# haowenz/FEM

Hardware: AMD Instinct MI355X
Metric: mapped Mreads/s (100 bp, e=3) at 1/2/4/8 MI355X + achieved HBM GB/s vs roofline (higher is better)
Workload: dtype u32/u64 integer + 32-bit Myers bit-vectors

## Files before the change

### fem_amd/csrc/fem_hip.hip

```cpp
#include "../../include/fem_hip.h"

#include <hip/hip_runtime.h>
#include <rccl/rccl.h>
#include <sched.h>
#if defined(__x86_64__)
#include <immintrin.h>
#endif

#include <algorithm>
#include <cctype>
#include <cstdio>
#include <cstdlib>
#include <cstring>
#include <condition_variable>
#include <functional>
#include <atomic>
#include <chrono>
#include <mutex>
#include <string>
#include <thread>
#include <vector>

#include "fem_index_build.hip.h"
#include "fem_pack.h"
#include "fem_kernels.hip.h"
#include "fem_seed_fast.hip.h"
#include "fem_seed_join.hip.h"
#include "fem_tail.hip.h"
#include "fem_bgzf.hip.h"

namespace {

#ifndef FEM_SLOTS
#define FEM_SLOTS 4
#endif
constexpr int kSlots = FEM_SLOTS;
constexpr uint32_t kMaxReadLen = 1024;
constexpr size_t kFrontPad = 16;
constexpr uint32_t kXcapSmall = 512, kFcap = 128, kCcap = 128;

constexpr int kTimedKernels = 15;
struct TimedLaunch {
  int kernel;
  hipEvent_t start, stop;
  bool counts = true;
};
constexpr int kMaxParts = 4;

struct Slot {
  hipStream_t stream = nullptr;
  uint8_t *d_bases_alloc = nullptr;
  uint8_t *bases() const { return d_bases_alloc + 16; }
  size_t bases_cap = 0;
  uint64_t *d_off = nullptr;
  size_t off_cap = 0;
  uint64_t n_reads = 0;
  uint64_t n_bases = 0;
  uint32_t max_len = 0;
  bool staged = false;
  char *h_bases = nullptr;
  size_t h_bases_cap = 0;
  uint64_t *h_off = nullptr;
  size_t h_off_cap = 0;
  uint64_t acq_reads = 0, acq_bases = 0;
  char *h_quals = nullptr, *h_names = nullptr;
  uint64_t *h_name_off = nullptr;
  size_t h_quals_cap = 0, h_names_cap = 0, h_name_off_cap = 0;
  uint8_t *d_quals = nullptr, *d_names = nullptr;
  uint64_t *d_name_off = nullptr;
  size_t d_quals_cap = 0, d_names_cap = 0, d_name_off_cap = 0;
  bool text_staged = false;
  bool host_quals = false;
  const uint64_t *qual_at = nullptr;
  hipStream_t text_stream = nullptr;
  hipStream_t out_stream = nullptr;
  hipEvent_t ev_text_staged = nullptr;
  hipEvent_t ev_text_order = nullptr;
  bool have_text_order = false;
  uint8_t *d_packed = nullptr;
  size_t packed_cap = 0;
  uint32_t *d_exc_bits = nullptr;
  size_t exc_bits_cap = 0;
  uint32_t packed_bpr = 0;
  bool prefetch_results = false, staged_by_copy = false;
  uint64_t prefetched_reads2 = 0, prefetched_cand = 0, last_n_cand = 0;
  uint64_t h2d_bytes = 0;
  bool sent_packed = false;
  int parts = 1;
  uint32_t part_begin[kMaxParts + 1] = {0, 0, 0, 0, 0};
  hipEvent_t ev_part[kMaxParts] = {nullptr, nullptr, nullptr, nullptr}, ev_sel[kMaxParts] = {nullptr, nullptr, nullptr, nullptr};
  hipEvent_t ev_zeroed = nullptr;
  hipEvent_t ev_results = nullptr, ev_home = nullptr;
  uint64_t *d_cand = nullptr;
  uint32_t *d_meta = nullptr;
  uint8_t *d_ed = nullptr;
  int16_t *d_end = nullptr;
  uint32_t cand_cap = 0;
  uint32_t *d_begin = nullptr, *d_count = nullptr, *d_nmap = nullptr;
  size_t per_read_cap = 0;
  uint8_t *d_ctl = nullptr;
  uint8_t *h_ctl = nullptr;
  uint64_t *d_arena = nullptr;
  uint64_t arena_cap = 0;
  uint32_t *d_slow = nullptr;
  uint32_t slow_cap = 0;
  uint2 *d_sel = nullptr, *d_sel_hdr = nullptr;
  size_t sel_cap = 0, sel_hdr_cap = 0;
  uint32_t *h_begin = nullptr, *h_count = nullptr;
  size_t h_per_read_cap = 0;
  uint64_t *h_cand = nullptr;
  uint8_t *h_ed = nullptr;
  int16_t *h_end = nullptr;
  size_t h_cand_cap = 0;
  uint8_t *d_count8 = nullptr, *d_ped = nullptr;
  uint32_t *d_seg = nullptr;
  uint64_t *d_pcand = nullptr;
  int16_t *d_pend = nullptr;
  uint2 *d_big = nullptr;
  size_t count8_cap = 0, seg_cap = 0, pcand_cap = 0;
  uint8_t *h_count8 = nullptr, *h_ped = nullptr;
  uint32_t *h_seg = nullptr;
  uint64_t *h_pcand = nullptr;
  int16_t *h_pend = nullptr;
  uint2 *h_big = nullptr;
  size_t h_count8_cap = 0, h_seg_cap = 0, h_pcand_cap = 0;
  bool want_packed = false;
  bool packed_enqueued = false;
  uint64_t packed_home = 0, last_n_packed = 0;
  bool packed_per_read_home = false;
  uint32_t n_packed = 0, n_big = 0;
  fem_params params{};
  bool mapped = false, synced = false;
  uint64_t stats[5] = {0, 0, 0, 0, 0};
  uint32_t n_cand = 0;
  std::vector<TimedLaunch> pending;
  femt::Tail *tail = nullptr;
  bool paired = false;
  int32_t min_insert = 0, max_insert = 0;
  uint64_t n_proper = 0;
  bool rescue = false;
  int32_t rescue_edits = 0;
  uint64_t n_rescued = 0;
  bool mapq = false;
  bool unmapped = false;
  uint64_t n_unmapped = 0;
  std::vector<uint16_t> pr_flag;
  std::vector<uint32_t> pr_tid, pr_pos0, pr_cigar_off, pr_cigar, pr_md_off;
  std::vector<uint8_t> pr_nm;
  std::vector<char> pr_md;
};

constexpr size_t kCtlPackCursor = 4 * sizeof(uint32_t) + 2 * sizeof(uint64_t) + 4 * sizeof(uint64_t);
constexpr size_t kCtlBytes = kCtlPackCursor + 2 * sizeof(uint32_t);
constexpr uint32_t kBigCap = 4096;
constexpr size_t kCtlWorkCursor = 128, kCtlWorkCursor2 = 192, kCtlPartStride = 128, kCtlAlloc = 1024;
static_assert(kCtlWorkCursor2 + (kMaxParts - 1) * kCtlPartStride + 64 <= kCtlAlloc, "control block layout");
static_assert(kCtlBytes <= kCtlWorkCursor, "control block layout");

}

namespace {
class StagePool {
 public:
  ~StagePool() {
    {
      std::lock_guard<std::mutex> l(m_);
      stop_ = true;
    }
    cv_.notify_all();
    for (auto &t : threads_) t.join();
  }
  void run(unsigned n, const std::function<void(unsigned)> &work) {
    if (n <= 1) return work(0u);
    {
      std::lock_guard<std::mutex> l(m_);
      while (threads_.size() + 1 < n) {
        const unsigned id = (unsigned)threads_.size() + 1;
        threads_.emplace_back([this, id] { loop(id); });
      }
      work_ = &work, n_ = n, pending_ = n - 1, ++epoch_;
    }
    cv_.notify_all();
    work(0u);
    std::unique_lock<std::mutex> l(m_);
    done_.wait(l, [&] { return pending_ == 0; });
    work_ = nullptr;
  }

 private:
  void loop(unsigned id) {
    uint64_t seen = 0;
    for (;;) {
      const std::function<void(unsigned)> *w = nullptr;
      {
        std::unique_lock<std::mutex> l(m_);
        cv_.wait(l, [&] { return stop_ || (epoch_ != seen && id < n_); });
        if (stop_) return;
        seen = epoch_, w = work_;
      }
      (*w)(id);
      std::lock_guard<std::mutex> l(m_);
      if (--pending_ == 0) done_.notify_one();
    }
  }
  std::mutex m_;
  std::condition_variable cv_, done_;
  std::vector<std::thread> threads_;
  const std::function<void(unsigned)> *work_ = nullptr;
  unsigned n_ = 0, pending_ = 0;
  uint64_t epoch_ = 0;
  bool stop_ = false;
};
}

struct fem_dev {
  femt::TextGate text_gate;
  femz::Bgzf *bgzf = nullptr;
  uint8_t *d_zin = nullptr;
  size_t d_zin_cap = 0;
  hipStream_t z_stream = nullptr;
  std::recursive_mutex mu;
  int device = 0;
  StagePool *stage_pool = nullptr;
  uint8_t *d_ref_names = nullptr;
  uint32_t *d_ref_name_off = nullptr;
  int n_cu = 256;
  std::string err;
  uint32_t *d_lookup = nullptr;
  uint64_t n_lookup = 0;
  uint64_t *d_occ = nullptr;
  uint64_t n_occ = 0;
  int32_t k = 0, step = 0;
  uint64_t fast_occ_key = ~0ull;
  int fast_occ_blocks = 0;
  uint32_t *d_summary = nullptr;
  uint32_t *d_occ32 = nullptr, *d_goff = nullptr, *d_blkseq = nullptr;
  uint32_t list_shift = 0;
  bool no_strided = false;
  uint32_t *d_freq11 = nullptr;
  uint32_t n_banks = 1, bank_first[5] = {0, 0, 0, 0, 0};
  uint32_t *d_bank_lo = nullptr;
  uint64_t bank_limit = 0;
  uint32_t bank_seqs = 0;
  int select_occ_blocks = 0, join_occ_blocks = 0;
  uint64_t select_occ_key = ~0ull, join_occ_key = ~0ull;
  uint8_t *d_planes = nullptr;
  uint8_t *d_ref_raw = nullptr;
  uint64_t ref_bytes = 0;
  uint64_t *d_seq_off = nullptr;
  uint32_t *d_seq_len = nullptr;
  uint32_t n_seq = 0;
  std::vector<uint64_t> seq_off;
  std::vector<uint32_t> seq_len;
  Slot slot[kSlots];
  bool timing = false;
  int verify_blocks_per_cu = 0;
  double t_ms[kTimedKernels] = {};
  uint64_t t_n[kTimedKernels] = {};
  bool force_generic = false;
  bool force_hash = false;
  bool force_dense = false;
  bool no_dense = false;
  bool tiny_buffers = false;
  std::vector<hipEvent_t> event_pool;
  hipEvent_t ev_kernels_done = nullptr;
  bool have_kernels_done = false;
  hipEvent_t ev_select_done = nullptr;
  bool have_select_done = false;
  bool no_overlap = false;
  hipEvent_t ev_h2d_done = nullptr;
  bool have_h2d_done = false;
  hipStream_t side_stream = nullptr;
  bool no_parts = false;
  int max_parts = 2;
  bool timeline = false, have_epoch = false;
  hipEvent_t ev_epoch = nullptr;
};

namespace {

bool testing_switch(const char *name) {
  const char *t = getenv("FEM_TESTING");
  if (!(t && t[0] == '1')) return false;
  const char *v = getenv(name);
  return v && v[0] == '1';
}

int fail(fem_dev *h, int rc, const std::string &msg) {
  if (h) {
    std::lock_guard<std::recursive_mutex> lock(h->mu);
    h->err = msg;
  }
  return rc;
}
#define FEM_LOCK(h) std::lock_guard<std::recursive_mutex> fem_lock_(h->mu)

#define HIP_TRY(h, expr)                                                                          \
  do {                                                                                            \
    hipError_t e_ = (expr);                                                                       \
    if (e_ != hipSuccess)                                                                         \
      return fail(h, e_ == hipErrorOutOfMemory ? FEM_ERR_NOMEM : FEM_ERR_HIP,                     \
                  std::string(#expr) + ": " + hipGetErrorString(e_));                             \
  } while (0)

template <typename T>
int dev_realloc(fem_dev *h, T **p, size_t *cap, size_t want, bool keep = false) {
  if (want <= *cap && *p) return FEM_OK;
  size_t n = std::max(want, *cap + *cap / 2);
  T *q = nullptr;
  HIP_TRY(h, hipMalloc((void **)&q, std::max<size_t>(n, 1) * sizeof(T)));
  if (keep && *p && *cap) HIP_TRY(h, hipMemcpy(q, *p, *cap * sizeof(T), hipMemcpyDeviceToDevice));
  if (*p) (void)hipFree(*p);
  *p = q;
  *cap = n;
  return FEM_OK;
}

template <typename T>
int pinned_realloc(fem_dev *h, T **p, size_t *cap, size_t want) {
  if (want <= *cap && *p) return FEM_OK;
  size_t n = std::max(want, *cap + *cap / 2);
  if (*p) (void)hipHostFree(*p);
  *p = nullptr;
  HIP_TRY(h, hipHostMalloc((void **)p, std::max<size_t>(n, 1) * sizeof(T), hipHostMallocDefault));
  *cap = n;
  return FEM_OK;
}

bool params_ok(const fem_params *p) {
  return p && p->k >= 1 && p->k <= 16 && p->step >= 1 && p->step <= 16 && p->e >= 0 && p->e <= 7 && p->a >= 0 &&
         p->a <= 2;
}

femk::SeedLayout make_layout(const fem_params &p, uint32_t max_len) {
  femk::SeedLayout l{};
  const uint32_t R = (uint32_t)(p.e + 1 + p.a);
  const uint32_t lg = (uint32_t)(p.k / p.step + (p.k % p.step ? 1 : 0));
  const uint32_t n_groups = 2u * (uint32_t)p.step;
  uint32_t smax = max_len >= (uint32_t)p.k ? max_len - (uint32_t)p.k + 1u : 1u;
  int c = (int)(smax / (uint32_t)p.step) - (int)(R * lg) + 2;
  uint32_t cmax = (uint32_t)std::max(c, 2);
  l.smax = smax;
  l.cmax = cmax;
  l.cw = (cmax + 31u) / 32u;
  l.n_words = (max_len + 15u) / 16u + 2u;
  l.xcap = kXcapSmall, l.fcap = kFcap, l.ccap = kCcap;
  uint32_t o = 0;
  auto take = [&](uint32_t bytes) {
    uint32_t at = o;
    o += (bytes + 15u) & ~15u;
    return at;
  };
  l.pkw = take(l.n_words * 4u);
  l.nkw = take(l.n_words * 4u);
  l.sf = take(2u * smax * 8u);
  l.dp_rows = take(n_groups * 2u * cmax * 4u);
  l.dp_bits = take(std::max(n_groups * R * l.cw * 4u, n_groups * R * 8u));
  l.picked = take(n_groups * R * 16u);
  l.rb = take(2u * (R + 1u) * 4u);
  l.X = take(l.xcap * 8u);
  l.F = take(l.fcap * 8u);
  l.A = take(l.ccap * 8u);
  l.B = take(l.ccap * 8u);
  l.wave_bytes = o;
  return l;
}

femk::SeedLayout make_layout_fast(const fem_params &p, uint32_t max_len, bool hash) {
  femk::SeedLayout l{};
  const uint32_t R = (uint32_t)(p.e + 1 + p.a);
  const uint32_t n_groups = 2u * (uint32_t)p.step;
  l.smax = max_len >= (uint32_t)p.k ? max_len - (uint32_t)p.k + 1u : 1u;
  l.n_words = (max_len + 15u) / 16u + 2u;
  l.xcap = 64;
  uint32_t o = 0;
  auto take = [&](uint32_t bytes) {
    uint32_t at = o;
    o += (bytes + 15u) & ~15u;
    return at;
  };
  if (hash) {
    l.pkw = take(l.n_words * 4u);
    l.nkw = take(l.n_words * 4u);
  }
  if (hash) l.sf = take(std::max(2u * l.smax * 8u, 2u * 64u * 8u));
  l.dp_bits = take(std::max(n_groups, femk::kGroupQueue) * R * 8u);
  if (hash) {
    l.X = take(64u * 8u);
    l.A = take(femk::kListScratchBytes);
  }
  l.B = take(2u * femk::kReadBlock * 8u);
  if (!hash) {
    const uint32_t blk_chars = femk::kReadBlock * std::min(max_len, 256u);
    l.strm_words = blk_chars / 16u + 3u;
    l.strm = take(3u * l.strm_words * 4u);
    const uint32_t q_at = o;
    l.F = take(femk::kQueueBytes);
    const uint32_t g0 = l.smax / (uint32_t)femk::kStep;
    const uint32_t n_used = g0 > (uint32_t)femk::kLg ? g0 - (uint32_t)femk::kLg + 1u : 1u;
    l.gq_cap = std::max(384u, n_groups * n_used);
    l.gq = take(std::max(l.gq_cap * 4u + femk::kGroupQueue * 16u + 2u * 32u * 4u, femk::kFlushScratchBytes));
    l.blk_bytes = blk_chars + 32u;
    l.blk = q_at;
    if (o < q_at + l.blk_bytes) take(q_at + l.blk_bytes - o);
  }
  if (hash) {
    l.xcap = (uint32_t)femk::bloom_chunks((int)R) * 64u;
    l.F = take(femk::bloom_slots((int)R) / 16u * 4u);
  }
  l.wave_bytes = o;
  return l;
}

femk::SeedLayout make_layout_select(const fem_params &p, uint32_t max_len) {
  femk::SeedLayout l{};
  const uint32_t R = (uint32_t)(p.e + 1 + p.a);
  l.smax = max_len >= (uint32_t)p.k ? max_len - (uint32_t)p.k + 1u : 1u;
  const uint32_t g_max = std::min<uint32_t>((l.smax + 2u) / 3u, femk::kSelMaxCols - 1u + 4u * R);
  l.gstride = 3u * g_max + 2u;
  l.gstride += l.gstride & 1u;
  if (!((l.gstride >> 1) & 1u)) l.gstride += 2u;
  l.nb = std::max<uint32_t>(1u, std::min<uint32_t>(femk::kReadBlock, 3100u / (2u * 2u * l.gstride)));
  l.strm_words = (l.nb * max_len + 15u) / 16u + 2u;
  uint32_t o = 0;
  auto take = [&](uint32_t bytes) {
    uint32_t at = o;
    o += (bytes + 15u) & ~15u;
    return at;
  };
  l.rb = take((femk::kReadBlock + 2u) * 8u);
  l.rinfo = take(4u * femk::kReadBlock * 4u);
  l.strm = take(2u * l.strm_words * 4u);
  l.fq = take(l.nb * 2u * l.gstride * 2u + 256u);
  l.wave_bytes = o;
  return l;
}

femk::SeedLayout make_layout_join(const fem_params &p, bool banked, bool padded = false) {
  femk::SeedLayout l{};
  const uint32_t R = (uint32_t)(p.e + 1 + p.a);
  uint32_t o = 0;
  auto take = [&](uint32_t bytes) {
    uint32_t at = o;
    o += (bytes + 15u) & ~15u;
    return at;
  };
  l.sf = take(2u * 64u * 4u);
  l.X = take(64u * 4u);
  l.A = take(3u * (femk::dense_flag_cap((int)R) + 1u) * 4u);
  l.B = take(2u * femk::kReadBlock * 8u);
  l.F = take(femk::join_bitmap_words((int)R, padded) * 4u);
  if (banked) l.gq = take(2u * 64u * 8u);
  l.wave_bytes = o;
  l.picked = 0;
  return l;
}

template <int R>
void launch_select_r(bool banked, dim3 grid, dim3 block, uint32_t lds, hipStream_t st, const femk::SeedParams &sp) {
  if (banked)
    hipLaunchKernelGGL((femk::seed_select_kernel<R, true>), grid, block, lds, st, sp);
  else
    hipLaunchKernelGGL((femk::seed_select_kernel<R>), grid, block, lds, st, sp);
}
template <int R>
int select_blocks_per_cu_r(bool banked, int block, uint32_t lds) {
  int nb = 0;
  const hipError_t e = banked ? hipOccupancyMaxActiveBlocksPerMultiprocessor(&nb, femk::seed_select_kernel<R, true>, block, lds)
                              : hipOccupancyMaxActiveBlocksPerMultiprocessor(&nb, femk::seed_select_kernel<R>, block, lds);
  return e == hipSuccess ? nb : 0;
}
typedef void (*JoinKernel)(femk::SeedParams);
JoinKernel join_kernel(int R, int which) {
  static const JoinKernel k[3][femk::kMaxR] = {
      {femk::seed_join_kernel_r1, femk::seed_join_kernel_r2, femk::seed_join_kernel_r3, femk::seed_join_kernel_r4, femk::seed_join_kernel_r5,
       femk::seed_join_kernel_r6, femk::seed_join_kernel_r7, femk::seed_join_kernel_r8, femk::seed_join_kernel_r9, femk::seed_join_kernel_r10},
      {femk::seed_join_banked_kernel_r1, femk::seed_join_banked_kernel_r2, femk::seed_join_banked_kernel_r3, femk::seed_join_banked_kernel_r4,
       femk::seed_join_banked_kernel_r5, femk::seed_join_banked_kernel_r6, femk::seed_join_banked_kernel_r7, femk::seed_join_banked_kernel_r8,
       femk::seed_join_banked_kernel_r9, femk::seed_join_banked_kernel_r10},
      {femk::seed_join_kernel_padded_r1, femk::seed_join_kernel_padded_r2, femk::seed_join_kernel_padded_r3, femk::seed_join_kernel_padded_r4,
       femk::seed_join_kernel_padded_r5, femk::seed_join_kernel_padded_r6, femk::seed_join_kernel_padded_r7, femk::seed_join_kernel_padded_r8,
       femk::seed_join_kernel_padded_r9, femk::seed_join_kernel_padded_r10}};
  return k[which][std::min(std::max(R, 1), femk::kMaxR) - 1];
}

#define FEM_DENSE_SWITCH(R, CALL)      \
  switch (R) {                         \
    case 1: CALL(1); break;            \
    case 2: CALL(2); break;            \
    case 3: CALL(3); break;            \
    case 4: CALL(4); break;            \
    case 5: CALL(5); break;            \
    case 6: CALL(6); break;            \
    case 7: CALL(7); break;            \
    case 8: CALL(8); break;            \
    case 9: CALL(9); break;            \
    default: CALL(10); break;          \
  }
template <int R>
uint32_t kernel_regs_r(bool join, int which) {
  hipFuncAttributes a{};
  const bool banked = which == 1;
  const void *f = join ? (const void *)join_kernel(R, which)
                       : banked ? (const void *)femk::seed_select_kernel<R, true> : (const void *)femk::seed_select_kernel<R>;
  return hipFuncGetAttributes(&a, f) == hipSuccess && a.numRegs > 0 ? (uint32_t)a.numRegs : 128u;
}
uint32_t kernel_regs(int R, bool join, int which = 0) {
  static std::atomic<uint32_t> cache[3][2][femk::kMaxR + 1] = {};
  std::atomic<uint32_t> &slot = cache[which][join ? 1 : 0][std::min(std::max(R, 1), femk::kMaxR)];
  uint32_t c = slot.load(std::memory_order_relaxed);
  if (c) return c;
#define FEM_CALL(r) c = kernel_regs_r<r>(join, which)
  FEM_DENSE_SWITCH(R, FEM_CALL)
#undef FEM_CALL
  slot.store(c, std::memory_order_relaxed);
  return c;
}
int select_blocks_per_cu(int R, bool banked, int block, uint32_t lds) {
  int nb = 0;
#define FEM_CALL(r) nb = select_blocks_per_cu_r<r>(banked, block, lds)
  FEM_DENSE_SWITCH(R, FEM_CALL)
#undef FEM_CALL
  return nb;
}
void launch_select(int R, bool banked, dim3 grid, dim3 block, uint32_t lds, hipStream_t st, const femk::SeedParams &sp) {
#define FEM_CALL(r) launch_select_r<r>(banked, grid, block, lds, st, sp)
  FEM_DENSE_SWITCH(R, FEM_CALL)
#undef FEM_CALL
}
int join_blocks_per_cu(int R, int which, int block, uint32_t lds) {
  int nb = 0;
  return hipOccupancyMaxActiveBlocksPerMultiprocessor(&nb, join_kernel(R, which), block, lds) == hipSuccess ? nb : 0;
}
void launch_join(int R, int which, dim3 grid, dim3 block, uint32_t lds, hipStream_t st, const femk::SeedParams &sp) {
  hipLaunchKernelGGL(join_kernel(R, which), grid, block, lds, st, sp);
}

template <int R>
void launch_fast(bool hash, dim3 grid, dim3 block, uint32_t lds, hipStream_t st, const femk::SeedParams &sp) {
  if (hash)
    hipLaunchKernelGGL((femk::seed_fast_kernel<R, true>), grid, block, lds, st, sp);
  else
    hipLaunchKernelGGL((femk::seed_fast_kernel<R, false>), grid, block, lds, st, sp);
}

template <int R>
int fast_blocks_per_cu_r(bool hash, int block, uint32_t lds) {
  int nb = 0;
  hipError_t err = hash ? hipOccupancyMaxActiveBlocksPerMultiprocessor(&nb, femk::seed_fast_kernel<R, true>, block, lds)
                        : hipOccupancyMaxActiveBlocksPerMultiprocessor(&nb, femk::seed_fast_kernel<R, false>, block, lds);
  return err == hipSuccess ? nb : 0;
}
int fast_blocks_per_cu(int R, bool hash, int block, uint32_t lds) {
  switch (R) {
    case 1: return fast_blocks_per_cu_r<1>(hash, block, lds);
    case 2: return fast_blocks_per_cu_r<2>(hash, block, lds);
    case 3: return fast_blocks_per_cu_r<3>(hash, block, lds);
    case 4: return fast_blocks_per_cu_r<4>(hash, block, lds);
    case 5: return fast_blocks_per_cu_r<5>(hash, block, lds);
    case 6: return fast_blocks_per_cu_r<6>(hash, block, lds);
    case 7: return fast_blocks_per_cu_r<7>(hash, block, lds);
    case 8: return fast_blocks_per_cu_r<8>(hash, block, lds);
    case 9: return fast_blocks_per_cu_r<9>(hash, block, lds);
    default: return fast_blocks_per_cu_r<10>(hash, block, lds);
  }
}

hipEvent_t get_event(fem_dev *h) {
  if (!h->event_pool.empty()) {
    hipEvent_t e = h->event_pool.back();
    h->event_pool.pop_back();
    return e;
  }
  hipEvent_t e = nullptr;
  (void)hipEventCreate(&e);
  return e;
}

struct Span {
  fem_dev *h;
  Slot &s;
  hipStream_t st;
  TimedLaunch t;
  bool on;
  Span(fem_dev *h_, Slot &s_, int id, hipStream_t st_) : h(h_), s(s_), st(st_), t{id, nullptr, nullptr, false}, on(h_->timing && h_->timeline) {
    if (on) {
      t.start = get_event(h), t.stop = get_event(h);
      (void)hipEventRecord(t.start, st);
    }
  }
  ~Span() {
    if (on) {
      (void)hipEventRecord(t.stop, st);
      s.pending.push_back(t);
    }
  }
};

void drain_timing(fem_dev *h, Slot &s) {
  for (auto &t : s.pending) {
    float ms = 0.f;
    if (hipEventElapsedTime(&ms, t.start, t.stop) == hipSuccess && t.kernel < kTimedKernels) {
      h->t_ms[t.kernel] += ms;
      h->t_n[t.kernel] += t.counts ? 1 : 0;
    }
    if (h->timeline && h->have_epoch) {
      float a = 0.f, b = 0.f;
      if (hipEventElapsedTime(&a, h->ev_epoch, t.start) == hipSuccess && hipEventElapsedTime(&b, h->ev_epoch, t.stop) == hipSuccess)
        fprintf(stderr, "TL slot %d id %2d  %9.3f %9.3f  (%.3f)\n", (int)(&s - h->slot), t.kernel, a, b, b - a);
    }
    h->event_pool.push_back(t.start);
    h->event_pool.push_back(t.stop);
  }
  s.pending.clear();
}

int ensure_outputs(fem_dev *h, Slot &s) {
  size_t want_reads = (size_t)s.n_reads;
  if (want_reads > s.per_read_cap || !s.d_begin) {
    size_t cap = std::max<size_t>(want_reads, 1);
    if (s.d_begin) (void)hipFree(s.d_begin);
    if (s.d_count) (void)hipFree(s.d_count);
    if (s.d_nmap) (void)hipFree(s.d_nmap);
    s.d_begin = s.d_count = s.d_nmap = nullptr;
    HIP_TRY(h, hipMalloc((void **)&s.d_begin, cap * 2 * sizeof(uint32_t)));
    HIP_TRY(h, hipMalloc((void **)&s.d_count, cap * 2 * sizeof(uint32_t)));
    HIP_TRY(h, hipMalloc((void **)&s.d_nmap, cap * sizeof(uint32_t)));
    s.per_read_cap = cap;
  }
  if (!s.d_cand || !s.d_meta || !s.d_ed || !s.d_end || s.cand_cap == 0) {
    for (void *p : {(void *)s.d_cand, (void *)s.d_meta, (void *)s.d_ed, (void *)s.d_end})
      if (p) (void)hipFree(p);
    s.d_cand = nullptr, s.d_meta = nullptr, s.d_ed = nullptr, s.d_end = nullptr;
    uint64_t want = 2 * s.n_reads + (5u << 20);
    if (h->tiny_buffers) want = 512;
    want = std::min<uint64_t>(want, 0xFFFFFFF0ull);
    s.cand_cap = 0;
    size_t c0 = 0, c1 = 0, c2 = 0, c3 = 0;
    int rc;
    if ((rc = dev_realloc(h, &s.d_cand, &c0, want))) return rc;
    if ((rc = dev_realloc(h, &s.d_meta, &c1, want))) return rc;
    if ((rc = dev_realloc(h, &s.d_ed, &c2, want))) return rc;
    if ((rc = dev_realloc(h, &s.d_end, &c3, want))) return rc;
    s.cand_cap = (uint32_t)want;
  }
  if (!s.d_ctl) {
    HIP_TRY(h, hipMalloc((void **)&s.d_ctl, kCtlAlloc));
    HIP_TRY(h, hipHostMalloc((void **)&s.h_ctl, kCtlBytes, hipHostMallocDefault));
  }
  if (!s.d_arena) {
    s.arena_cap = h->tiny_buffers ? 256u : (4u << 20);
    HIP_TRY(h, hipMalloc((void **)&s.d_arena, s.arena_cap * sizeof(uint64_t)));
  }
  {
    const double avg_bucket = (double)h->n_occ / (double)(h->n_lookup ? h->n_lookup : 1);
    uint64_t want = avg_bucket > 1.0 ? s.n_reads + (1u << 20) : (1u << 18);
    if (h->tiny_buffers) want = s.d_slow ? s.slow_cap : 32;
    if (want > s.slow_cap || !s.d_slow) {
      if (s.d_slow) (void)hipFree(s.d_slow);
      s.d_slow = nullptr;
      HIP_TRY(h, hipMalloc((void **)&s.d_slow, want * sizeof(uint32_t)));
      s.slow_cap = (uint32_t)want;
    }
  }
  return FEM_OK;
}

int grow_candidates(fem_dev *h, Slot &s, uint64_t want) {
  if (want > 0xFFFFFFF0ull) return fail(h, FEM_ERR_UNSUPPORTED, "more than 2^32 candidates in one batch; split the batch");
  s.cand_cap = 0;
  for (void *p : {(void *)s.d_cand, (void *)s.d_meta, (void *)s.d_ed, (void *)s.d_end})
    if (p) (void)hipFree(p);
  s.d_cand = nullptr, s.d_meta = nullptr, s.d_ed = nullptr, s.d_end = nullptr;
  HIP_TRY(h, hipMalloc((void **)&s.d_cand, want * sizeof(uint64_t)));
  HIP_TRY(h, hipMalloc((void **)&s.d_meta, want * sizeof(uint32_t)));
  HIP_TRY(h, hipMalloc((void **)&s.d_ed, want * sizeof(uint8_t)));
  HIP_TRY(h, hipMalloc((void **)&s.d_end, want * sizeof(int16_t)));
  s.cand_cap = (uint32_t)want;
  return FEM_OK;
}

int h2d_begin(fem_dev *h, Slot &s) {
  if (h->have_h2d_done) HIP_TRY(h, hipStreamWaitEvent(s.stream, h->ev_h2d_done, 0));
  return FEM_OK;
}
int h2d_end(fem_dev *h, Slot &s) {
  HIP_TRY(h, hipEventRecord(h->ev_h2d_done, s.stream));
  h->have_h2d_done = true;
  return FEM_OK;
}
bool device_idle(fem_dev *h) {
  return (!h->have_kernels_done || hipEventQuery(h->ev_kernels_done) == hipSuccess) &&
         (!h->have_select_done || hipEventQuery(h->ev_select_done) == hipSuccess);
}
constexpr uint64_t kPartMinReads = 1u << 16;

hipStream_t d2h_begin(fem_dev *h, Slot &s) {
  (void)h;
  return s.stream;
}
int d2h_end(fem_dev *h, Slot &s, hipStream_t st) {
  if (st == s.stream) return FEM_OK;
  HIP_TRY(h, hipEventRecord(s.ev_home, st));
  HIP_TRY(h, hipStreamWaitEvent(s.stream, s.ev_home, 0));
  return FEM_OK;
}

int enqueue_pack(fem_dev *h, Slot &s, bool kernel, bool send_home) {
  const size_t n2 = (size_t)s.n_reads * 2, n_seg = (n2 + 255) / 256;
  int rc;
  if ((rc = dev_realloc(h, &s.d_count8, &s.count8_cap, n2 + 16))) return rc;
  if ((rc = dev_realloc(h, &s.d_seg, &s.seg_cap, n_seg + 4))) return rc;
  if (s.pcand_cap < s.cand_cap || !s.d_pcand) {
    for (void *q : {(void *)s.d_pcand, (void *)s.d_ped, (void *)s.d_pend})
      if (q) (void)hipFree(q);
    s.d_pcand = nullptr, s.d_ped = nullptr, s.d_pend = nullptr, s.pcand_cap = 0;
    HIP_TRY(h, hipMalloc((void **)&s.d_pcand, (size_t)s.cand_cap * sizeof(uint64_t)));
    HIP_TRY(h, hipMalloc((void **)&s.d_ped, (size_t)s.cand_cap * sizeof(uint8_t)));
    HIP_TRY(h, hipMalloc((void **)&s.d_pend, (size_t)s.cand_cap * sizeof(int16_t)));
    s.pcand_cap = s.cand_cap;
  }
  if (!s.d_big) HIP_TRY(h, hipMalloc((void **)&s.d_big, kBigCap * sizeof(uint2)));
  if (n2 + 16 > s.h_count8_cap || !s.h_count8) {
    if (s.h_count8) (void)hipHostFree(s.h_count8);
    s.h_count8 = nullptr, s.h_count8_cap = 0;
    if ((rc = pinned_realloc(h, &s.h_count8, &s.h_count8_cap, n2 + 16))) return rc;
  }
  if (n_seg + 4 > s.h_seg_cap || !s.h_seg) {
    if (s.h_seg) (void)hipHostFree(s.h_seg);
    s.h_seg = nullptr, s.h_seg_cap = 0;
    if ((rc = pinned_realloc(h, &s.h_seg, &s.h_seg_cap, n_seg + 4))) return rc;
  }
  if (!s.h_big) {
    size_t c = 0;
    if ((rc = pinned_realloc(h, &s.h_big, &c, (size_t)kBigCap))) return rc;
  }
  if (kernel) {
  femk::PackParams pp{};
  pp.cand_begin = s.d_begin, pp.cand_count = s.d_count, pp.cand = s.d_cand, pp.ed = s.d_ed, pp.end = s.d_end;
  pp.ctr = (const uint32_t *)s.d_ctl, pp.n_strands = (uint32_t)n2;
  pp.count8 = s.d_count8, pp.seg_begin = s.d_seg, pp.pcand = s.d_pcand, pp.ped = s.d_ped, pp.pend = s.d_pend, pp.pcap = (uint32_t)s.pcand_cap;
  pp.cursor = (uint32_t *)(s.d_ctl + kCtlPackCursor), pp.big = s.d_big, pp.big_cap = kBigCap;
  const uint32_t grid = (uint32_t)std::max<size_t>(1, (n_seg + femk::kPackSegs - 1) / femk::kPackSegs);
  {
    TimedLaunch t{6, nullptr, nullptr, true};
    if (h->timing) {
      t.start = get_event(h), t.stop = get_event(h);
      HIP_TRY(h, hipEventRecord(t.start, s.stream));
    }
    hipLaunchKernelGGL(femk::pack_results_kernel, dim3(grid), dim3(256), 0, s.stream, pp);
    HIP_TRY(h, hipGetLastError());
    if (h->timing) {
      HIP_TRY(h, hipEventRecord(t.stop, s.stream));
      s.pending.push_back(t);
    }
  }
  s.packed_enqueued = true;
  }
  if (send_home) {
    hipStream_t st = d2h_begin(h, s);
    {
      Span span(h, s, 21, st);
      HIP_TRY(h, hipMemcpyAsync(s.h_count8, s.d_count8, n2, hipMemcpyDeviceToHost, st));
      HIP_TRY(h, hipMemcpyAsync(s.h_seg, s.d_seg, n_seg * sizeof(uint32_t), hipMemcpyDeviceToHost, st));
      s.packed_per_read_home = true;
      const size_t guess = std::min<size_t>({(size_t)(s.last_n_packed + s.last_n_packed / 32 + 1024), s.h_pcand_cap, s.pcand_cap});
      if (s.last_n_packed && s.h_pcand && guess) {
        HIP_TRY(h, hipMemcpyAsync(s.h_pcand, s.d_pcand, guess * sizeof(uint64_t), hipMemcpyDeviceToHost, st));
        HIP_TRY(h, hipMemcpyAsync(s.h_ped, s.d_ped, guess * sizeof(uint8_t), hipMemcpyDeviceToHost, st));
        HIP_TRY(h, hipMemcpyAsync(s.h_pend, s.d_pend, guess * sizeof(int16_t), hipMemcpyDeviceToHost, st));
        s.packed_home = guess;
      }
    }
    if ((rc = d2h_end(h, s, st))) return rc;
  }
  return FEM_OK;
}

int launch_batch(fem_dev *h, Slot &s) {
  const fem_params &p = s.params;
  uint32_t *d_ctr = (uint32_t *)s.d_ctl;
  unsigned long long *d_arena_ctr = (unsigned long long *)(s.d_ctl + 4 * sizeof(uint32_t));
  unsigned long long *d_stats = (unsigned long long *)(s.d_ctl + 4 * sizeof(uint32_t) + 2 * sizeof(uint64_t));
  int parts = 1;
  uint32_t part_begin[kMaxParts + 1] = {0, 0, 0, 0, 0};
  const bool copied_in_parts = s.parts > 1;
  {
    const int R_ = p.e + 1 + p.a;
    const bool dense_overlap = !h->force_generic && p.k == femk::kK && p.step == femk::kStep && R_ >= 1 && R_ <= femk::kMaxR && h->d_occ32 &&
                               h->d_freq11 && !h->no_overlap;
    if (dense_overlap && !h->no_parts && s.n_reads >= 2 * kPartMinReads && (copied_in_parts || device_idle(h))) {
      parts = copied_in_parts ? s.parts : (int)std::min<uint64_t>((uint64_t)h->max_parts, s.n_reads / kPartMinReads);
      for (int q = 0; q <= parts; ++q)
        part_begin[q] = copied_in_parts ? s.part_begin[q] : q == parts ? (uint32_t)s.n_reads : (uint32_t)((s.n_reads * q / parts) & ~63ull);
    }
    s.parts = 1;
  }
  if (parts > 1) {
    if (h->have_select_done) HIP_TRY(h, hipStreamWaitEvent(h->side_stream, h->ev_select_done, 0));
    HIP_TRY(h, hipMemsetAsync(s.d_ctl, 0, kCtlAlloc, h->side_stream));
  } else {
    HIP_TRY(h, hipMemsetAsync(s.d_ctl, 0, kCtlAlloc, s.stream));
  }

  femk::SeedParams sp{};
  sp.bases = s.bases();
  sp.read_off = s.d_off;
  sp.n_reads = (uint32_t)s.n_reads;
  sp.read_begin = 0;
  sp.lookup = h->d_lookup;
  sp.occ = h->d_occ;
  sp.inf32 = (uint32_t)h->n_occ;
  sp.seq_len = h->d_seq_len;
  sp.e = p.e, sp.a = p.a, sp.R = p.e + 1 + p.a, sp.k = p.k, sp.step = p.step;
  sp.lg = p.k / p.step + (p.k % p.step ? 1 : 0);
  sp.cand = s.d_cand, sp.cand_meta = s.d_meta, sp.cand_cap = s.cand_cap;
  sp.cand_begin = s.d_begin, sp.cand_count = s.d_count;
  sp.ctr = d_ctr;
  sp.work_cursor = (uint32_t *)(s.d_ctl + kCtlWorkCursor);
  sp.stats = d_stats;
  sp.arena = s.d_arena, sp.arena_cap = s.arena_cap, sp.arena_ctr = d_arena_ctr;
  sp.lay = make_layout(p, std::max<uint32_t>(s.max_len, (uint32_t)p.k));

  sp.n_seq = h->n_seq;
  sp.summary = h->d_summary;
  sp.slow_queue = s.d_slow, sp.slow_cap = s.slow_cap;
  sp.work_queue = nullptr;
  const int R = p.e + 1 + p.a;
  const bool use_fast = !h->force_generic && p.k == femk::kK && p.step == femk::kStep && R >= 1 && R <= femk::kMaxR;

  auto shape = [&](const femk::SeedLayout &lay, uint32_t *wpb_out, uint32_t *lds_out, uint32_t *grid_out) {
    uint32_t wpb = std::min<uint32_t>(4u, std::max<uint32_t>(1u, (64u * 1024u) / lay.wave_bytes));
    uint32_t lds_bytes = wpb * lay.wave_bytes;
    uint32_t waves_per_cu = std::min<uint32_t>(32u, (160u * 1024u / lds_bytes) * wpb);
    uint64_t blocks_wanted = (s.n_reads + wpb - 1) / wpb;
    uint64_t blocks_resident = (uint64_t)h->n_cu * std::max<uint32_t>(1u, waves_per_cu / wpb);
    *wpb_out = wpb, *lds_out = lds_bytes;
    *grid_out = (uint32_t)std::max<uint64_t>(1, std::min<uint64_t>(blocks_wanted, blocks_resident * 4));
  };
  if (sp.lay.wave_bytes > 64u * 1024u) return fail(h, FEM_ERR_UNSUPPORTED, "read too long for the device path");

  auto timed = [&](int id, hipStream_t st, auto &&launch, bool counts = true) -> int {
    TimedLaunch t{id, nullptr, nullptr, counts};
    if (h->timing) {
      t.start = get_event(h), t.stop = get_event(h);
      HIP_TRY(h, hipEventRecord(t.start, st));
    }
    launch();
    HIP_TRY(h, hipGetLastError());
    if (h->timing) {
      HIP_TRY(h, hipEventRecord(t.stop, st));
      s.pending.push_back(t);
    }
    return FEM_OK;
  };

  if (s.n_reads) {
    int rc;
    const bool split_dense = use_fast && h->d_occ32 && h->d_freq11;
    const bool overlap = split_dense && !h->no_overlap;
    if (!overlap && h->have_kernels_done) HIP_TRY(h, hipStreamWaitEvent(s.stream, h->ev_kernels_done, 0));
    femk::VerifyParams vp{};
    vp.bases = s.bases(), vp.read_off = s.d_off;
    vp.planes = h->d_planes, vp.seq_off = h->d_seq_off;
    vp.cand = s.d_cand, vp.cand_meta = s.d_meta;
    vp.ctr = d_ctr, vp.cand_cap = s.cand_cap, vp.e = p.e;
    vp.ed = s.d_ed, vp.end = s.d_end;
    vp.n_map = s.d_nmap, vp.stats = d_stats;
    HIP_TRY(h, hipMemsetAsync(s.d_nmap, 0, (size_t)s.n_reads * sizeof(uint32_t), s.stream));
    if (h->verify_blocks_per_cu == 0) {
      int nb = 0;
      if (hipOccupancyMaxActiveBlocksPerMultiprocessor(&nb, femk::verify_kernel, 256, 0) != hipSuccess || nb <= 0) nb = 4;
      h->verify_blocks_per_cu = nb;
    }
    const uint32_t vgrid = (uint32_t)h->n_cu * (uint32_t)h->verify_blocks_per_cu;
    if (split_dense) {
      const uint32_t max_len = std::max<uint32_t>(s.max_len, (uint32_t)p.k);
      const bool banked = h->n_banks > 1;
      const size_t want_sel = (size_t)s.n_reads * 6u * (size_t)R * h->n_banks;
      if ((rc = dev_realloc(h, &s.d_sel, &s.sel_cap, want_sel))) return rc;
      if ((rc = dev_realloc(h, &s.d_sel_hdr, &s.sel_hdr_cap, (size_t)s.n_reads))) return rc;
      femk::SeedParams fp = sp;
      fp.occ32 = h->d_occ32, fp.list_shift = h->list_shift, fp.goff = h->d_goff, fp.blkseq = h->d_blkseq;
      fp.freq11 = h->d_freq11, fp.sel = s.d_sel, fp.sel_hdr = s.d_sel_hdr;
      fp.n_banks = h->n_banks, fp.bank_lo = h->d_bank_lo, fp.n_buckets = (uint32_t)(h->n_lookup - 1);
      fp.blk_stride = (femk::kDenseRemap >> femk::kDenseBlkShift) + 1u;
      for (uint32_t b = 0; b <= femk::kDenseMaxBanks; ++b) fp.bank_first[b] = h->bank_first[b];
      uint32_t select_lds = 0, select_threads = 256;
      fp.lay = make_layout_select(p, max_len);
      if (fp.lay.wave_bytes > 64u * 1024u) return fail(h, FEM_ERR_UNSUPPORTED, "read too long for the device path");
      const femk::SeedLayout lay_select = fp.lay;
      femk::SeedLayout lay_join = make_layout_join(p, banked, !banked && h->list_shift != 0);
      const uint32_t wpb_s = std::min<uint32_t>(4u, std::max<uint32_t>(1u, (64u * 1024u) / lay_select.wave_bytes));
      const uint32_t wpb_j = std::min<uint32_t>(4u, std::max<uint32_t>(1u, (60u * 1024u) / lay_join.wave_bytes));
      lay_join.picked = wpb_j * lay_join.wave_bytes;
      const uint32_t lds_j = wpb_j * lay_join.wave_bytes + 64u * 8u;
      const int which = banked ? 1 : h->list_shift ? 2 : 0;
      uint64_t per_cu_s, per_cu_j;
      {
        const uint32_t lds_bytes = wpb_s * lay_select.wave_bytes;
        const uint64_t key = ((uint64_t)banked << 48) | ((uint64_t)R << 40) | lds_bytes;
        if (h->select_occ_key != key) h->select_occ_key = key, h->select_occ_blocks = select_blocks_per_cu(R, banked, (int)(64u * wpb_s), lds_bytes);
        per_cu_s = h->select_occ_blocks > 0 ? (uint64_t)h->select_occ_blocks : std::max<uint64_t>(1, 160u * 1024u / lds_bytes);
        if (overlap) per_cu_s = 1;
        select_lds = lds_bytes, select_threads = 64u * wpb_s;
      }
      {
        const uint64_t key = ((uint64_t)which << 48) | ((uint64_t)R << 40) | lds_j;
        if (h->join_occ_key != key) h->join_occ_key = key, h->join_occ_blocks = join_blocks_per_cu(R, which, (int)(64u * wpb_j), lds_j);
        per_cu_j = h->join_occ_blocks > 0 ? (uint64_t)h->join_occ_blocks : std::max<uint64_t>(1, 160u * 1024u / lds_j);
        if (overlap) {
          const uint32_t vj = (kernel_regs(R, true, which) + 7u) & ~7u, vs = (kernel_regs(R, false, banked ? 1 : 0) + 7u) & ~7u;
          const uint32_t wj = 64u * wpb_j / 256u ? 64u * wpb_j / 256u : 1u, ws = select_threads / 256u ? select_threads / 256u : 1u;
          const uint32_t lj = (lds_j + 511u) & ~511u, ls = (select_lds + 511u) & ~511u;
          while (per_cu_j > 1 && (per_cu_j * wj * vj + ws * vs > 512u || per_cu_j * lj + ls > 160u * 1024u || per_cu_j * wj + ws > 8u)) --per_cu_j;
        }
      }
      if (parts > 1 && !copied_in_parts) {
        HIP_TRY(h, hipEventRecord(s.ev_zeroed, s.stream));
        HIP_TRY(h, hipStreamWaitEvent(h->side_stream, s.ev_zeroed, 0));
      }
      for (int q = 0; q < parts; ++q) {
        const uint32_t r_lo = parts > 1 ? part_begin[q] : 0u, r_hi = parts > 1 ? part_begin[q + 1] : (uint32_t)s.n_reads;
        const uint64_t blocks_of_reads = ((uint64_t)(r_hi - r_lo) + femk::kReadBlock - 1) / femk::kReadBlock;
        fp.read_begin = r_lo, fp.n_reads = r_hi;
        hipStream_t st_sel = parts > 1 ? h->side_stream : s.stream;
        {
          fp.lay = lay_select;
          if (parts > 1) {
            if (copied_in_parts) HIP_TRY(h, hipStreamWaitEvent(st_sel, s.ev_part[q], 0));
          } else if (overlap && h->have_select_done) {
            HIP_TRY(h, hipStreamWaitEvent(s.stream, h->ev_select_done, 0));
          }
          const uint32_t grid = (uint32_t)std::max<uint64_t>(1, std::min<uint64_t>((blocks_of_reads + wpb_s - 1) / wpb_s, (uint64_t)h->n_cu * per_cu_s));
          fp.work_cursor = (uint32_t *)(s.d_ctl + kCtlWorkCursor + (size_t)q * kCtlPartStride);
          rc = timed(8, st_sel, [&] { launch_select(R, banked, dim3(grid), dim3(64u * wpb_s), select_lds, st_sel, fp); }, q == 0);
          if (rc) return rc;
          if (parts > 1) {
            HIP_TRY(h, hipEventRecord(s.ev_sel[q], st_sel));
            HIP_TRY(h, hipStreamWaitEvent(s.stream, s.ev_sel[q], 0));
          }
          if (overlap && q + 1 == parts) {
            HIP_TRY(h, hipEventRecord(h->ev_select_done, st_sel));
            h->have_select_done = true;
          }
          if (overlap && q == 0 && h->have_kernels_done) HIP_TRY(h, hipStreamWaitEvent(s.stream, h->ev_kernels_done, 0));
        }
        {
          fp.lay = lay_join;
          const uint32_t grid = (uint32_t)std::max<uint64_t>(1, std::min<uint64_t>((blocks_of_reads + wpb_j - 1) / wpb_j, (uint64_t)h->n_cu * per_cu_j));
          fp.work_cursor = (uint32_t *)(s.d_ctl + kCtlWorkCursor2 + (size_t)q * kCtlPartStride);
          rc = timed(0, s.stream, [&] { launch_join(R, which, dim3(grid), dim3(64u * wpb_j), lds_j, s.stream, fp); }, q == 0);
          if (rc) return rc;
        }
      }
      sp.work_queue = s.d_slow;
    } else if (use_fast) {
      femk::SeedParams fp = sp;
      const bool hash = h->force_hash || (double)h->n_occ > (double)h->n_lookup;
      fp.lay = make_layout_fast(p, std::max<uint32_t>(s.max_len, (uint32_t)p.k), hash);
      uint32_t wpb, lds_bytes, grid;
      shape(fp.lay, &wpb, &lds_bytes, &grid);
      {
        const uint64_t key = ((uint64_t)R << 40) | ((uint64_t)hash << 32) | lds_bytes;
        if (h->fast_occ_key != key) h->fast_occ_key = key, h->fast_occ_blocks = fast_blocks_per_cu((int)R, hash, (int)(64u * wpb), lds_bytes);
        static const uint64_t mult = testing_switch("FEM_TESTING") && getenv("FEM_GRID_MULT") ? (uint64_t)std::max(1, atoi(getenv("FEM_GRID_MULT"))) : 1;
        const uint64_t per_cu = h->fast_occ_blocks > 0 ? (uint64_t)h->fast_occ_blocks : std::max<uint64_t>(1, 160u * 1024u / lds_bytes);
        const uint64_t wanted = (s.n_reads + (uint64_t)femk::kReadBlock * wpb - 1) / ((uint64_t)femk::kReadBlock * wpb);
        grid = (uint32_t)std::max<uint64_t>(1, std::min<uint64_t>(wanted, (uint64_t)h->n_cu * per_cu * mult));
      }
      auto launch_range = [&](uint32_t lo, uint32_t hi) {
        femk::SeedParams q = fp;
        q.read_begin = lo, q.n_reads = hi;
        dim3 g(grid), b(64u * wpb);
        switch (R) {
          case 1: launch_fast<1>(hash, g, b, lds_bytes, s.stream, q); break;
          case 2: launch_fast<2>(hash, g, b, lds_bytes, s.stream, q); break;
          case 3: launch_fast<3>(hash, g, b, lds_bytes, s.stream, q); break;
          case 4: launch_fast<4>(hash, g, b, lds_bytes, s.stream, q); break;
          case 5: launch_fast<5>(hash, g, b, lds_bytes, s.stream, q); break;
          case 6: launch_fast<6>(hash, g, b, lds_bytes, s.stream, q); break;
          case 7: launch_fast<7>(hash, g, b, lds_bytes, s.stream, q); break;
          case 8: launch_fast<8>(hash, g, b, lds_bytes, s.stream, q); break;
          case 9: launch_fast<9>(hash, g, b, lds_bytes, s.stream, q); break;
          default: launch_fast<10>(hash, g, b, lds_bytes, s.stream, q); break;
        }
      };
      rc = timed(0, s.stream, [&] { launch_range(0, (uint32_t)s.n_reads); });
      if (rc) return rc;
      sp.work_queue = s.d_slow;
    }
    {
      uint32_t wpb, lds_bytes, grid;
      shape(sp.lay, &wpb, &lds_bytes, &grid);
      rc = timed(2, s.stream, [&] { hipLaunchKernelGGL(femk::seed_filter_kernel, dim3(grid), dim3(64u * wpb), lds_bytes, s.stream, sp); });
      if (rc) return rc;
    }
    rc = timed(1, s.stream, [&] { hipLaunchKernelGGL(femk::verify_kernel, dim3(vgrid), dim3(256), 0, s.stream, vp); });
    if (rc) return rc;
    s.packed_enqueued = false, s.packed_home = 0, s.packed_per_read_home = false;
    if (s.want_packed && split_dense && (rc = enqueue_pack(h, s, true, false))) return rc;
    HIP_TRY(h, hipEventRecord(h->ev_kernels_done, s.stream));
    h->have_kernels_done = true;
    if (s.want_packed && (rc = enqueue_pack(h, s, !split_dense, true))) return rc;
  } else {
    s.packed_enqueued = false, s.packed_home = 0, s.packed_per_read_home = false;
  }
  HIP_TRY(h, hipMemcpyAsync(s.h_ctl, s.d_ctl, kCtlBytes, hipMemcpyDeviceToHost, s.stream));
  s.prefetched_reads2 = 0, s.prefetched_cand = 0;
  static const bool no_prefetch = testing_switch("FEM_NO_PREFETCH");
  if (s.prefetch_results && !s.want_packed && s.staged_by_copy && !no_prefetch) {
    hipStream_t st = d2h_begin(h, s);
    {
      Span span(h, s, 21, st);
      const size_t n2 = (size_t)s.n_reads * 2;
      if (n2 && s.h_begin && n2 <= s.h_per_read_cap) {
        HIP_TRY(h, hipMemcpyAsync(s.h_begin, s.d_begin, n2 * sizeof(uint32_t), hipMemcpyDeviceToHost, st));
        HIP_TRY(h, hipMemcpyAsync(s.h_count, s.d_count, n2 * sizeof(uint32_t), hipMemcpyDeviceToHost, st));
        s.prefetched_reads2 = n2;
      }
      const size_t guess = std::min<size_t>({(size_t)(s.last_n_cand + s.last_n_cand / 32 + 1024), s.h_cand_cap, (size_t)s.cand_cap});
      if (s.last_n_cand && s.h_cand && guess) {
        HIP_TRY(h, hipMemcpyAsync(s.h_cand, s.d_cand, guess * sizeof(uint64_t), hipMemcpyDeviceToHost, st));
        HIP_TRY(h, hipMemcpyAsync(s.h_ed, s.d_ed, guess * sizeof(uint8_t), hipMemcpyDeviceToHost, st));
        HIP_TRY(h, hipMemcpyAsync(s.h_end, s.d_end, guess * sizeof(int16_t), hipMemcpyDeviceToHost, st));
        s.prefetched_cand = guess;
      }
    }
    int rc2 = d2h_end(h, s, st);
    if (rc2) return rc2;
  }
  s.mapped = true;
  s.synced = false;
  return FEM_OK;
}

int refresh_summary(fem_dev *h) {
  if (h->d_summary) (void)hipFree(h->d_summary);
  h->d_summary = nullptr;
  const uint64_t n_buckets = h->n_lookup - 1;
  if (h->n_occ >= n_buckets || h->n_occ >= 0x80000000ull || (n_buckets >> 3) >= (1ull << 22)) return FEM_OK;
  const uint64_t words = n_buckets / femk::kSummaryBuckets + 2;
  HIP_TRY(h, hipMalloc((void **)&h->d_summary, words * sizeof(uint32_t)));
  HIP_TRY(h, hipMemset(h->d_summary, 0, words * sizeof(uint32_t)));
  hipLaunchKernelGGL(femk::bucket_summary_kernel, dim3((uint32_t)h->n_cu * 8u), dim3(256), 0, 0, h->d_lookup, n_buckets, h->d_summary);
  HIP_TRY(h, hipGetLastError());
  HIP_TRY(h, hipDeviceSynchronize());
  return FEM_OK;
}

constexpr double kDenseMinAvgBucket = 4.0;
int refresh_dense(fem_dev *h) {
  for (void *p : {(void *)h->d_occ32, (void *)h->d_goff, (void *)h->d_blkseq, (void *)h->d_freq11, (void *)h->d_bank_lo})
    if (p) (void)hipFree(p);
  h->d_occ32 = nullptr, h->d_goff = nullptr, h->d_blkseq = nullptr, h->d_freq11 = nullptr, h->d_bank_lo = nullptr;
  h->n_banks = 1, h->list_shift = 0;
  if (!h->d_occ || !h->d_ref_raw || h->no_dense || h->k != femk::kK || h->step != femk::kStep || h->n_occ == 0) return FEM_OK;
  const uint64_t n_buckets = h->n_lookup - 1;
  if (!h->force_dense && (double)h->n_occ < kDenseMinAvgBucket * (double)n_buckets) return FEM_OK;
  const uint64_t limit = h->bank_limit ? std::min<uint64_t>(h->bank_limit, femk::kDenseLimit) : femk::kDenseLimit;
  const uint32_t seq_limit = h->bank_seqs ? std::min<uint32_t>(h->bank_seqs, femk::kDenseMaxSeq) : femk::kDenseMaxSeq;
  std::vector<uint32_t> goff(h->n_seq + 1);
  uint32_t n_banks = 1, bank_first[5] = {0, 0, 0, 0, 0};
  uint64_t cap = limit;
  {
    uint64_t total_c = femk::kDenseGap, longest = 0;
    for (uint32_t i = 0; i < h->n_seq; ++i) total_c += (uint64_t)h->seq_len[i] + femk::kDenseGap, longest = std::max<uint64_t>(longest, h->seq_len[i]);
    const uint64_t want = (total_c + limit - 1) / limit;
    if (want > 1) cap = std::min<uint64_t>(limit, (total_c + want - 1) / want + longest + femk::kDenseGap);
  }
  uint64_t at = femk::kDenseGap;
  for (uint32_t i = 0; i < h->n_seq; ++i) {
    if ((at + (uint64_t)h->seq_len[i] + femk::kDenseGap > cap && at != femk::kDenseGap) || i - bank_first[n_banks - 1] >= seq_limit) {
      if (n_banks == femk::kDenseMaxBanks) return FEM_OK;
      bank_first[n_banks++] = i;
      at = femk::kDenseGap;
    }
    goff[i] = (uint32_t)at;
    at += (uint64_t)h->seq_len[i] + femk::kDenseGap;
    if (at > femk::kDenseLimit) return FEM_OK;
  }
  goff[h->n_seq] = (uint32_t)at;
  for (uint32_t b = n_banks; b <= femk::kDenseMaxBanks; ++b) bank_first[b] = h->n_seq;
  const uint32_t n_blk = (femk::kDenseRemap >> femk::kDenseBlkShift) + 1u;
  std::vector<uint32_t> blkseq((size_t)n_blk * n_banks, 0);
  for (uint32_t bank = 0; bank < n_banks; ++bank)
    for (uint32_t b = 0, sq = bank_first[bank]; b < n_blk; ++b) {
      const uint64_t first = (uint64_t)b << femk::kDenseBlkShift;
      while (sq + 1u < bank_first[bank + 1] && goff[sq + 1u] <= first) ++sq;
      blkseq[(size_t)bank * n_blk + b] = sq;
    }
  uint32_t *d_bad = nullptr;
  auto decline = [&]() {
    for (void *q : {(void *)h->d_occ32, (void *)h->d_goff, (void *)h->d_blkseq, (void *)h->d_freq11, (void *)h->d_bank_lo, (void *)d_bad})
      if (q) (void)hipFree(q);
    h->d_occ32 = nullptr, h->d_goff = nullptr, h->d_blkseq = nullptr, h->d_freq11 = nullptr, h->d_bank_lo = nullptr;
    h->n_banks = 1, h->list_shift = 0;
    (void)hipGetLastError();
    return FEM_OK;
  };
  uint32_t list_shift = 0;
  const bool strided_pays = h->force_dense || h->n_occ >= (n_buckets << 4);
  if (n_banks == 1 && !h->no_strided && strided_pays) {
    const size_t words = ((size_t)n_buckets + femk::kDensePadBuckets) << femk::kDenseListShift;
    bool ok = hipMalloc((void **)&h->d_occ32, words * sizeof(uint32_t)) == hipSuccess;
    if (ok) {
      hipLaunchKernelGGL(femk::dense_pad_kernel, dim3((uint32_t)h->n_cu * 16u), dim3(256), 0, 0, (uint4 *)h->d_occ32, (uint64_t)(words / 4));
      ok = hipGetLastError() == hipSuccess;
    }
    if (ok) {
      list_shift = femk::kDenseListShift;
    } else {
      if (h->d_occ32) (void)hipFree(h->d_occ32);
      h->d_occ32 = nullptr;
      (void)hipGetLastError();
    }
  }
  if (hipMalloc((void **)&h->d_goff, goff.size() * sizeof(uint32_t)) != hipSuccess ||
      hipMalloc((void **)&h->d_blkseq, blkseq.size() * sizeof(uint32_t)) != hipSuccess ||
      (!list_shift && hipMalloc((void **)&h->d_occ32, (h->n_occ + 256) * sizeof(uint32_t)) != hipSuccess) ||
      hipMalloc((void **)&h->d_freq11, (size_t)femk::kX11 * 4u * sizeof(uint32_t)) != hipSuccess ||
      (n_banks > 1 && hipMalloc((void **)&h->d_bank_lo, (size_t)(n_banks - 1) * n_buckets * sizeof(uint32_t)) != hipSuccess) ||
      hipMalloc((void **)&d_bad, sizeof(uint32_t)) != hipSuccess)
    return decline();
  if (hipMemset(d_bad, 0, sizeof(uint32_t)) != hipSuccess ||
      hipMemcpy(h->d_goff, goff.data(), goff.size() * sizeof(uint32_t), hipMemcpyHostToDevice) != hipSuccess ||
      hipMemcpy(h->d_blkseq, blkseq.data(), blkseq.size() * sizeof(uint32_t), hipMemcpyHostToDevice) != hipSuccess) {
    (void)decline();
    return fail(h, FEM_ERR_HIP, "dense tables: copy to the device failed");
  }
  femk::BankFirst bf{};
  bf.n = n_banks;
  for (uint32_t b = 0; b <= femk::kDenseMaxBanks; ++b) bf.first[b] = bank_first[b];
  if (list_shift)
    hipLaunchKernelGGL(femk::dense_occ32_strided_kernel, dim3((uint32_t)h->n_cu * 8u), dim3(256), 0, 0, h->d_occ, h->d_lookup, (uint32_t)n_buckets, h->d_goff,
                       h->n_seq, h->d_occ32, d_bad);
  else
    hipLaunchKernelGGL(femk::dense_occ32_kernel, dim3((uint32_t)h->n_cu * 8u), dim3(256), 0, 0, h->d_occ, h->n_occ, h->d_goff, h->n_seq, bf,
                       h->d_occ32, d_bad);
  uint32_t bad = 0;
  if (hipGetLastError() != hipSuccess || hipMemcpy(&bad, d_bad, sizeof bad, hipMemcpyDeviceToHost) != hipSuccess) {
    (void)decline();
    return fail(h, FEM_ERR_HIP, "dense tables: building the 32-bit occurrence table failed");
  }
  if (bad) return decline();
  (void)hipFree(d_bad);
  d_bad = nullptr;
  for (uint32_t b = 1; b < n_banks; ++b)
    hipLaunchKernelGGL(femk::bank_split_kernel, dim3((uint32_t)h->n_cu * 8u), dim3(256), 0, 0, h->d_occ, h->d_lookup, (uint32_t)n_buckets, bank_first[b],
                       h->d_bank_lo + (size_t)(b - 1) * n_buckets);
  h->n_banks = n_banks, h->list_shift = list_shift;
  for (uint32_t b = 0; b <= femk::kDenseMaxBanks; ++b) h->bank_first[b] = bank_first[b];
  hipLaunchKernelGGL(femk::freq11_kernel, dim3((uint32_t)h->n_cu * 8u), dim3(256), 0, 0, h->d_lookup, h->d_freq11);
  HIP_TRY(h, hipGetLastError());
  HIP_TRY(h, hipDeviceSynchronize());
  return FEM_OK;
}

struct CommSet {
  std::vector<int> devs;
  std::vector<ncclComm_t> comms;
  std::vector<uint64_t *> bufs;
};
std::mutex g_comm_mu;
CommSet *g_comm = nullptr;
void destroy_comm_set() {
  if (!g_comm) return;
  for (size_t i = 0; i < g_comm->devs.size(); ++i) {
    (void)hipSetDevice(g_comm->devs[i]);
    if (g_comm->bufs[i]) (void)hipFree(g_comm->bufs[i]);
    if (g_comm->comms[i]) ncclCommDestroy(g_comm->comms[i]);
  }
  delete g_comm;
  g_comm = nullptr;
}

int check_slot(fem_dev *h, int slot) {
  if (!h) return FEM_ERR_INVALID;
  if (slot < 0 || slot >= kSlots) return fail(h, FEM_ERR_INVALID, "slot out of range");
  return FEM_OK;
}


using fempack::pack_bases;

int enqueue_packed(fem_dev *h, Slot &s, uint64_t n, uint32_t len, uint64_t n_exc) {
  const uint32_t bpr = fempack::bytes_per_read(len);
  const uint64_t code_bytes = fempack::code_bytes(n, len), n_bases = n * (uint64_t)len;
  const uint64_t total = code_bytes + n_exc * 5u;
  int rc;
  if ((rc = dev_realloc(h, &s.d_packed, &s.packed_cap, (size_t)total + 64))) return rc;
  if ((rc = dev_realloc(h, &s.d_bases_alloc, &s.bases_cap, kFrontPad + (size_t)n_bases + 64))) return rc;
  if ((rc = dev_realloc(h, &s.d_off, &s.off_cap, (size_t)n + 1))) return rc;
  if ((rc = dev_realloc(h, &s.d_exc_bits, &s.exc_bits_cap, (size_t)n / 32 + 2))) return rc;
  s.parts = 1;
  if (!h->no_parts && !h->no_overlap && n_exc == 0 && n >= 2 * kPartMinReads && device_idle(h))
    s.parts = (int)std::min<uint64_t>((uint64_t)h->max_parts, n / kPartMinReads);
  for (int q = 0; q <= s.parts; ++q) s.part_begin[q] = q == s.parts ? (uint32_t)n : (uint32_t)((n * q / s.parts) & ~63ull);
  HIP_TRY(h, hipMemsetAsync(s.d_exc_bits, 0, ((size_t)n / 32 + 1) * sizeof(uint32_t), s.stream));
  hipLaunchKernelGGL(femk::uniform_offsets_kernel, dim3((uint32_t)std::min<uint64_t>((n + 256) / 256, (uint64_t)h->n_cu * 8u)), dim3(256), 0,
                     s.stream, s.d_off, n, len);
  if ((rc = h2d_begin(h, s))) return rc;
  for (int q = 0; q < s.parts; ++q) {
    const uint64_t r0 = s.part_begin[q], r1 = s.part_begin[q + 1];
    const uint64_t b0 = r0 * bpr, b1 = q + 1 == s.parts ? total : r1 * bpr;
    Span span(h, s, 20, s.stream);
    if (b1 > b0) HIP_TRY(h, hipMemcpyAsync(s.d_packed + b0, s.h_bases + b0, b1 - b0, hipMemcpyHostToDevice, s.stream));
    if (q + 1 == s.parts && (rc = h2d_end(h, s))) return rc;
    if (r1 > r0) {
      const uint32_t grid = (uint32_t)std::min<uint64_t>(((r1 - r0) * bpr + 255) / 256, (uint64_t)h->n_cu * 16u);
      hipLaunchKernelGGL(femk::unpack_reads_kernel, dim3(grid), dim3(256), 0, s.stream, (const uint8_t *)s.d_packed + b0, r1 - r0, len, bpr,
                         s.bases() + r0 * len);
    }
    if (s.parts > 1) HIP_TRY(h, hipEventRecord(s.ev_part[q], s.stream));
  }
  if (n_exc) {
    const dim3 g((uint32_t)std::min<uint64_t>((n_exc + 255) / 256, (uint64_t)h->n_cu * 4u));
    hipLaunchKernelGGL(femk::scatter_chars_kernel, g, dim3(256), 0, s.stream, (const uint32_t *)(s.d_packed + code_bytes),
                       (const uint8_t *)(s.d_packed + code_bytes + 4u * n_exc), n_exc, s.bases());
    hipLaunchKernelGGL(femk::mark_exception_reads_kernel, g, dim3(256), 0, s.stream, (const uint32_t *)(s.d_packed + code_bytes), n_exc, len,
                       s.d_exc_bits);
  }
  s.packed_bpr = bpr;
  HIP_TRY(h, hipGetLastError());
  s.n_reads = n, s.n_bases = n_bases, s.max_len = len;
  s.staged = true, s.mapped = false, s.synced = false;
  s.h2d_bytes = total, s.sent_packed = true;
  return FEM_OK;
}

unsigned stage_threads(uint64_t n_reads) {
  unsigned want = 12;
  if (const char *e = getenv("FEM_STAGE_THREADS")) want = (unsigned)std::max(1, atoi(e));
  const unsigned hw = std::thread::hardware_concurrency();
  return (unsigned)std::max<uint64_t>(1, std::min<uint64_t>({(uint64_t)(hw ? hw : 1), (uint64_t)want, n_reads / 65536 + 1}));
}

}

extern "C" {

const char *fem_strerror(int rc) {
  switch (rc) {
    case FEM_OK: return "ok";
    case FEM_ERR_INVALID: return "invalid argument";
    case FEM_ERR_HIP: return "HIP runtime error";
    case FEM_ERR_NOMEM: return "out of memory";
    case FEM_ERR_STATE: return "call order violated";
    case FEM_ERR_UNSUPPORTED: return "input not supported by the device path";
    case FEM_ERR_RCCL: return "RCCL error";
    default: return "unknown error";
  }
}

const char *fem_dev_last_error(const fem_dev *h) { return h ? h->err.c_str() : "null handle"; }

static std::atomic<int> g_blocking_waits{0};
int fem_set_blocking_waits(int on) {
  g_blocking_waits.store(on ? 1 : 0);
  return FEM_OK;
}

int fem_dev_open(int device, fem_dev **out) {
  if (!out) return FEM_ERR_INVALID;
  *out = nullptr;
  int n = 0;
  if (hipGetDeviceCount(&n) != hipSuccess || n <= 0) return FEM_ERR_HIP;
  if (device < 0 || device >= n) return FEM_ERR_INVALID;
  fem_dev *h = new (std::nothrow) fem_dev();
  if (!h) return FEM_ERR_NOMEM;
  h->device = device;
  if (hipSetDevice(device) != hipSuccess) {
    delete h;
    return FEM_ERR_HIP;
  }
  if (g_blocking_waits.load() || testing_switch("FEM_BLOCKING_SYNC")) (void)hipSetDeviceFlags(hipDeviceScheduleBlockingSync);
  hipDeviceProp_t prop;
  if (hipGetDeviceProperties(&prop, device) == hipSuccess) h->n_cu = prop.multiProcessorCount;
  for (int i = 0; i < kSlots; ++i) {
    if (hipStreamCreateWithFlags(&h->slot[i].stream, hipStreamNonBlocking) != hipSuccess) {
      delete h;
      return FEM_ERR_HIP;
    }
  }
  bool ok_ev = hipEventCreateWithFlags(&h->ev_kernels_done, hipEventDisableTiming) == hipSuccess &&
               hipEventCreateWithFlags(&h->ev_select_done, hipEventDisableTiming) == hipSuccess &&
               hipEventCreateWithFlags(&h->ev_h2d_done, hipEventDisableTiming) == hipSuccess &&
               hipStreamCreateWithFlags(&h->side_stream, hipStreamNonBlocking) == hipSuccess;
  for (int i = 0; ok_ev && i < kSlots; ++i) {
    Slot &sl = h->slot[i];
    ok_ev = hipEventCreateWithFlags(&sl.ev_zeroed, hipEventDisableTiming) == hipSuccess &&
            hipEventCreateWithFlags(&sl.ev_results, hipEventDisableTiming) == hipSuccess &&
            hipEventCreateWithFlags(&sl.ev_home, hipEventDisableTiming) == hipSuccess;
    for (int q = 0; ok_ev && q < kMaxParts; ++q)
      ok_ev = hipEventCreateWithFlags(&sl.ev_part[q], hipEventDisableTiming) == hipSuccess &&
              hipEventCreateWithFlags(&sl.ev_sel[q], hipEventDisableTiming) == hipSuccess;
  }
  if (!ok_ev) {
    (void)fem_dev_close(h);
    return FEM_ERR_HIP;
  }
  if (testing_switch("FEM_TESTING")) {
    h->no_overlap = testing_switch("FEM_NO_OVERLAP");
    h->no_parts = testing_switch("FEM_NO_PARTS");
    if (const char *mp = getenv("FEM_PARTS")) h->max_parts = std::min(kMaxParts, std::max(1, atoi(mp)));
    h->timeline = testing_switch("FEM_TIMELINE");
    if (h->timeline && hipEventCreate(&h->ev_epoch) == hipSuccess && hipEventRecord(h->ev_epoch, h->side_stream) == hipSuccess)
      h->timing = true, h->have_epoch = true;
    h->force_generic = testing_switch("FEM_FORCE_GENERIC");
    h->force_hash = testing_switch("FEM_FORCE_HASH");
    h->force_dense = testing_switch("FEM_FORCE_DENSE");
    h->no_dense = testing_switch("FEM_NO_DENSE");
    h->no_strided = testing_switch("FEM_NO_STRIDED");
    h->tiny_buffers = testing_switch("FEM_TEST_TINY_BUFFERS");
    if (const char *bl = getenv("FEM_TEST_BANK_BASES")) h->bank_limit = strtoull(bl, nullptr, 10);
    if (const char *bs = getenv("FEM_TEST_BANK_SEQS")) h->bank_seqs = (uint32_t)strtoul(bs, nullptr, 10);
  }
  *out = h;
  return FEM_OK;
}

int fem_dev_close(fem_dev *h) {
  if (!h) return FEM_ERR_INVALID;
  {
    std::lock_guard<std::mutex> lock(g_comm_mu);
    if (g_comm && std::find(g_comm->devs.begin(), g_comm->devs.end(), h->device) != g_comm->devs.end()) destroy_comm_set();
  }
  (void)hipSetDevice(h->device);
  (void)hipDeviceSynchronize();
  delete h->stage_pool;
  h->stage_pool = nullptr;
  for (auto &s : h->slot) {
    drain_timing(h, s);
    for (void *p : {(void *)s.d_bases_alloc, (void *)s.d_off, (void *)s.d_cand, (void *)s.d_meta, (void *)s.d_ed,
                    (void *)s.d_end, (void *)s.d_begin, (void *)s.d_count, (void *)s.d_nmap, (void *)s.d_ctl,
                    (void *)s.d_arena, (void *)s.d_slow, (void *)s.d_sel, (void *)s.d_sel_hdr, (void *)s.d_packed, (void *)s.d_exc_bits, (void *)s.d_quals, (void *)s.d_names,
                    (void *)s.d_name_off, (void *)s.d_count8, (void *)s.d_seg, (void *)s.d_pcand, (void *)s.d_ped, (void *)s.d_pend, (void *)s.d_big})
      if (p) (void)hipFree(p);
    for (void *p : {(void *)s.h_ctl, (void *)s.h_begin, (void *)s.h_count, (void *)s.h_cand, (void *)s.h_ed,
                    (void *)s.h_end, (void *)s.h_bases, (void *)s.h_off, (void *)s.h_quals, (void *)s.h_names, (void *)s.h_name_off,
                    (void *)s.h_count8, (void *)s.h_seg, (void *)s.h_pcand, (void *)s.h_ped, (void *)s.h_pend, (void *)s.h_big})
      if (p) (void)hipHostFree(p);
    if (s.stream) (void)hipStreamDestroy(s.stream);
    if (s.text_stream) (void)hipStreamDestroy(s.text_stream);
    if (s.out_stream) (void)hipStreamDestroy(s.out_stream);
    if (s.ev_text_staged) (void)hipEventDestroy(s.ev_text_staged);
    if (s.ev_text_order) (void)hipEventDestroy(s.ev_text_order);
    delete s.tail;
    s.tail = nullptr;
  }
  delete h->bgzf;
  h->bgzf = nullptr;
  if (h->d_zin) (void)hipFree(h->d_zin);
  if (h->z_stream) (void)hipStreamDestroy(h->z_stream);
  if (h->d_ref_names) (void)hipFree(h->d_ref_names);
  if (h->d_ref_name_off) (void)hipFree(h->d_ref_name_off);
  for (hipEvent_t e : h->event_pool) (void)hipEventDestroy(e);
  if (h->ev_kernels_done) (void)hipEventDestroy(h->ev_kernels_done);
  if (h->ev_select_done) (void)hipEventDestroy(h->ev_select_done);
  if (h->ev_h2d_done) (void)hipEventDestroy(h->ev_h2d_done);
  if (h->ev_epoch) (void)hipEventDestroy(h->ev_epoch);
  if (h->side_stream) (void)hipStreamDestroy(h->side_stream);
  for (int i = 0; i < kSlots; ++i) {
    Slot &sl = h->slot[i];
    if (sl.ev_zeroed) (void)hipEventDestroy(sl.ev_zeroed);
    if (sl.ev_results) (void)hipEventDestroy(sl.ev_results);
    if (sl.ev_home) (void)hipEventDestroy(sl.ev_home);
    for (int q = 0; q < kMaxParts; ++q) {
      if (sl.ev_part[q]) (void)hipEventDestroy(sl.ev_part[q]);
      if (sl.ev_sel[q]) (void)hipEventDestroy(sl.ev_sel[q]);
    }
  }
  for (void *p : {(void *)h->d_lookup, (void *)h->d_occ, (void *)h->d_ref_raw, (void *)h->d_seq_off,
                  (void *)h->d_seq_len, (void *)h->d_summary, (void *)h->d_planes, (void *)h->d_occ32, (void *)h->d_goff, (void *)h->d_blkseq,
                  (void *)h->d_freq11, (void *)h->d_bank_lo})
    if (p) (void)hipFree(p);
  delete h;
  return FEM_OK;
}

int fem_dev_limits(const fem_dev *h, uint32_t *max_read_len, int32_t *n_slots) {
  if (!h) return FEM_ERR_INVALID;
  if (max_read_len) *max_read_len = kMaxReadLen;
  if (n_slots) *n_slots = kSlots;
  return FEM_OK;
}

int fem_dev_upload_index(fem_dev *h, int32_t k, int32_t step, const uint32_t *lookup, uint64_t n_lookup,
                         const uint64_t *occ, uint64_t n_occ) {
  if (!h || !lookup || (!occ && n_occ)) return FEM_ERR_INVALID;
  if (k < 1 || k > 16 || step < 1) return fail(h, FEM_ERR_INVALID, "k must be 1..16 and step >= 1");
  if (n_lookup != (1ull << (2 * k)) + 1) return fail(h, FEM_ERR_INVALID, "lookup table must have 4^k + 1 entries");
  if (n_occ > 0xFFFFFFFFull) return fail(h, FEM_ERR_INVALID, "occurrence table larger than its uint32 prefix sums");
  HIP_TRY(h, hipSetDevice(h->device));
  if (h->d_lookup) (void)hipFree(h->d_lookup);
  if (h->d_occ) (void)hipFree(h->d_occ);
  h->d_lookup = nullptr, h->d_occ = nullptr;
  HIP_TRY(h, hipMalloc((void **)&h->d_lookup, n_lookup * sizeof(uint32_t)));
  HIP_TRY(h, hipMalloc((void **)&h->d_occ, std::max<uint64_t>(n_occ, 1) * sizeof(uint64_t)));
  HIP_TRY(h, hipMemcpy(h->d_lookup, lookup, n_lookup * sizeof(uint32_t), hipMemcpyHostToDevice));
  if (n_occ) HIP_TRY(h, hipMemcpy(h->d_occ, occ, n_occ * sizeof(uint64_t), hipMemcpyHostToDevice));
  h->n_lookup = n_lookup, h->n_occ = n_occ, h->k = k, h->step = step;
  int rc = refresh_summary(h);
  return rc ? rc : refresh_dense(h);
}

namespace {
int make_codes(fem_dev *h, uint8_t **out) {
  *out = nullptr;
  uint8_t *codes = nullptr;
  const uint64_t total = h->ref_bytes;
  HIP_TRY(h, hipMalloc((void **)&codes, total + 128));
  hipError_t e = hipMemcpy(codes, h->d_ref_raw, total, hipMemcpyDeviceToDevice);
  if (e == hipSuccess) e = hipMemset(codes + total, 4, 128);
  if (e == hipSuccess && total) {
    hipLaunchKernelGGL(femk::ref_encode_kernel, dim3((uint32_t)h->n_cu * 8u), dim3(256), 0, 0, codes, total);
    e = hipGetLastError();
    if (e == hipSuccess) e = hipDeviceSynchronize();
  }
  if (e != hipSuccess) {
    (void)hipFree(codes);
    HIP_TRY(h, e);
  }
  *out = codes;
  return FEM_OK;
}
}

int fem_dev_upload_reference(fem_dev *h, uint32_t n_seq, const char *const *seq, const uint32_t *seq_len) {
  if (!h || !seq || !seq_len || n_seq == 0) return FEM_ERR_INVALID;
  HIP_TRY(h, hipSetDevice(h->device));
  h->seq_off.assign(n_seq, 0);
  h->seq_len.assign(seq_len, seq_len + n_seq);
  uint64_t total = 0;
  for (uint32_t i = 0; i < n_seq; ++i) {
    h->seq_off[i] = total;
    total += seq_len[i];
  }
  for (void *p : {(void *)h->d_ref_raw, (void *)h->d_seq_off, (void *)h->d_seq_len, (void *)h->d_planes})
    if (p) (void)hipFree(p);
  h->d_ref_raw = nullptr, h->d_seq_off = nullptr, h->d_seq_len = nullptr;
  h->d_planes = nullptr;
  h->ref_bytes = 0, h->n_seq = 0;
  HIP_TRY(h, hipMalloc((void **)&h->d_ref_raw, total + 128));
  HIP_TRY(h, hipMalloc((void **)&h->d_seq_off, n_seq * sizeof(uint64_t)));
  HIP_TRY(h, hipMalloc((void **)&h->d_seq_len, n_seq * sizeof(uint32_t)));
  for (uint32_t i = 0; i < n_seq; ++i)
    if (seq_len[i]) HIP_TRY(h, hipMemcpy(h->d_ref_raw + h->seq_off[i], seq[i], seq_len[i], hipMemcpyHostToDevice));
  HIP_TRY(h, hipMemset(h->d_ref_raw + total, 0, 128));
  HIP_TRY(h, hipMemcpy(h->d_seq_off, h->seq_off.data(), n_seq * sizeof(uint64_t), hipMemcpyHostToDevice));
  HIP_TRY(h, hipMemcpy(h->d_seq_len, h->seq_len.data(), n_seq * sizeof(uint32_t), hipMemcpyHostToDevice));
  HIP_TRY(h, hipMemset(h->d_ref_raw + total, 'N', 128));
  h->ref_bytes = total, h->n_seq = n_seq;
  {
    auto drop_reference = [&]() {
      for (void *q : {(void *)h->d_ref_raw, (void *)h->d_seq_off, (void *)h->d_seq_len, (void *)h->d_planes})
        if (q) (void)hipFree(q);
      h->d_ref_raw = nullptr, h->d_seq_off = nullptr, h->d_seq_len = nullptr, h->d_planes = nullptr;
      h->ref_bytes = 0, h->n_seq = 0;
    };
    uint8_t *codes = nullptr;
    int rc = make_codes(h, &codes);
    if (rc) {
      drop_reference();
      return rc;
    }
    const uint64_t n_pb = (total + 64 + 7) / 8;
    hipError_t e = hipMalloc((void **)&h->d_planes, femk::plane_bytes(n_pb));
    if (e == hipSuccess) e = hipMemset(h->d_planes, 0, femk::plane_bytes(n_pb));
    if (e == hipSuccess) {
      hipLaunchKernelGGL(femk::ref_planes_kernel, dim3((uint32_t)h->n_cu * 8u), dim3(256), 0, 0, codes, h->d_ref_raw, n_pb, h->d_planes);
      e = hipGetLastError();
      if (e == hipSuccess) e = hipDeviceSynchronize();
    }
    (void)hipFree(codes);
    if (e != hipSuccess) drop_reference();
    HIP_TRY(h, e);
  }
  return refresh_dense(h);
}

int fem_dev_build_index(fem_dev *h, int32_t k, int32_t step, uint32_t *lookup_out, uint64_t *occ_out, uint64_t occ_cap,
                        uint64_t *n_occ_out) {
  if (!h) return FEM_ERR_INVALID;
  if (!h->d_ref_raw) return fail(h, FEM_ERR_STATE, "upload the reference before building the index");
  if (k < 1 || k > 16 || step < 1) return fail(h, FEM_ERR_INVALID, "k must be 1..16 and step >= 1");
  HIP_TRY(h, hipSetDevice(h->device));
  if (h->d_lookup) (void)hipFree(h->d_lookup);
  if (h->d_occ) (void)hipFree(h->d_occ);
  h->d_lookup = nullptr, h->d_occ = nullptr;
  uint64_t n_occ = 0;
  std::string err;
  uint8_t *codes = nullptr;
  int rc = make_codes(h, &codes);
  if (rc) return rc;
  rc = femix::build_index(codes, h->seq_off, h->seq_len, k, step, h->n_cu, &h->d_lookup, &h->d_occ, &n_occ, &err);
  (void)hipFree(codes);
  if (rc != FEM_OK) return fail(h, rc, err);
  h->n_lookup = (1ull << (2 * k)) + 1, h->n_occ = n_occ, h->k = k, h->step = step;
  if ((rc = refresh_summary(h))) return rc;
  if ((rc = refresh_dense(h))) return rc;
  if (n_occ_out) *n_occ_out = n_occ;
  if (lookup_out)
    HIP_TRY(h, hipMemcpy(lookup_out, h->d_lookup, h->n_lookup * sizeof(uint32_t), hipMemcpyDeviceToHost));
  if (occ_out) {
    if (occ_cap < n_occ) return fail(h, FEM_ERR_INVALID, "occ_out too small");
    if (n_occ) HIP_TRY(h, hipMemcpy(occ_out, h->d_occ, n_occ * sizeof(uint64_t), hipMemcpyDeviceToHost));
  }
  return FEM_OK;
}

int fem_dev_fetch_index(fem_dev *h, uint32_t *lookup_out, uint64_t *occ_out, uint64_t occ_cap) {
  if (!h) return FEM_ERR_INVALID;
  if (!h->d_lookup) return fail(h, FEM_ERR_STATE, "no index is resident");
  HIP_TRY(h, hipSetDevice(h->device));
  if (lookup_out) HIP_TRY(h, hipMemcpy(lookup_out, h->d_lookup, h->n_lookup * sizeof(uint32_t), hipMemcpyDeviceToHost));
  if (occ_out) {
    if (occ_cap < h->n_occ) return fail(h, FEM_ERR_INVALID, "occ_out too small");
    if (h->n_occ) HIP_TRY(h, hipMemcpy(occ_out, h->d_occ, h->n_occ * sizeof(uint64_t), hipMemcpyDeviceToHost));
  }
  return FEM_OK;
}

int fem_dev_acquire_stage(fem_dev *h, int slot, uint64_t n_reads_cap, uint64_t n_bases_cap, char **bases, uint64_t **offsets) {
  int rc = check_slot(h, slot);
  if (rc) return rc;
  FEM_LOCK(h);
  if (!bases || !offsets) return fail(h, FEM_ERR_INVALID, "null output pointer");
  if (n_reads_cap > 0x3FFFFFF0ull) return fail(h, FEM_ERR_UNSUPPORTED, "more than 2^30 reads in one batch");
  Slot &s = h->slot[slot];
  HIP_TRY(h, hipSetDevice(h->device));
  HIP_TRY(h, hipStreamSynchronize(s.stream));
  if (s.out_stream) HIP_TRY(h, hipStreamSynchronize(s.out_stream));
  drain_timing(h, s);
  if ((rc = pinned_realloc(h, &s.h_bases, &s.h_bases_cap, (size_t)n_bases_cap + 64))) return rc;
  if ((rc = pinned_realloc(h, &s.h_off, &s.h_off_cap, (size_t)n_reads_cap + 1))) return rc;
  s.staged = false, s.mapped = false, s.synced = false, s.text_staged = false;
  s.acq_reads = n_reads_cap, s.acq_bases = n_bases_cap;
  *bases = s.h_bases, *offsets = s.h_off;
  return FEM_OK;
}

int fem_dev_commit_stage(fem_dev *h, int slot, uint64_t n_reads, uint32_t max_len) {
  int rc = check_slot(h, slot);
  if (rc) return rc;
  FEM_LOCK(h);
  Slot &s = h->slot[slot];
  if (!s.h_bases || !s.h_off) return fail(h, FEM_ERR_STATE, "acquire the slot's staging buffers first");
  if (n_reads > s.acq_reads) return fail(h, FEM_ERR_INVALID, "more reads than the staging buffers were acquired for");
  if (max_len > kMaxReadLen)
    return fail(h, FEM_ERR_UNSUPPORTED, "read longer than the device path supports (" + std::to_string(kMaxReadLen) + ")");
  const uint64_t n_bases = n_reads ? s.h_off[n_reads] : 0;
  if (n_reads && (s.h_off[0] != 0 || n_bases > s.acq_bases)) return fail(h, FEM_ERR_INVALID, "staged offsets must start at 0 and end inside the buffer");
  HIP_TRY(h, hipSetDevice(h->device));
  if ((rc = dev_realloc(h, &s.d_bases_alloc, &s.bases_cap, kFrontPad + (size_t)n_bases + 64))) return rc;
  if ((rc = dev_realloc(h, &s.d_off, &s.off_cap, (size_t)n_reads + 1))) return rc;
  if ((rc = h2d_begin(h, s))) return rc;
  if (n_bases) HIP_TRY(h, hipMemcpyAsync(s.bases(), s.h_bases, n_bases, hipMemcpyHostToDevice, s.stream));
  if (n_reads) HIP_TRY(h, hipMemcpyAsync(s.d_off, s.h_off, (n_reads + 1) * sizeof(uint64_t), hipMemcpyHostToDevice, s.stream));
  if ((rc = h2d_end(h, s))) return rc;
  s.parts = 1;
  s.n_reads = n_reads, s.n_bases = n_bases, s.max_len = max_len;
  s.staged = true, s.mapped = false, s.synced = false;
  s.h2d_bytes = n_bases + (n_reads ? (n_reads + 1) * sizeof(uint64_t) : 0), s.sent_packed = false, s.staged_by_copy = false;
  return FEM_OK;
}

int fem_dev_commit_stage_uniform(fem_dev *h, int slot, uint64_t n_reads, uint32_t read_len) {
  int rc = check_slot(h, slot);
  if (rc) return rc;
  FEM_LOCK(h);
  Slot &s = h->slot[slot];
  if (!s.h_bases) return fail(h, FEM_ERR_STATE, "acquire the slot's staging buffers first");
  if (read_len > kMaxReadLen)
    return fail(h, FEM_ERR_UNSUPPORTED, "read longer than the device path supports (" + std::to_string(kMaxReadLen) + ")");
  const uint64_t n_bases = n_reads * (uint64_t)read_len;
  if (n_reads > s.acq_reads || n_bases > s.acq_bases) return fail(h, FEM_ERR_INVALID, "more reads than the staging buffers were acquired for");
  HIP_TRY(h, hipSetDevice(h->device));
  if ((rc = dev_realloc(h, &s.d_bases_alloc, &s.bases_cap, kFrontPad + (size_t)n_bases + 64))) return rc;
  if ((rc = dev_realloc(h, &s.d_off, &s.off_cap, (size_t)n_reads + 1))) return rc;
  if ((rc = h2d_begin(h, s))) return rc;
  if (n_bases) HIP_TRY(h, hipMemcpyAsync(s.bases(), s.h_bases, n_bases, hipMemcpyHostToDevice, s.stream));
  if ((rc = h2d_end(h, s))) return rc;
  s.parts = 1;
  hipLaunchKernelGGL(femk::uniform_offsets_kernel, dim3((uint32_t)std::min<uint64_t>((n_reads + 256) / 256, (uint64_t)h->n_cu * 8u)), dim3(256), 0,
                     s.stream, s.d_off, n_reads, read_len);
  HIP_TRY(h, hipGetLastError());
  s.n_reads = n_reads, s.n_bases = n_bases, s.max_len = read_len;
  s.staged = true, s.mapped = false, s.synced = false;
  s.h2d_bytes = n_bases, s.sent_packed = false, s.staged_by_copy = false;
  return FEM_OK;
}

int fem_dev_packed_layout(uint64_t n_reads, uint32_t read_len, uint32_t *bytes_per_read, uint64_t *exc_offset, uint64_t *exc_cap) {
  if (read_len == 0 || read_len > kMaxReadLen) return FEM_ERR_INVALID;
  const uint64_t n_bases = n_reads * (uint64_t)read_len, cb = fempack::code_bytes(n_reads, read_len);
  if (bytes_per_read) *bytes_per_read = fempack::bytes_per_read(read_len);
  if (exc_offset) *exc_offset = cb;
  if (exc_cap) *exc_cap = std::min<uint64_t>((n_bases + 64 - std::min<uint64_t>(cb, n_bases + 64)) / 5u, n_bases / 16u);
  return FEM_OK;
}

int fem_dev_commit_stage_packed(fem_dev *h, int slot, uint64_t n_reads, uint32_t read_len, uint64_t n_exceptions) {
  int rc = check_slot(h, slot);
  if (rc) return rc;
  FEM_LOCK(h);
  Slot &s = h->slot[slot];
  if (!s.h_bases) return fail(h, FEM_ERR_STATE, "acquire the slot's staging buffers first");
  if (read_len == 0 && n_reads) return fail(h, FEM_ERR_INVALID, "packed batches hold reads of one non-zero length");
  if (read_len > kMaxReadLen)
    return fail(h, FEM_ERR_UNSUPPORTED, "read longer than the device path supports (" + std::to_string(kMaxReadLen) + ")");
  const uint64_t n_bases = n_reads * (uint64_t)read_len;
  if (n_reads > s.acq_reads || n_bases > s.acq_bases) return fail(h, FEM_ERR_INVALID, "more reads than the staging buffers were acquired for");
  if (n_bases >= 0xFFFFFFF0ull) return fail(h, FEM_ERR_UNSUPPORTED, "a packed batch holds fewer than 2^32 bases; split the batch");
  const uint64_t code_bytes = fempack::code_bytes(n_reads, read_len);
  if (code_bytes + n_exceptions * 5u > s.acq_bases + 64 || n_exceptions > n_bases / 16u)
    return fail(h, FEM_ERR_INVALID, "more exceptions than a packed batch may carry (fem_dev_packed_layout): commit the characters instead");
  const uint32_t *pos = (const uint32_t *)(s.h_bases + code_bytes);
  for (uint64_t i = 0; i < n_exceptions; ++i)
    if (pos[i] >= n_bases) return fail(h, FEM_ERR_INVALID, "exception position outside the batch");
  HIP_TRY(h, hipSetDevice(h->device));
  if ((rc = enqueue_packed(h, s, n_reads, read_len, n_exceptions))) return rc;
  s.staged_by_copy = true;
  return FEM_OK;
}

int fem_dev_stage_reads(fem_dev *h, int slot, const fem_read_batch *reads) {
  int rc = check_slot(h, slot);
  if (rc) return rc;
  if (!reads || (reads->n_reads && (!reads->bases || !reads->offsets))) return fail(h, FEM_ERR_INVALID, "null read batch");
  if (reads->n_reads > 0x3FFFFFF0ull) return fail(h, FEM_ERR_UNSUPPORTED, "more than 2^30 reads in one batch");
  const uint64_t n = reads->n_reads;
  const uint64_t base0 = n ? reads->offsets[0] : 0;
  if (n && reads->offsets[n] < base0) return fail(h, FEM_ERR_INVALID, "read offsets must be ascending");
  const uint64_t n_bases = n ? reads->offsets[n] - base0 : 0;
  char *hb = nullptr;
  uint64_t *ho = nullptr;
  if ((rc = fem_dev_acquire_stage(h, slot, n, n_bases, &hb, &ho))) return rc;
  Slot &s = h->slot[slot];
  const unsigned n_thr = stage_threads(n);
  if (!h->stage_pool) h->stage_pool = new (std::nothrow) StagePool();
  if (!h->stage_pool) return fail(h, FEM_ERR_NOMEM, "out of host memory");
  auto run_threads = [&](unsigned nt, const std::function<void(unsigned)> &work) { h->stage_pool->run(nt, work); };
  std::vector<uint32_t> t_max(n_thr, 0), t_min(n_thr, 0xFFFFFFFFu);
  std::atomic<int> bad{0};
  run_threads(n_thr, [&](unsigned t) {
    const uint64_t r_lo = n * t / n_thr, r_hi = n * (t + 1) / n_thr;
    uint32_t mx = 0, mn = 0xFFFFFFFFu;
    for (uint64_t i = r_lo; i < r_hi; ++i) {
      const uint64_t o0 = reads->offsets[i], o1 = reads->offsets[i + 1];
      if (o1 < o0) {
        bad.store(1);
        return;
      }
      const uint64_t len = o1 - o0;
      if (len > kMaxReadLen) {
        bad.store(2);
        return;
      }
      mx = std::max<uint32_t>(mx, (uint32_t)len), mn = std::min<uint32_t>(mn, (uint32_t)len);
    }
    t_max[t] = mx, t_min[t] = mn;
  });
  if (bad.load() == 1) return fail(h, FEM_ERR_INVALID, "read offsets must be ascending");
  if (bad.load() == 2)
    return fail(h, FEM_ERR_UNSUPPORTED, "read longer than the device path supports (" + std::to_string(kMaxReadLen) + ")");
  uint32_t max_len = 0, min_len = 0xFFFFFFFFu;
  for (unsigned t = 0; t < n_thr; ++t) max_len = std::max(max_len, t_max[t]), min_len = std::min(min_len, t_min[t]);
  const bool no_pack = testing_switch("FEM_NO_PACK");
  if (n && min_len == max_len && max_len > 0 && n_bases < 0xFFFFFFF0ull && !no_pack) {
    const uint32_t len = max_len, bpr = (len + 3u) / 4u;
    const uint64_t code_bytes = (n * bpr + 7u) & ~7ull;
    const uint64_t exc_cap = (n_bases + 64 - std::min<uint64_t>(code_bytes, n_bases + 64)) / 5u;
    std::vector<std::vector<uint64_t>> exc(n_thr);
    const uint8_t *src = (const uint8_t *)reads->bases + base0;
    constexpr uint64_t kPiece = 32768;
    std::atomic<uint64_t> next_piece{0};
    run_threads(n_thr, [&](unsigned t) {
      for (;;) {
        const uint64_t r_lo = next_piece.fetch_add(1, std::memory_order_relaxed) * kPiece;
        if (r_lo >= n) break;
        const uint64_t r_hi = std::min(n, r_lo + kPiece);
        if ((len & 3u) == 0u) {
          pack_bases(src + r_lo * len, (r_hi - r_lo) * len, (uint8_t *)hb + r_lo * bpr, r_lo * len, exc[t]);
        } else {
          for (uint64_t i = r_lo; i < r_hi; ++i) pack_bases(src + i * len, len, (uint8_t *)hb + i * bpr, i * len, exc[t]);
        }
      }
    });
    uint64_t n_exc = 0;
    for (const auto &v : exc) n_exc += v.size();
    if (n_exc <= exc_cap && n_exc <= n_bases / 16u) {
      uint32_t *he = (uint32_t *)(hb + code_bytes);
      uint8_t *hc = (uint8_t *)(he + n_exc);
      for (const auto &v : exc)
        for (uint64_t x : v) *he++ = (uint32_t)(x >> 8), *hc++ = (uint8_t)x;
      {
        FEM_LOCK(h);
        if ((rc = enqueue_packed(h, s, n, len, n_exc))) return rc;
      }
      s.staged_by_copy = true;
      return FEM_OK;
    }
  }
  run_threads(n_thr, [&](unsigned t) {
    const uint64_t r_lo = n * t / n_thr, r_hi = n * (t + 1) / n_thr;
    for (uint64_t i = r_lo; i < r_hi; ++i) ho[i] = reads->offsets[i] - base0;
    if (r_hi == n) ho[n] = reads->offsets[n] - base0;
    if (r_hi > r_lo) memcpy(hb + (reads->offsets[r_lo] - base0), reads->bases + reads->offsets[r_lo], reads->offsets[r_hi] - reads->offsets[r_lo]);
  });
  if (n == 0) ho[0] = 0;
  rc = fem_dev_commit_stage(h, slot, n, max_len);
  s.staged_by_copy = true;
  return rc;
}

int fem_dev_stage_info(fem_dev *h, int slot, uint64_t *h2d_bytes, int32_t *packed) {
  int rc = check_slot(h, slot);
  if (rc) return rc;
  if (h2d_bytes) *h2d_bytes = h->slot[slot].h2d_bytes;
  if (packed) *packed = h->slot[slot].sent_packed ? 1 : 0;
  return FEM_OK;
}

int fem_dev_map_staged(fem_dev *h, int slot, const fem_params *p) {
  int rc = check_slot(h, slot);
  if (rc) return rc;
  FEM_LOCK(h);
  if (!params_ok(p)) return fail(h, FEM_ERR_INVALID, "parameters out of range (k 1..16, step 1..16, e 0..7, a 0..2)");
  if (!h->d_lookup || !h->d_ref_raw || !h->d_planes) return fail(h, FEM_ERR_STATE, "index and reference must be uploaded first");
  if (p->k != h->k) return fail(h, FEM_ERR_INVALID, "k differs from the uploaded index");
  Slot &s = h->slot[slot];
  if (!s.staged) return fail(h, FEM_ERR_STATE, "no reads staged in this slot");
  HIP_TRY(h, hipSetDevice(h->device));
  s.params = *p;
  if ((rc = ensure_outputs(h, s))) return rc;
  return launch_batch(h, s);
}

int fem_dev_sync(fem_dev *h, int slot) {
  int rc = check_slot(h, slot);
  if (rc) return rc;
  Slot &s = h->slot[slot];
  if (!s.mapped) return fail(h, FEM_ERR_STATE, "nothing was mapped in this slot");
  HIP_TRY(h, hipSetDevice(h->device));
  if (s.synced) return FEM_OK;
  for (int attempt = 0; attempt < 8; ++attempt) {
    HIP_TRY(h, hipStreamSynchronize(s.stream));
    FEM_LOCK(h);
    drain_timing(h, s);
    const uint32_t *ctr = (const uint32_t *)s.h_ctl;
    const uint64_t *arena_ctr = (const uint64_t *)(s.h_ctl + 4 * sizeof(uint32_t));
    const uint64_t *st = (const uint64_t *)(s.h_ctl + 4 * sizeof(uint32_t) + 2 * sizeof(uint64_t));
    uint32_t flags = ctr[1];
    if (flags & femk::kFlagTooLarge)
      return fail(h, FEM_ERR_UNSUPPORTED, "a read selects more than 2^31 occurrence entries in one seed group");
    if (flags == 0) {
      s.n_cand = ctr[0];
      s.n_packed = ((const uint32_t *)(s.h_ctl + kCtlPackCursor))[0], s.n_big = ((const uint32_t *)(s.h_ctl + kCtlPackCursor))[1];
      s.stats[0] = s.n_reads;
      s.stats[1] = st[3];
      s.stats[2] = st[0];
      s.stats[3] = st[1];
      s.stats[4] = st[2];
      s.synced = true;
      return FEM_OK;
    }
    if (flags & femk::kFlagCandOverflow) {
      uint64_t want = (uint64_t)ctr[0] + ctr[0] / 8 + 1024;
      if ((rc = grow_candidates(h, s, std::min<uint64_t>(want, 0xFFFFFFF0ull)))) return rc;
    }
    if (flags & femk::kFlagQueueOverflow) {
      uint64_t want = (uint64_t)ctr[2] + ctr[2] / 8 + 4096;
      (void)hipFree(s.d_slow);
      s.d_slow = nullptr;
      s.slow_cap = 0;
      hipError_t e = hipMalloc((void **)&s.d_slow, want * sizeof(uint32_t));
      if (e != hipSuccess) return fail(h, FEM_ERR_NOMEM, "slow-read queue does not fit in device memory");
      s.slow_cap = (uint32_t)std::min<uint64_t>(want, 0xFFFFFFF0ull);
    }
    if (flags & femk::kFlagArenaOverflow) {
      uint64_t want = arena_ctr[1] + arena_ctr[1] / 8 + 1024;
      (void)hipFree(s.d_arena);
      s.d_arena = nullptr;
      hipError_t e = hipMalloc((void **)&s.d_arena, want * sizeof(uint64_t));
      if (e != hipSuccess) {
        s.arena_cap = 0;
        return fail(h, FEM_ERR_NOMEM, "scratch arena for oversized seed lists does not fit in device memory; use smaller batches");
      }
      s.arena_cap = want;
    }
    if ((rc = launch_batch(h, s))) return rc;
  }
  return fail(h, FEM_ERR_HIP, "batch kept overflowing its scratch buffers");
}

int fem_dev_fetch_stats(fem_dev *h, int slot, uint64_t stats[5]) {
  int rc = fem_dev_sync(h, slot);
  if (rc) return rc;
  if (stats) memcpy(stats, h->slot[slot].stats, sizeof(uint64_t) * 5);
  h->slot[slot].prefetch_results = false;
  return FEM_OK;
}

int fem_dev_fetch(fem_dev *h, int slot, fem_batch_result *out) {
  int rc = fem_dev_sync(h, slot);
  if (rc) return rc;
  if (!out) return fail(h, FEM_ERR_INVALID, "null result");
  Slot &s = h->slot[slot];
  const size_t n2 = (size_t)s.n_reads * 2, nc = s.n_cand;
  bool regrown = false;
  if (n2 > s.h_per_read_cap || !s.h_begin) {
    regrown = true;
    size_t c0 = 0, c1 = 0;
    if (s.h_begin) (void)hipHostFree(s.h_begin);
    if (s.h_count) (void)hipHostFree(s.h_count);
    s.h_begin = s.h_count = nullptr;
    if ((rc = pinned_realloc(h, &s.h_begin, &c0, std::max<size_t>(n2, 2)))) return rc;
    if ((rc = pinned_realloc(h, &s.h_count, &c1, std::max<size_t>(n2, 2)))) return rc;
    s.h_per_read_cap = c0;
  }
  if (nc > s.h_cand_cap || !s.h_cand) {
    regrown = true;
    size_t c0 = 0, c1 = 0, c2 = 0;
    for (void *p : {(void *)s.h_cand, (void *)s.h_ed, (void *)s.h_end})
      if (p) (void)hipHostFree(p);
    s.h_cand = nullptr, s.h_ed = nullptr, s.h_end = nullptr;
    size_t want = std::max<size_t>(nc + nc / 4, 1024);
    if ((rc = pinned_realloc(h, &s.h_cand, &c0, want))) return rc;
    if ((rc = pinned_realloc(h, &s.h_ed, &c1, want))) return rc;
    if ((rc = pinned_realloc(h, &s.h_end, &c2, want))) return rc;
    s.h_cand_cap = c0;
  }
  const bool per_read_home = !regrown && s.prefetched_reads2 == n2;
  const size_t c_from = regrown ? 0 : std::min<size_t>(s.prefetched_cand, nc);
  if (n2 && !per_read_home) {
    HIP_TRY(h, hipMemcpyAsync(s.h_begin, s.d_begin, n2 * sizeof(uint32_t), hipMemcpyDeviceToHost, s.stream));
    HIP_TRY(h, hipMemcpyAsync(s.h_count, s.d_count, n2 * sizeof(uint32_t), hipMemcpyDeviceToHost, s.stream));
  }
  if (nc > c_from) {
    HIP_TRY(h, hipMemcpyAsync(s.h_cand + c_from, s.d_cand + c_from, (nc - c_from) * sizeof(uint64_t), hipMemcpyDeviceToHost, s.stream));
    HIP_TRY(h, hipMemcpyAsync(s.h_ed + c_from, s.d_ed + c_from, (nc - c_from) * sizeof(uint8_t), hipMemcpyDeviceToHost, s.stream));
    HIP_TRY(h, hipMemcpyAsync(s.h_end + c_from, s.d_end + c_from, (nc - c_from) * sizeof(int16_t), hipMemcpyDeviceToHost, s.stream));
  }
  if ((n2 && !per_read_home) || nc > c_from) HIP_TRY(h, hipStreamSynchronize(s.stream));
  s.prefetch_results = true, s.last_n_cand = nc, s.want_packed = false;
  out->n_reads = s.n_reads;
  out->n_candidates = nc;
  out->cand_begin = s.h_begin, out->cand_count = s.h_count;
  out->cand = s.h_cand, out->ed = s.h_ed, out->end = s.h_end;
  memcpy(out->stats, s.stats, sizeof s.stats);
  return FEM_OK;
}

int fem_dev_fetch_packed(fem_dev *h, int slot, fem_batch_packed *out) {
  int rc = fem_dev_sync(h, slot);
  if (rc) return rc;
  if (!out) return fail(h, FEM_ERR_INVALID, "null result");
  Slot &s = h->slot[slot];
  const size_t n2 = (size_t)s.n_reads * 2, n_seg = (n2 + 255) / 256;
  if (!s.packed_enqueued && s.n_reads) {
    if ((rc = enqueue_pack(h, s, true, false))) return rc;
    HIP_TRY(h, hipMemcpyAsync(s.h_ctl, s.d_ctl, kCtlBytes, hipMemcpyDeviceToHost, s.stream));
    HIP_TRY(h, hipStreamSynchronize(s.stream));
    s.n_packed = ((const uint32_t *)(s.h_ctl + kCtlPackCursor))[0], s.n_big = ((const uint32_t *)(s.h_ctl + kCtlPackCursor))[1];
  }
  if (s.n_big > kBigCap) return fail(h, FEM_ERR_UNSUPPORTED, "more strands with 255 candidates and more than a packed result lists: use fem_dev_fetch");
  const size_t np = s.n_reads ? s.n_packed : 0;
  bool regrown = false;
  if (np > s.h_pcand_cap || !s.h_pcand) {
    regrown = true;
    for (void *q : {(void *)s.h_pcand, (void *)s.h_ped, (void *)s.h_pend})
      if (q) (void)hipHostFree(q);
    s.h_pcand = nullptr, s.h_ped = nullptr, s.h_pend = nullptr;
    size_t c0 = 0, c1 = 0, c2 = 0;
    const size_t want = std::max<size_t>(np + np / 4, 1024);
    if ((rc = pinned_realloc(h, &s.h_pcand, &c0, want))) return rc;
    if ((rc = pinned_realloc(h, &s.h_ped, &c1, want))) return rc;
    if ((rc = pinned_realloc(h, &s.h_pend, &c2, want))) return rc;
    s.h_pcand_cap = c0;
  }
  bool copied = false;
  if (n2 && !s.packed_per_read_home) {
    HIP_TRY(h, hipMemcpyAsync(s.h_count8, s.d_count8, n2, hipMemcpyDeviceToHost, s.stream));
    HIP_TRY(h, hipMemcpyAsync(s.h_seg, s.d_seg, n_seg * sizeof(uint32_t), hipMemcpyDeviceToHost, s.stream));
    s.packed_per_read_home = true, copied = true;
  }
  const size_t c_from = regrown ? 0 : std::min<size_t>(s.packed_home, np);
  if (np > c_from) {
    HIP_TRY(h, hipMemcpyAsync(s.h_pcand + c_from, s.d_pcand + c_from, (np - c_from) * sizeof(uint64_t), hipMemcpyDeviceToHost, s.stream));
    HIP_TRY(h, hipMemcpyAsync(s.h_ped + c_from, s.d_ped + c_from, (np - c_from) * sizeof(uint8_t), hipMemcpyDeviceToHost, s.stream));
    HIP_TRY(h, hipMemcpyAsync(s.h_pend + c_from, s.d_pend + c_from, (np - c_from) * sizeof(int16_t), hipMemcpyDeviceToHost, s.stream));
    s.packed_home = np, copied = true;
  }
  if (s.n_big) {
    HIP_TRY(h, hipMemcpyAsync(s.h_big, s.d_big, (size_t)s.n_big * sizeof(uint2), hipMemcpyDeviceToHost, s.stream));
    copied = true;
  }
  if (copied) HIP_TRY(h, hipStreamSynchronize(s.stream));
  s.want_packed = true, s.last_n_packed = np;
  out->n_reads = s.n_reads;
  out->n_candidates = np;
  out->count = s.h_count8, out->seg_begin = s.h_seg;
  out->cand = s.h_pcand, out->ed = s.h_ped, out->end = s.h_pend;
  out->big = (const uint32_t *)s.h_big, out->n_big = s.n_big;
  memcpy(out->stats, s.stats, sizeof s.stats);
  return FEM_OK;
}

int fem_dev_upload_reference_names(fem_dev *h, uint32_t n_seq, const char *names, const uint64_t *name_off) {
  if (!h || !names || !name_off || n_seq == 0) return FEM_ERR_INVALID;
  if (h->n_seq && n_seq != h->n_seq) return fail(h, FEM_ERR_INVALID, "as many names as reference sequences, please");
  if (name_off[n_seq] < name_off[0] || name_off[n_seq] - name_off[0] > 0xFFFFFFF0ull) return fail(h, FEM_ERR_INVALID, "name offsets out of range");
  HIP_TRY(h, hipSetDevice(h->device));
  std::vector<uint32_t> off(n_seq + 1);
  for (uint32_t i = 0; i <= n_seq; ++i) {
    if (name_off[i] < name_off[0] || (i && name_off[i] < name_off[i - 1])) return fail(h, FEM_ERR_INVALID, "name offsets must be ascending");
    off[i] = (uint32_t)(name_off[i] - name_off[0]);
  }
  if (h->d_ref_names) (void)hipFree(h->d_ref_names);
  if (h->d_ref_name_off) (void)hipFree(h->d_ref_name_off);
  h->d_ref_names = nullptr, h->d_ref_name_off = nullptr;
  HIP_TRY(h, hipMalloc((void **)&h->d_ref_names, std::max<size_t>(off[n_seq], 1)));
  HIP_TRY(h, hipMalloc((void **)&h->d_ref_name_off, (n_seq + 1) * sizeof(uint32_t)));
  if (off[n_seq]) HIP_TRY(h, hipMemcpy(h->d_ref_names, names + name_off[0], off[n_seq], hipMemcpyHostToDevice));
  HIP_TRY(h, hipMemcpy(h->d_ref_name_off, off.data(), (n_seq + 1) * sizeof(uint32_t), hipMemcpyHostToDevice));
  return FEM_OK;
}

int fem_dev_acquire_text_stage(fem_dev *h, int slot, uint64_t n_reads_cap, uint64_t n_bases_cap, uint64_t n_name_bytes_cap, char **quals,
                               char **names, uint64_t **name_off) {
  int rc = check_slot(h, slot);
  if (rc) return rc;
  FEM_LOCK(h);
  if (!quals || !names || !name_off) return fail(h, FEM_ERR_INVALID, "null output pointer");
  Slot &s = h->slot[slot];
  HIP_TRY(h, hipSetDevice(h->device));
  HIP_TRY(h, hipStreamSynchronize(s.stream));
  if (s.text_stream) HIP_TRY(h, hipStreamSynchronize(s.text_stream));
  if (s.out_stream) HIP_TRY(h, hipStreamSynchronize(s.out_stream));
  if ((rc = pinned_realloc(h, &s.h_quals, &s.h_quals_cap, (size_t)n_bases_cap + 64))) return rc;
  if ((rc = pinned_realloc(h, &s.h_names, &s.h_names_cap, (size_t)n_name_bytes_cap + 64))) return rc;
  if ((rc = pinned_realloc(h, &s.h_name_off, &s.h_name_off_cap, (size_t)n_reads_cap + 1))) return rc;
  s.text_staged = false;
  *quals = s.h_quals, *names = s.h_names, *name_off = s.h_name_off;
  return FEM_OK;
}

int fem_dev_reserve_text(fem_dev *h, int slot, uint64_t n_reads, uint64_t n_bases, uint64_t n_name_bytes, uint64_t text_bytes) {
  int rc = check_slot(h, slot);
  if (rc) return rc;
  FEM_LOCK(h);
  Slot &s = h->slot[slot];
  HIP_TRY(h, hipSetDevice(h->device));
  if ((rc = dev_realloc(h, &s.d_bases_alloc, &s.bases_cap, kFrontPad + (size_t)n_bases + 64))) return rc;
  if ((rc = dev_realloc(h, &s.d_off, &s.off_cap, (size_t)n_reads + 1))) return rc;
  if ((rc = dev_realloc(h, &s.d_quals, &s.d_quals_cap, (size_t)n_bases + 64))) return rc;
  if ((rc = dev_realloc(h, &s.d_names, &s.d_names_cap, (size_t)n_name_bytes + 64))) return rc;
  if ((rc = dev_realloc(h, &s.d_name_off, &s.d_name_off_cap, (size_t)n_reads + 1))) return rc;
  if (!s.tail) s.tail = new (std::nothrow) femt::Tail();
  if (!s.tail) return fail(h, FEM_ERR_NOMEM, "out of host memory");
  std::string err;
  if ((rc = s.tail->reserve_text(text_bytes, &err))) return fail(h, rc, err);
  return FEM_OK;
}

static hipStream_t out_stream_of(fem_dev *h, Slot &s) {
  static const bool plain = testing_switch("FEM_NO_OUT_PRIORITY");
  if (plain) return s.stream;
  if (!s.out_stream) {
    int least = 0, greatest = 0;
    if (hipDeviceGetStreamPriorityRange(&least, &greatest) != hipSuccess ||
        hipStreamCreateWithPriority(&s.out_stream, hipStreamNonBlocking, greatest) != hipSuccess)
      s.out_stream = nullptr;
  }
  (void)h;
  return s.out_stream ? s.out_stream : s.stream;
}

int fem_dev_reserve_batch(fem_dev *h, int slot, uint64_t n_reads, uint64_t n_records, uint32_t max_len, const fem_params *p) {
  int rc = check_slot(h, slot);
  if (rc) return rc;
  FEM_LOCK(h);
  if (!params_ok(p)) return fail(h, FEM_ERR_INVALID, "parameters out of range (k 1..16, step 1..16, e 0..7, a 0..2)");
  if (!h->d_lookup) return fail(h, FEM_ERR_STATE, "the index must be uploaded first (what a batch needs depends on it)");
  if (n_reads == 0 || n_reads > 0x7FFFFFF0ull || n_records > 0xFFFFFFF0ull || max_len == 0 || max_len > kMaxReadLen)
    return fail(h, FEM_ERR_INVALID, "batch shape out of range");
  Slot &s = h->slot[slot];
  if (s.mapped && !s.synced) return fail(h, FEM_ERR_STATE, "a batch is in flight in this slot");
  HIP_TRY(h, hipSetDevice(h->device));
  const uint64_t n_was = s.n_reads;
  s.n_reads = n_reads;
  rc = ensure_outputs(h, s);
  s.n_reads = n_was;
  if (rc) return rc;
  const uint64_t n_bases = n_reads * (uint64_t)max_len;
  if ((rc = dev_realloc(h, &s.d_packed, &s.packed_cap, (size_t)fempack::code_bytes(n_reads, max_len) + 64))) return rc;
  if ((rc = dev_realloc(h, &s.d_bases_alloc, &s.bases_cap, kFrontPad + (size_t)n_bases + 64))) return rc;
  if ((rc = dev_realloc(h, &s.d_off, &s.off_cap, (size_t)n_reads + 1))) return rc;
  if ((rc = dev_realloc(h, &s.d_exc_bits, &s.exc_bits_cap, (size_t)n_reads / 32 + 2))) return rc;
  if (h->d_occ32 && h->d_freq11 && p->k == 12 && p->step == 3) {
    const size_t R = (size_t)(p->e + 1 + p->a);
    if ((rc = dev_realloc(h, &s.d_sel, &s.sel_cap, (size_t)n_reads * 6u * R * h->n_banks))) return rc;
    if ((rc = dev_realloc(h, &s.d_sel_hdr, &s.sel_hdr_cap, (size_t)n_reads))) return rc;
  }
  if (!s.tail) s.tail = new (std::nothrow) femt::Tail();
  if (!s.tail) return fail(h, FEM_ERR_NOMEM, "out of host memory");
  std::string err;
  if ((rc = s.tail->reserve((uint32_t)n_reads, (uint32_t)n_records, max_len, p->e, h->tiny_buffers, &err))) return fail(h, rc, err);
  if (!s.text_stream) HIP_TRY(h, hipStreamCreateWithFlags(&s.text_stream, hipStreamNonBlocking));
  HIP_TRY(h, hipMemsetAsync(s.d_sel_hdr ? (void *)s.d_sel_hdr : (void *)s.d_off, 0, 8, s.text_stream));
  HIP_TRY(h, hipStreamSynchronize(s.text_stream));
  HIP_TRY(h, hipMemsetAsync(s.d_off, 0, 8, h->side_stream));
  HIP_TRY(h, hipStreamSynchronize(h->side_stream));
  const size_t probe = 1u << 20;
  if (s.h_bases && s.h_bases_cap >= probe && s.bases_cap >= kFrontPad + probe)
    HIP_TRY(h, hipMemcpyAsync(s.d_bases_alloc + kFrontPad, s.h_bases, probe, hipMemcpyHostToDevice, s.stream));
  if (s.h_quals && s.d_quals && s.h_quals_cap >= probe && s.d_quals_cap >= probe)
    HIP_TRY(h, hipMemcpyAsync(s.d_quals, s.h_quals, probe, hipMemcpyHostToDevice, s.text_stream));
  HIP_TRY(h, hipMemcpyAsync(s.h_ctl, s.d_ctl, kCtlBytes, hipMemcpyDeviceToHost, s.stream));
  HIP_TRY(h, hipStreamSynchronize(s.text_stream));
  HIP_TRY(h, hipStreamSynchronize(s.stream));
  if ((rc = s.tail->warm(out_stream_of(h, s), &err))) return fail(h, rc, err);
  return FEM_OK;
}

static int commit_text(fem_dev *h, int slot, uint64_t n_reads, uint64_t n_name_bytes, bool with_quals) {
  int rc = check_slot(h, slot);
  if (rc) return rc;
  FEM_LOCK(h);
  Slot &s = h->slot[slot];
  if (!s.staged) return fail(h, FEM_ERR_STATE, "commit the reads of the batch first");
  if ((with_quals && !s.h_quals) || !s.h_names || !s.h_name_off) return fail(h, FEM_ERR_STATE, "acquire the slot's text staging buffers first");
  if (n_reads != s.n_reads) return fail(h, FEM_ERR_INVALID, "as many names as reads, please");
  if ((with_quals && s.n_bases + 64 > s.h_quals_cap) || n_name_bytes + 64 > s.h_names_cap || n_reads + 1 > s.h_name_off_cap)
    return fail(h, FEM_ERR_INVALID, "more qualities or names than the text staging buffers were acquired for");
  if (n_reads && (s.h_name_off[0] != 0 || s.h_name_off[n_reads] != n_name_bytes))
    return fail(h, FEM_ERR_INVALID, "name offsets must start at 0 and end at the number of name bytes");
  HIP_TRY(h, hipSetDevice(h->device));
  if (with_quals && (rc = dev_realloc(h, &s.d_quals, &s.d_quals_cap, (size_t)s.n_bases + 64))) return rc;
  if ((rc = dev_realloc(h, &s.d_names, &s.d_names_cap, (size_t)n_name_bytes + 64))) return rc;
  if ((rc = dev_realloc(h, &s.d_name_off, &s.d_name_off_cap, (size_t)n_reads + 1))) return rc;
  if (!s.text_stream) HIP_TRY(h, hipStreamCreateWithFlags(&s.text_stream, hipStreamNonBlocking));
  if (!s.ev_text_staged) HIP_TRY(h, hipEventCreateWithFlags(&s.ev_text_staged, hipEventDisableTiming));
  if (s.have_text_order) HIP_TRY(h, hipStreamWaitEvent(s.text_stream, s.ev_text_order, 0));
  if (with_quals && s.n_bases) HIP_TRY(h, hipMemcpyAsync(s.d_quals, s.h_quals, s.n_bases, hipMemcpyHostToDevice, s.text_stream));
  if (n_name_bytes) HIP_TRY(h, hipMemcpyAsync(s.d_names, s.h_names, n_name_bytes, hipMemcpyHostToDevice, s.text_stream));
  HIP_TRY(h, hipMemcpyAsync(s.d_name_off, s.h_name_off, (n_reads + 1) * sizeof(uint64_t), hipMemcpyHostToDevice, s.text_stream));
  HIP_TRY(h, hipEventRecord(s.ev_text_staged, s.text_stream));
  s.text_staged = true, s.host_quals = !with_quals, s.qual_at = nullptr;
// ... 571 lines not shown
```

### fem_amd/csrc/fem_kernels.hip.h

```cpp
#pragma once
#include <hip/hip_runtime.h>
#include <stdint.h>
#include "fem_planes.hip.h"

namespace femk {

constexpr int kWave = 64;
constexpr uint32_t kFlagCandOverflow = 1u;
constexpr uint32_t kFlagArenaOverflow = 2u;
constexpr uint32_t kFlagTooLarge = 4u;
constexpr uint32_t kInvalidMeta = 0xFFFFFFFFu;
constexpr int kMaxR = 10;
constexpr uint32_t kMeta16 = 0x80000000u;
constexpr uint32_t kSlotChunk = 256u;
constexpr uint32_t kFlagQueueOverflow = 8u;
constexpr uint32_t kQueueChunk = 32u;
constexpr uint32_t kInvalidRead = 0xFFFFFFFFu;

struct SeedLayout {
  uint32_t pkw, nkw;
  uint32_t sf;
  uint32_t dp_rows;
  uint32_t dp_bits;
  uint32_t picked;
// ... 885 lines not shown
  lds.B = (uint64_t *)(wbase + p.lay.B);
  lds.xcap = p.lay.xcap, lds.fcap = p.lay.fcap, lds.ccap = p.lay.ccap;

  const int k = p.k, step = p.step, R = p.R, lg = p.lg;
  const uint32_t hash_mask = (k == 16) ? 0xFFFFFFFFu : ((1u << (2 * k)) - 1u);
  const uint32_t smax = p.lay.smax, cmax = p.lay.cmax, cw = p.lay.cw;
  unsigned long long pre_sum = 0, cand_sum = 0;
  SlotChunk chunk;
  Prof prof;

  const uint32_t wave_global = blockIdx.x * waves_per_block + wave_in_block;
  const uint32_t n_waves = gridDim.x * waves_per_block;

  const uint32_t n_items = p.work_queue ? min(p.ctr[2], p.slow_cap) : p.n_reads;
  for (uint32_t item = wave_global; item < n_items; item += n_waves) {
    const uint32_t read = p.work_queue ? p.work_queue[item] : item;
    if (read == kInvalidRead) continue;
    STAMP_START(prof);
    const uint64_t off = p.read_off[read];
    const uint32_t L = (uint32_t)(p.read_off[read + 1] - off);
    const uint8_t *seq = p.bases + off;
    const int S = (int)L - k + 1;

    bool shape_ok = S > 0 && R <= S / step;
    if (shape_ok) {
      int g_min = (S - (step - 1)) / step;
      shape_ok = g_min - R * lg + 2 >= 2;
    }
    if (!shape_ok || (uint32_t)S > smax) {
      if (ln < 2) {
        p.cand_begin[read * 2u + ln] = 0;
        p.cand_count[read * 2u + ln] = 0;
      }
      continue;
    }

    uint32_t n_fwd_amb = 0, n_rev_amb = 0;
    {
      const uint32_t n_words = (L + 15u) / 16u + 2u;
      for (uint32_t w = ln; w < n_words; w += kWave) {
        pkw[w] = 0;
        nkw[w] = 0;
      }
      wave_sync_lds();
      uint8_t *pkb = (uint8_t *)pkw, *nkb = (uint8_t *)nkw;
      for (uint32_t b0 = 0; b0 < L; b0 += 256u) {
        uint32_t idx = b0 + 4u * ln;
        if (idx < L) {
          uint32_t pv = 0, nv = 0;
#pragma unroll
          for (int q = 0; q < 4; ++q) {
            uint32_t c = 0, isn = 0;
            if (idx + q < L) {
              uint32_t code = base_code(seq[idx + q]);
              isn = code >> 2;
              c = code & 3u & (isn - 1u);
              n_fwd_amb += isn & (uint32_t)(idx + q >= (uint32_t)k);
              n_rev_amb += isn & (uint32_t)(L - 1u - (idx + q) >= (uint32_t)k);
            }
            pv = (pv << 2) | c;
            nv = (nv << 2) | (isn * 3u);
          }
          uint32_t byte_addr = (idx >> 4) * 4u + (3u - ((idx >> 2) & 3u));
          pkb[byte_addr] = (uint8_t)pv;
          nkb[byte_addr] = (uint8_t)nv;
        }
      }
      if (__any(n_fwd_amb | n_rev_amb)) {
        for (int d = 32; d >= 1; d >>= 1) {
          n_fwd_amb += __shfl_xor(n_fwd_amb, d);
          n_rev_amb += __shfl_xor(n_rev_amb, d);
        }
      }
      wave_sync_lds();
    }
    const bool strand_ok[2] = {n_fwd_amb <= (uint32_t)p.e, n_rev_amb <= (uint32_t)p.e};
    STAMP(prof, 0);

    for (int j0 = 0; j0 < S; j0 += kWave) {
      int j = j0 + (int)ln;
      if (j < S) {
        uint32_t w = (uint32_t)j >> 4, sh = 2u * ((uint32_t)j & 15u);
        uint64_t pw = ((uint64_t)pkw[w] << 32) | pkw[w + 1];
        uint64_t nw = ((uint64_t)nkw[w] << 32) | nkw[w + 1];
        uint32_t hf = (uint32_t)(pw >> (64 - 2 * k - sh)) & hash_mask;
        uint32_t nm = (uint32_t)(nw >> (64 - 2 * k - sh)) & hash_mask;
        uint32_t hr = reverse_pairs((~hf) & ~nm & hash_mask, k);
        if (strand_ok[0]) {
          uint32_t lo = p.lookup[hf], hi = p.lookup[hf + 1];
          sf[j] = make_uint2(lo, hi - lo);
        }
        if (strand_ok[1]) {
          uint32_t lo = p.lookup[hr], hi = p.lookup[hr + 1];
          sf[smax + (uint32_t)(S - 1 - j)] = make_uint2(lo, hi - lo);
        }
      }
    }
    wave_sync_lds();
    STAMP(prof, 1);

    uint32_t pre_g = 0;
    uint32_t dp_w = 0;
    if (2u * (uint32_t)step * (uint32_t)R <= (uint32_t)kWave && R <= kMaxR) {
      uint32_t widest = (uint32_t)(S / step - R * lg + 1);
      dp_w = widest <= 16u ? 16u : widest <= 32u ? 32u : widest <= 64u ? 64u : 0u;
    }
    if (dp_w) {
      pre_g = select_seeds_dpp<0, 0, 0>(p, S, strand_ok, sf, smax, dp_w, (unsigned long long *)dp_bits, picked);
    } else if (ln < 2u * (uint32_t)step && strand_ok[ln / (uint32_t)step]) {
      const uint32_t strand = ln / (uint32_t)step, si = ln % (uint32_t)step;
      const int G = (S - (int)si) / step;
      const int C = G - R * lg + 2;
      uint32_t *rows = dp_rows + (size_t)ln * 2u * cmax;
      uint32_t *bits = dp_bits + (size_t)ln * (uint32_t)R * cw;
      const uint2 *sfs = sf + strand * smax;
      for (int c = 1; c < C; ++c) rows[c] = 0;
      uint32_t left = p.inf32;
      for (int row = 1; row <= R; ++row) {
        const uint32_t *prev = rows + (size_t)((row - 1) & 1) * cmax;
        uint32_t *cur = rows + (size_t)(row & 1) * cmax;
        left = p.inf32;
        uint32_t acc = 0;
        for (int col = 1; col < C; ++col) {
          uint32_t pos = (uint32_t)(col + (row - 1) * lg - 1);
          uint32_t with_new = prev[col] + sfs[si + (uint32_t)step * pos].y;
          bool take = with_new < left;
          left = take ? with_new : left;
          cur[col] = left;
          acc |= (uint32_t)take << (col & 31);
          if ((col & 31) == 31 || col == C - 1) {
            bits[(uint32_t)(row - 1) * cw + ((uint32_t)col >> 5)] = acc;
            acc = 0;
          }
        }
      }
      pre_g = left;
      Picked *out = picked + (size_t)ln * (uint32_t)R;
      for (int t = 0; t < R; ++t) out[t] = Picked{0, 0, 0, 0};
      int r = R, c = C - 1, n_out = 0;
      while (r > 0 && c > 0) {
        uint32_t bit = (bits[(uint32_t)(r - 1) * cw + ((uint32_t)c >> 5)] >> (c & 31)) & 1u;
        if (bit) {
          uint32_t sidx = si + (uint32_t)step * (uint32_t)(c + (r - 1) * lg - 1);
          uint2 s = sfs[sidx];
          out[n_out++] = Picked{sidx, s.x, s.y, 0};
          --r;
        } else {
          --c;
        }
      }
      for (int i = 1; i < R; ++i) {
        Picked t = out[i];
        int j = i;
        while (j > 0 && t.freq < out[j - 1].freq) {
          out[j] = out[j - 1];
          --j;
        }
        out[j] = t;
      }
    }
    wave_sync_lds();
    STAMP(prof, 2);

    for (uint32_t strand = 0; strand < 2; ++strand) {
      if (!strand_ok[strand]) {
        if (ln == 0) {
          p.cand_begin[read * 2u + strand] = 0;
          p.cand_count[read * 2u + strand] = 0;
        }
        continue;
      }
      uint32_t pre = 0, pre_max = 0;
      unsigned long long pre_wide = 0;
      for (int si = 0; si < step; ++si) {
        uint32_t v = __shfl(pre_g, (int)(strand * (uint32_t)step) + si);
        pre += v;
        pre_wide += v;
        pre_max = v > pre_max ? v : pre_max;
      }
      pre_sum += pre;
      const Picked *pk = picked + (size_t)strand * (uint32_t)step * (uint32_t)R;
      uint64_t *list = nullptr;
      STAMP(prof, 3);
      if (strand_small(p, pk, lds.X, read, strand, L, cand_sum, chunk)) {
        STAMP(prof, 8);
        continue;
      }
      uint32_t n = strand_lists<false>(p, pk, rb, lds, &list, prof);
      if (n < 0xFFFFFFFEu) {
        clip_and_emit<false>(p, read, strand, L, list, n, list == lds.A ? lds.B : lds.A, cand_sum, chunk);
      } else if (n == 0xFFFFFFFEu) {
        if (ln == 0) atomicOr(&p.ctr[1], kFlagTooLarge);
      } else {
        unsigned long long want = 2ull * pre_max + 2ull * pre_wide + 8ull;
        unsigned long long base = 0;
        if (ln == 0) {
          base = atomicAdd(&p.arena_ctr[0], want);
          atomicAdd(&p.arena_ctr[1], want);
        }
        base = ((unsigned long long)bcast0((uint32_t)(base >> 32)) << 32) | bcast0((uint32_t)base);
        if (base + want > p.arena_cap) {
          if (ln == 0) atomicOr(&p.ctr[1], kFlagArenaOverflow);
          if (ln == 0) {
            p.cand_begin[read * 2u + strand] = 0;
            p.cand_count[read * 2u + strand] = 0;
          }
        } else {
          Bufs g;
          g.X = p.arena + base;
          g.F = g.X + pre_max + 2;
          g.A = g.F + pre_max + 2;
          g.B = g.A + pre_wide + 2;
          g.xcap = pre_max + 1u, g.fcap = pre_max + 1u;
          g.ccap = pre_wide > 0x7ffffff0ull ? 0x7ffffff0u : (uint32_t)pre_wide + 1u;
          uint32_t n2 = strand_lists_big(p, pk, rb, g, lds.X, p.lay.xcap + p.lay.fcap + 2u * p.lay.ccap, &list, prof);
          if (n2 < 0xFFFFFFFEu) {
            clip_and_emit<true>(p, read, strand, L, list, n2, list == g.A ? g.B : g.A, cand_sum, chunk);
          } else {
            if (ln == 0) atomicOr(&p.ctr[1], kFlagTooLarge);
          }
        }
      }
      wave_sync_lds();
      STAMP(prof, 7);
    }
  }
  pad_chunk(p, chunk);
#ifdef FEM_STAMPS
  prof.flush();
#endif
  if (ln == 0) {
    if (pre_sum) atomicAdd(&p.stats[0], pre_sum);
    if (cand_sum) atomicAdd(&p.stats[1], cand_sum);
  }
}

struct VerifyParams {
  const uint8_t *bases;
  const uint64_t *read_off;
  const uint8_t *planes;
  const uint64_t *seq_off;
  const uint64_t *cand;
  const uint32_t *cand_meta;
  const uint32_t *ctr;
  uint32_t cand_cap;
  int32_t e;
  uint8_t *ed;
  int16_t *end;
  uint32_t *n_map;
  unsigned long long *stats;
};

__device__ __forceinline__ uint4 load_u128_unaligned(const uint8_t *p) {
  uint4 w;
  __builtin_memcpy(&w, p, 16);
  return w;
}

__device__ __forceinline__ uint4 plane_window(const uint8_t *planes, int q, uint64_t at) {
  return load_u128_unaligned(plane_addr(planes, q, at));
}
__device__ __forceinline__ uint32_t load_u32_unaligned(const uint8_t *p) {
  uint32_t w;
  __builtin_memcpy(&w, p, 4);
  return w;
}

struct MyersState {
  uint32_t VP, VN;
  int score;
};

__device__ __forceinline__ void decode4(uint32_t chars, uint32_t complement, uint32_t &code, uint32_t &nflag) {
  const uint32_t t = (chars >> 1) & 0x03030303u;
  const uint32_t c = t ^ ((t >> 1) & 0x01010101u);
  const uint32_t upper = chars & 0xDFDFDFDFu;
  const uint32_t expect = __builtin_amdgcn_perm(0u, 0x54474341u , c);
  const uint32_t z = upper ^ expect;
  nflag = ((((z & 0x7F7F7F7Fu) + 0x7F7F7F7Fu) | z) >> 7) & 0x01010101u;
  code = (c ^ complement) & ~(nflag * 3u);
}

__device__ __forceinline__ uint32_t window_head(const uint4 &w, uint32_t off) { return __builtin_amdgcn_alignbit(w.y, w.x, off); }
__device__ __forceinline__ void window_advance16(uint4 &w) {
  w.x = __builtin_amdgcn_alignbit(w.y, w.x, 16u), w.y = __builtin_amdgcn_alignbit(w.z, w.y, 16u);
  w.z = __builtin_amdgcn_alignbit(w.w, w.z, 16u), w.w >>= 16;
}

__device__ __forceinline__ void myers_column(MyersState &m, uint32_t B0, uint32_t B1, uint32_t B2, uint32_t m0, uint32_t m1,
                                             uint32_t m2, uint32_t j, uint32_t width, uint32_t wm) {
  const uint32_t eq = __builtin_amdgcn_ubfe(~((B0 ^ m0) | (B1 ^ m1) | (B2 ^ m2)), j, width);
  uint32_t X = eq | m.VN;
  const uint32_t D0 = ((((X & m.VP) + m.VP) ^ m.VP) | X) & wm;
  const uint32_t HN = m.VP & D0;
  const uint32_t HP = (m.VN | ~(m.VP | D0)) & wm;
  X = D0 >> 1;
  m.VN = X & HP;
  m.VP = (HN | ~(X | HP)) & wm;
  m.score += 1 - (int)(D0 & 1u);
}

constexpr int kStepsPerPlaneLoad = 6;

__global__ void __launch_bounds__(256) verify_kernel(VerifyParams p) {
  if (p.ctr[1] != 0) return;
  const uint32_t total = min(p.ctr[0], p.cand_cap);
  const uint32_t stride = gridDim.x * blockDim.x;
  const int e = p.e;
  const uint32_t width = 2u * (uint32_t)e + 1u;
  constexpr int kStageChunks = 4;
  __shared__ uint4 stage[kStageChunks][256];
  uint32_t(*part)[4] = (uint32_t(*)[4]) & stage[0][0];
  uint32_t mappings = 0, mapped = 0;
  for (uint32_t i = blockIdx.x * blockDim.x + threadIdx.x; i < total; i += stride) {
    const uint32_t meta = p.cand_meta[i];
    if (meta == kInvalidMeta) {
      p.ed[i] = 0xFF, p.end[i] = 0;
      continue;
    }
    const uint32_t read = (meta & ~kMeta16) >> 1, strand = meta & 1u;
    const uint32_t wm = (meta & kMeta16) ? 0xFFFFu : 0xFFFFFFFFu;
    const uint64_t c = p.cand[i];
    const uint64_t pat = p.seq_off[(uint32_t)(c >> 32)] + (uint32_t)c;
    const uint64_t off = p.read_off[read];
    const int L = (int)(p.read_off[read + 1] - off);
    const uint8_t *rd = p.bases + off;
    const uint32_t complement = strand ? 0x03030303u : 0u;
    MyersState m{0, 0, 0};
    bool rejected = false;
    const int n_steps = (L + 15) >> 4;
    auto text_chunk = [&](int col) { return load_u128_unaligned(strand == 0 ? rd + col : rd + (L - 16 - col)); };
    auto plane_chunk = [&](int q, int col) { return plane_window(p.planes, q, (pat + (uint32_t)col) >> 3); };
    uint4 P0 = make_uint4(0, 0, 0, 0), P1 = P0, P2 = P0, P0n = P0, P1n = P0, P2n = P0;
    if (n_steps > 0) {
      P0n = plane_chunk(0, 0), P1n = plane_chunk(1, 0), P2n = plane_chunk(2, 0);
    }
    const uint32_t pat_bit = (uint32_t)pat & 7u;
    for (int step = 0; step < n_steps && !rejected; ++step) {
      const int col = step << 4, sub = step % kStepsPerPlaneLoad;
      if (step % kStageChunks == 0) {
        uint4 t4[kStageChunks];
#pragma unroll
        for (int c = 0; c < kStageChunks; ++c) t4[c] = step + c < n_steps ? text_chunk(col + 16 * c) : make_uint4(0, 0, 0, 0);
#pragma unroll
        for (int c = 0; c < kStageChunks; ++c) stage[c][threadIdx.x] = t4[c];
      }
      const uint4 r = stage[step % kStageChunks][threadIdx.x];
      if (sub == 0) {
        P0 = P0n, P1 = P1n, P2 = P2n;
        if (step + kStepsPerPlaneLoad < n_steps) {
          const int nc = col + 16 * kStepsPerPlaneLoad;
          P0n = plane_chunk(0, nc), P1n = plane_chunk(1, nc), P2n = plane_chunk(2, nc);
        }
      } else {
        window_advance16(P0), window_advance16(P1), window_advance16(P2);
      }
      const uint32_t b0 = window_head(P0, pat_bit), b1 = window_head(P1, pat_bit), b2 = window_head(P2, pat_bit);
      uint32_t cw[4], nw[4];
      {
        const uint32_t w0 = strand ? __builtin_bswap32(r.w) : r.x, w1 = strand ? __builtin_bswap32(r.z) : r.y;
        const uint32_t w2 = strand ? __builtin_bswap32(r.y) : r.z, w3 = strand ? __builtin_bswap32(r.x) : r.w;
        decode4(w0, complement, cw[0], nw[0]);
        decode4(w1, complement, cw[1], nw[1]);
        decode4(w2, complement, cw[2], nw[2]);
        decode4(w3, complement, cw[3], nw[3]);
      }
      if (col + 16 <= L) {
#pragma unroll
        for (int q = 0; q < 16; ++q) {
          const uint32_t m0 = (uint32_t)__builtin_amdgcn_sbfe((int)cw[q >> 2], 8 * (q & 3), 1);
          const uint32_t m1 = (uint32_t)__builtin_amdgcn_sbfe((int)cw[q >> 2], 8 * (q & 3) + 1, 1);
          const uint32_t m2 = (uint32_t)__builtin_amdgcn_sbfe((int)nw[q >> 2], 8 * (q & 3), 1);
          myers_column(m, b0, b1, b2, m0, m1, m2, (uint32_t)q, width, wm);
        }
      } else {
        const uint64_t clo = ((uint64_t)cw[1] << 32) | cw[0], chi = ((uint64_t)cw[3] << 32) | cw[2];
        const uint64_t nlo = ((uint64_t)nw[1] << 32) | nw[0], nhi = ((uint64_t)nw[3] << 32) | nw[2];
        for (int q = 0; q < L - col; ++q) {
          const uint32_t cb = (uint32_t)((q < 8 ? clo : chi) >> (8 * (q & 7)));
          const uint32_t nb = (uint32_t)((q < 8 ? nlo : nhi) >> (8 * (q & 7)));
          myers_column(m, b0, b1, b2, 0u - (cb & 1u), 0u - ((cb >> 1) & 1u), 0u - (nb & 1u), (uint32_t)q, width, wm);
        }
      }
      rejected = m.score > 3 * e;
    }
    int score = m.score;
    int best = score, endp = L - 1;
    if (!rejected) {
      for (int j = 0; j < 2 * e; ++j) {
        score += (int)((m.VP >> j) & 1u) - (int)((m.VN >> j) & 1u);
        if (score < best) {
          best = score;
          endp = L + j;
        }
      }
    }
    const bool accepted = !rejected && best <= e;
    p.ed[i] = accepted ? (uint8_t)best : (uint8_t)0xFF;
    p.end[i] = accepted ? (int16_t)endp : (int16_t)0;
    {
      const uint32_t ln = lane_id();
      const uint64_t acc = __ballot(accepted);
      const uint32_t prev_read = __shfl_up(read, 1);
      const bool joins_prev = accepted && ln > 0u && ((acc >> (ln - 1u)) & 1ull) && prev_read == read;
      const uint64_t heads = __ballot(accepted && !joins_prev);
      if (accepted && !joins_prev) {
        const uint64_t stop = (heads | ~acc) >> ln >> 1;
        const uint32_t run = stop ? (uint32_t)__builtin_ctzll(stop) + 1u : 64u - ln;
        mapped += (uint32_t)(atomicAdd(&p.n_map[read], run) == 0u);
      }
      if (accepted) ++mappings;
    }
  }
  for (int d = 32; d >= 1; d >>= 1) mappings += __shfl_xor(mappings, d), mapped += __shfl_xor(mapped, d);
  __syncthreads();
  if (lane_id() == 0) part[0][threadIdx.x >> 6] = mappings, part[1][threadIdx.x >> 6] = mapped;
  __syncthreads();
  if (threadIdx.x == 0) {
    const uint32_t a = part[0][0] + part[0][1] + part[0][2] + part[0][3], b = part[1][0] + part[1][1] + part[1][2] + part[1][3];
    if (a) atomicAdd(&p.stats[2], (unsigned long long)a);
    if (b) atomicAdd(&p.stats[3], (unsigned long long)b);
  }
}

struct PackParams {
  const uint32_t *cand_begin, *cand_count;
  const uint64_t *cand;
  const uint8_t *ed;
  const int16_t *end;
  const uint32_t *ctr;
  uint32_t n_strands;
  uint8_t *count8;
  uint32_t *seg_begin;
  uint64_t *pcand;
  uint8_t *ped;
  int16_t *pend;
  uint32_t pcap;
  uint32_t *cursor;
  uint2 *big;
  uint32_t big_cap;
};
constexpr uint32_t kPackSegs = 16;
__global__ void __launch_bounds__(256) pack_results_kernel(PackParams p) {
  if (p.ctr[1] != 0) return;
  __shared__ uint32_t part[kPackSegs * 4u];
  __shared__ uint32_t block_base;
  const uint32_t seg0 = blockIdx.x * kPackSegs;
  const uint32_t wave = threadIdx.x >> 6;
  uint32_t cnt[kPackSegs], beg[kPackSegs], incl[kPackSegs];
#pragma unroll
  for (uint32_t i = 0; i < kPackSegs; ++i) {
    const uint32_t s = (seg0 + i) * 256u + threadIdx.x;
    const bool in = s < p.n_strands;
    cnt[i] = in ? p.cand_count[s] : 0u;
    beg[i] = in ? p.cand_begin[s] : 0u;
  }
#pragma unroll
  for (uint32_t i = 0; i < kPackSegs; ++i) {
    uint32_t x = cnt[i];
    for (int d = 1; d < 64; d <<= 1) {
      const uint32_t o = __shfl_up(x, d);
      if ((int)lane_id() >= d) x += o;
    }
    incl[i] = x;
    if (lane_id() == 63) part[i * 4u + wave] = x;
  }
  __syncthreads();
  if (threadIdx.x < 64u) {
    const uint32_t v = part[threadIdx.x];
    uint32_t x = v;
    for (int d = 1; d < 64; d <<= 1) {
      const uint32_t o = __shfl_up(x, d);
      if ((int)threadIdx.x >= d) x += o;
    }
    part[threadIdx.x] = x - v;
    if (threadIdx.x == 63u) block_base = x ? atomicAdd(&p.cursor[0], x) : 0u;
  }
  __syncthreads();
  const uint32_t n_seg = (p.n_strands + 255u) / 256u;
#pragma unroll
  for (uint32_t i = 0; i < kPackSegs; ++i) {
    const uint32_t seg = seg0 + i, s = seg * 256u + threadIdx.x;
    if (threadIdx.x == 0 && seg < n_seg) p.seg_begin[seg] = block_base + part[i * 4u];
    if (s >= p.n_strands) continue;
    const uint32_t c = cnt[i], at = block_base + part[i * 4u + wave] + incl[i] - c;
    p.count8[s] = (uint8_t)(c < 255u ? c : 255u);
    if (c >= 255u) {
      const uint32_t j = atomicAdd(&p.cursor[1], 1u);
      if (j < p.big_cap) p.big[j] = make_uint2(s, c);
    }
    for (uint32_t k = 0; k < c; ++k) {
      if (at + k >= p.pcap) break;
      p.pcand[at + k] = p.cand[beg[i] + k];
      p.ped[at + k] = p.ed[beg[i] + k];
      p.pend[at + k] = p.end[beg[i] + k];
    }
  }
}

__global__ void ref_planes_kernel(const uint8_t *codes, const uint8_t *raw, uint64_t n_bytes, uint8_t *planes) {
  const uint64_t stride = (uint64_t)gridDim.x * blockDim.x;
  for (uint64_t b = (uint64_t)blockIdx.x * blockDim.x + threadIdx.x; b < n_bytes; b += stride) {
    uint64_t w, r;
    __builtin_memcpy(&w, codes + 8 * b, 8);
    __builtin_memcpy(&r, raw + 8 * b, 8);
    uint32_t o[4] = {0, 0, 0, 0};
    for (int k = 0; k < 8; ++k) {
      const uint32_t c = (uint32_t)(w >> (8 * k)) & 0xFFu, ch = (uint32_t)(r >> (8 * k)) & 0xFFu;
      o[0] |= (c & 1u) << k, o[1] |= ((c >> 1) & 1u) << k, o[2] |= ((c >> 2) & 1u) << k;
      o[3] |= (uint32_t)(ch != ((0x4E54474341ull >> (8u * c)) & 0xFFu)) << k;
    }
    const uint64_t g = b >> 4, r16 = b & 15u;
    for (int q = 0; q < 4; ++q) {
      planes[g * kPlaneGroup + (uint32_t)q * 32u + r16] = (uint8_t)o[q];
      if (g) planes[(g - 1) * kPlaneGroup + (uint32_t)q * 32u + 16u + r16] = (uint8_t)o[q];
    }
  }
}

constexpr uint32_t kSummaryBuckets = 24;

__device__ __forceinline__ void summary_slot(uint32_t h, uint32_t &q, uint32_t &r) {
  q = (uint32_t)((float)(h >> 3) * 0.33333334f);
  r = h - __umul24(q, kSummaryBuckets);
}
__device__ __forceinline__ bool summary_nonempty(uint32_t w, uint32_t r) { return (w >> r) & 1u; }
__device__ __forceinline__ bool summary_multi(uint32_t w, uint32_t r) { return (w >> (kSummaryBuckets + (__umul24(r, 11u) >> 5))) & 1u; }

__global__ void bucket_summary_kernel(const uint32_t *lookup, uint64_t n_buckets, uint32_t *summary) {
  const uint64_t stride = (uint64_t)gridDim.x * blockDim.x;
  for (uint64_t h = (uint64_t)blockIdx.x * blockDim.x + threadIdx.x; h < n_buckets; h += stride) {
    const uint32_t f = lookup[h + 1] - lookup[h];
    if (f == 0u) continue;
    const uint32_t q = (uint32_t)(h / kSummaryBuckets), r = (uint32_t)(h % kSummaryBuckets);
    atomicOr(&summary[q], (1u << r) | (f >= 2u ? 1u << (kSummaryBuckets + r / 3u) : 0u));
  }
}

__global__ void ref_encode_kernel(uint8_t *text, uint64_t n) {
  uint64_t stride = (uint64_t)gridDim.x * blockDim.x;
  for (uint64_t i = (uint64_t)blockIdx.x * blockDim.x + threadIdx.x; i < n; i += stride)
    text[i] = (uint8_t)base_code(text[i]);
}

}
```

### fem_amd/csrc/fem_seed_join.hip.h

```cpp
#pragma once
#include "fem_seed_dense.hip.h"

namespace femk {

#ifndef FEM_JOIN_SLOTS_HI
#define FEM_JOIN_SLOTS_HI 32768u
#endif
#ifndef FEM_JOIN_OPT
#define FEM_JOIN_OPT 15
#endif
#ifndef FEM_JOIN_OPT_HI
#define FEM_JOIN_OPT_HI 12
#endif
#ifndef FEM_JOIN_ABL
#define FEM_JOIN_ABL 0
#endif
#ifndef FEM_JOIN_SLOTS_LO
#define FEM_JOIN_SLOTS_LO 32768u
#endif
constexpr uint32_t join_slots(int R, bool padded = false) { return R >= 7 ? FEM_JOIN_SLOTS_HI : padded ? FEM_JOIN_SLOTS_LO : 32768u; }
#ifndef FEM_JOIN_BATCH_HI
#define FEM_JOIN_BATCH_HI 3
#endif

// ... 182 lines not shown
          }
        };
#pragma unroll 1
        for (int t = 0; t < R; ++t) {
          uint32_t a_ = 0, b_ = 0;
#pragma unroll
          for (int q = 0; q < R; ++q) a_ = q == t ? val[q] : a_, b_ = q == t ? hv[q] : b_;
          uint32_t f_t = 0, st_t = 0;
#pragma unroll
          for (int q = 0; q < R; ++q) f_t = q == t ? f[q] : f_t, st_t = q == t ? st[q] : st_t;
          settle(a_, ln < f_t, st_t);
          settle(b_, long_lists && ln + (uint32_t)kWave < f_t, st_t);
          if (t < R - 1) {
            if (a_ < kDenseVLimit) mx = a_ > mx ? a_ : mx, have_u = 1;
            if (b_ < kDenseVLimit) mx = b_ > mx ? b_ : mx, have_u = 1;
          }
          if (kOptSent) a_ = a_ < kDenseVLimit ? a_ : sent_b;
#pragma unroll
          for (int q = 0; q < R; ++q) val[q] = q == t ? a_ : val[q], hv[q] = q == t ? b_ : hv[q];
        }
        any_u = __builtin_amdgcn_ballot_w64(have_u != 0) != 0;
        max_u = wave_max_u32(mx);
        if (kOptSent) {
#pragma unroll
          for (int t = 0; t < R; ++t) vm[t] = __builtin_amdgcn_ballot_w64(val[t] < kDenseVLimit);
        }
      } else {
        if (kOptSent) {
#pragma unroll
          for (int t = 0; t < R; ++t) {
            if (PADDED) {
              vm[t] = __builtin_amdgcn_ballot_w64(ln < f[t]);
              val[t] -= st[t];
            } else {
              const bool in = ln < f[t];
              vm[t] = __builtin_amdgcn_ballot_w64(in);
              val[t] = (in ? val[t] : sent_a) - st[t];
            }
          }
        } else {
#pragma unroll
          for (int t = 0; t < R; ++t) val[t] = PADDED ? val[t] - st[t] : ln < f[t] ? val[t] - st[t] : kDenseSent;
        }
        if (long_lists) {
#pragma unroll
          for (int t = 0; t < R; ++t) {
            if (PADDED && (!kOptLong || f[t] > (uint32_t)kWave))
              hv[t] -= st[t];
            else
              hv[t] = ln + (uint32_t)kWave < f[t] ? hv[t] - st[t] : kDenseSent;
          }
#pragma unroll
          for (int t = 0; t < R - 1; ++t) {
            const uint32_t l_lo = (uint32_t)__builtin_amdgcn_readlane((int)val[t], (int)((f[t] - 1u) & 63u));
            const uint32_t l_hi = (uint32_t)__builtin_amdgcn_readlane((int)hv[t], (int)((f[t] - 65u) & 63u));
            const uint32_t lastv = f[t] > (uint32_t)kWave ? l_hi : l_lo;
            max_u = f[t] && lastv > max_u ? lastv : max_u;
          }
        } else {
#pragma unroll
          for (int t = 0; t < R - 1; ++t) {
            const uint32_t lastv = (uint32_t)__builtin_amdgcn_readlane((int)val[t], (int)((f[t] - 1u) & 63u));
            max_u = f[t] && lastv > max_u ? lastv : max_u;
          }
        }
      }
      if (keep_all) any_u = true, max_u = 0xFFFFFFFFu;
      if (any_u) {
        if (kOptSent) {
          const bool keep = val[R - 1] <= max_u;
          vm[R - 1] &= __builtin_amdgcn_ballot_w64(keep);
          val[R - 1] = keep ? val[R - 1] : sent_b;
        } else {
          val[R - 1] = val[R - 1] <= max_u ? val[R - 1] : kDenseSent;
        }
        if (long_lists) hv[R - 1] = hv[R - 1] <= max_u ? hv[R - 1] : kDenseSent;
        constexpr int kBatch = R <= 6 ? R : FEM_JOIN_BATCH_HI;
        auto flag_chunk = [&](uint32_t v, uint32_t xw, uint64_t valid, bool exact) {
          if (FEM_JOIN_ABL & 1) {
            asm volatile("" ::"v"(xw), "v"(v));
            return;
          }
          bool near = xw >= kNearTop;
          if (exact) near = near && v < kDenseVLimit;
          const uint64_t m = exact ? __builtin_amdgcn_ballot_w64(near) : __builtin_amdgcn_ballot_w64(near) & valid;
          if (!exact && m == 0) return;
          uint32_t pos = __builtin_amdgcn_mbcnt_hi((uint32_t)(m >> 32), __builtin_amdgcn_mbcnt_lo((uint32_t)m, n_flag));
          pos = pos < kFlagCap ? pos : kFlagCap;
          if (near) flg_g[pos] = v;
          n_flag += (uint32_t)__popcll(m);
        };
        auto insert_all = [&](uint32_t (&vals)[R], bool checked, bool second) {
#pragma unroll
          for (int t0 = 0; t0 < R; t0 += kBatch) {
            uint32_t hit[kBatch];
#pragma unroll
            for (int q = 0; q < kBatch; ++q)
              if (t0 + q < R) {
                hit[q] = 0;
                if (second && kOptLong && f[t0 + q] <= (uint32_t)kWave) continue;
                hit[q] = checked ? insert(vals[t0 + q]) : insert_plain(vals[t0 + q]);
              }
#pragma unroll
            for (int q = 0; q < kBatch; ++q)
              if (t0 + q < R) {
                if (second && kOptLong && f[t0 + q] <= (uint32_t)kWave) continue;
                if (kOptHit) {
                  mark(vals[t0 + q], hit[q]);
                } else if (__builtin_amdgcn_ballot_w64(hit[q] != 0u)) {
                  mark(vals[t0 + q], hit[q]);
                }
              }
          }
        };
        auto flag_all = [&](uint32_t (&vals)[R], bool second, bool exact) {
#pragma unroll
          for (int t0 = 0; t0 < R; t0 += kBatch) {
            uint32_t x[kBatch];
#pragma unroll
            for (int q = 0; q < kBatch; ++q)
              if (t0 + q < R) {
                if (second && kOptLong && f[t0 + q] <= (uint32_t)kWave) continue;
                x[q] = window_top(vals[t0 + q]);
              }
#pragma unroll
            for (int q = 0; q < kBatch; ++q)
              if (t0 + q < R) {
                if (second && kOptLong && f[t0 + q] <= (uint32_t)kWave) continue;
                flag_chunk(vals[t0 + q], x[q], vm[t0 + q], exact);
              }
          }
        };
        if (FEM_JOIN_ABL & 64) {
#pragma unroll
          for (int t = 0; t < R; ++t) asm volatile("" ::"v"(val[t]), "v"(hv[t]));
        } else {
        insert_all(val, !kOptSent, false);
        if (long_lists) insert_all(hv, true, true);
        wave_sync_lds();
        if (!kOptSent || __builtin_expect(remap, 0)) flag_all(val, false, true); else flag_all(val, false, false);
        if (long_lists) flag_all(hv, true, true);
        wave_sync_lds();
        }
        if (!(FEM_JOIN_ABL & 8)) {
          uint4 *b4 = (uint4 *)bitmap;
#pragma unroll
          for (uint32_t k = 0; k < kWords / 4u / (uint32_t)kWave; ++k) b4[k * (uint32_t)kWave + ln] = make_uint4(0u, 0u, 0u, 0u);
        }
        wave_sync_lds();
        if (n_flag > kFlagCap) return false;
      }
    }
    if (kSecondProbe && n_flag > kProbeMin) {
      const bool have0 = ln < n_flag, have1 = ln + (uint32_t)kWave < n_flag;
      const uint32_t v0 = have0 ? flg_g[ln] : 0u, v1 = have1 ? flg_g[ln + (uint32_t)kWave] : 0u;
      auto key2 = [&](uint32_t v) -> uint32_t {
        const uint32_t slot2 = (__builtin_amdgcn_ubfe(v, 3u, kSlotBits) + (v >> kPeriodBits) * 0x9E5u) & (kSlots - 1u);
        return (slot2 << 3) | (v & 7u);
      };
      auto edge = [&](uint32_t v) -> bool {
        const uint32_t lo = v & ((1u << kPeriodBits) - 1u);
        return lo < e || lo + e >= (1u << kPeriodBits);
      };
      auto wipe = [&](uint32_t k) {
        const uint32_t qm = (k >> 3) - 1u;
        uint32_t *w = bitmap + __builtin_amdgcn_ubfe(qm, 5u, kWordBits);
        w[0] = 0u, w[1] = 0u;
      };
      const uint32_t k0 = key2(v0), k1 = key2(v1);
      const uint32_t h0 = insert(have0 ? k0 : kDenseSent), h1 = insert(have1 ? k1 : kDenseSent);
      if (__builtin_amdgcn_ballot_w64((h0 | h1) != 0u)) mark(k0, h0), mark(k1, h1);
      wave_sync_lds();
      const bool keep0 = have0 && (edge(v0) || (window(k0) & 5u) != 0u);
      const bool keep1 = have1 && (edge(v1) || (window(k1) & 5u) != 0u);
      wave_sync_lds();
      if (have0) wipe(k0);
      if (have1) wipe(k1);
      wave_sync_lds();
      if (ln == 0) bitmap[kWords] = 0xFFFFFFFFu;
      const uint64_t m0 = __builtin_amdgcn_ballot_w64(keep0), m1 = __builtin_amdgcn_ballot_w64(keep1);
      const uint32_t c0 = (uint32_t)__popcll(m0);
      if (keep0) flg_g[__builtin_amdgcn_mbcnt_hi((uint32_t)(m0 >> 32), __builtin_amdgcn_mbcnt_lo((uint32_t)m0, 0u))] = v0;
      if (keep1) flg_g[__builtin_amdgcn_mbcnt_hi((uint32_t)(m1 >> 32), __builtin_amdgcn_mbcnt_lo((uint32_t)m1, c0))] = v1;
      n_flag = c0 + (uint32_t)__popcll(m1);
      wave_sync_lds();
      if (kOptPairs) {
        if (ln >= n_flag) flg_g[ln] = 0xFFFFFFFFu;
        if (kFlagCap > (uint32_t)kWave && ln + (uint32_t)kWave >= n_flag) flg_g[ln + (uint32_t)kWave] = 0xFFFFFFFFu;
        wave_sync_lds();
      }
    }
    if (!(FEM_JOIN_ABL & 2) && n_flag > (uint32_t)p.a) {
      const bool have = ln < n_flag;
      uint32_t fv;
      uint32_t cnt = 0;
      bool pass_hi = false;
      uint32_t fv_hi = 0;
      if (kOptPairs && n_flag <= 8u) {
        const uint32_t xj = flg_g[ln & 7u], fi = flg_g[ln >> 3];
        const uint64_t m = __builtin_amdgcn_ballot_w64(xj - fi <= e);
        cnt = (uint32_t)__popc((uint32_t)(m >> (8u * (ln & 7u))) & 0xFFu);
        fv = have ? xj : 0u;
      } else if (kOptPairs && n_flag <= 16u) {
        const uint32_t xj = flg_g[ln & 15u];
        const uint32_t *fp = flg_g + (ln >> 4);
        const uint64_t m0 = __builtin_amdgcn_ballot_w64(xj - fp[0] <= e), m1 = __builtin_amdgcn_ballot_w64(xj - fp[4] <= e);
        const uint64_t m2 = __builtin_amdgcn_ballot_w64(xj - fp[8] <= e), m3 = __builtin_amdgcn_ballot_w64(xj - fp[12] <= e);
        const uint32_t r0 = (uint32_t)(m0 >> sh16), r1 = (uint32_t)(m1 >> sh16), r2 = (uint32_t)(m2 >> sh16), r3 = (uint32_t)(m3 >> sh16);
        uint32_t row = r0;
        asm("v_cndmask_b32 %0, %0, %1, %2" : "+v"(row) : "v"(r1), "s"(q_is1));
        asm("v_cndmask_b32 %0, %0, %1, %2" : "+v"(row) : "v"(r2), "s"(q_is2));
        asm("v_cndmask_b32 %0, %0, %1, %2" : "+v"(row) : "v"(r3), "s"(q_is3));
        cnt = (uint32_t)__popc(row & 0xFFFFu);
        fv = have ? xj : 0u;
      } else {
        fv = have ? flg_g[ln] : 0u;
        const uint32_t n_lo = n_flag < (uint32_t)kWave ? n_flag : (uint32_t)kWave;
        if (kFlagCap > (uint32_t)kWave && n_flag > (uint32_t)kWave) {
          const bool have_hi = ln + (uint32_t)kWave < n_flag;
          fv_hi = have_hi ? flg_g[ln + (uint32_t)kWave] : 0u;
          uint32_t cnt_hi = 0;
          for (uint32_t j = 0; j < n_lo; ++j) {
            const uint32_t x = (uint32_t)__builtin_amdgcn_readlane((int)fv, (int)j);
            cnt += (uint32_t)(x - fv <= e), cnt_hi += (uint32_t)(x - fv_hi <= e);
          }
          for (uint32_t j = (uint32_t)kWave; j < n_flag; ++j) {
            const uint32_t x = (uint32_t)__builtin_amdgcn_readlane((int)fv_hi, (int)(j - (uint32_t)kWave));
            cnt += (uint32_t)(x - fv <= e), cnt_hi += (uint32_t)(x - fv_hi <= e);
          }
          pass_hi = have_hi && cnt_hi > (uint32_t)p.a;
        } else {
          for (uint32_t j = 0; j < n_lo; ++j) {
            const uint32_t x = (uint32_t)__builtin_amdgcn_readlane((int)fv, (int)j);
            cnt += (uint32_t)(x - fv <= e);
          }
        }
      }
      const bool pass = have && cnt > (uint32_t)p.a;
      const uint64_t pm = __builtin_amdgcn_ballot_w64(pass);
      if (__builtin_amdgcn_ballot_w64(pass_hi)) {
        any_hi = true;
        cmin = pass_hi && fv_hi < cmin ? fv_hi : cmin;
        cmax = pass_hi && fv_hi > cmax ? fv_hi : cmax;
      }
      if (pm != 0) {
        if (g == 0) pm0 = pm, nf0 = n_flag;
        else if (g == 1) pm1 = pm, nf1 = n_flag;
        else pm2 = pm, nf2 = n_flag;
        cmin = pass && fv < cmin ? fv : cmin;
        cmax = pass && fv > cmax ? fv : cmax;
      }
    }
    if (g != (uint32_t)kStep - 1u) continue;
    uint32_t kept = 0, cv = 0;
    if ((pm0 | pm1 | pm2) != 0 || any_hi) {
      const uint32_t lo_all = wave_min_u32(cmin), hi_all = wave_max_u32(cmax);
      if (hi_all - lo_all <= e) {
        cv = ln == 0 ? lo_all : 0u;
        kept = 1;
      } else if (any_hi) {
        return false;
      } else {
#pragma unroll 1
        for (uint32_t gg = 0; gg < (uint32_t)kStep; ++gg) {
          const uint64_t pm = gg == 0 ? pm0 : gg == 1 ? pm1 : pm2;
          const uint32_t nfl = gg == 0 ? nf0 : gg == 1 ? nf1 : nf2;
          if (pm == 0) continue;
          const uint32_t nF = (uint32_t)__popcll(pm);
          const bool mine = (pm >> ln) & 1ull;
          const uint32_t fv = ln < nfl ? flg[gg * kFlgStride + ln] : 0u;
          uint32_t rank = 0;
          for (uint64_t m = pm; m;) {
            const int j = __builtin_ctzll(m);
            m &= m - 1;
            const uint32_t x = (uint32_t)__builtin_amdgcn_readlane((int)fv, j);
            rank += (uint32_t)(x < fv || (x == fv && (uint32_t)j < ln));
          }
          wave_sync_lds();
          if (mine) scatter[rank] = fv;
          wave_sync_lds();
          const uint32_t fs = ln < nF ? scatter[ln] : 0u;
          kept = dense_merge_group(cv, kept, fs, nF, e);
          if (kept == 0xFFFFFFFFu) return false;
        }
      }
    }
    cand_lds[(u >= (uint32_t)kStep ? (uint32_t)kWave : 0u) + ln] = cv;
    if (u >= (uint32_t)kStep) kept1 = kept; else kept0 = kept;
    cmin = 0xFFFFFFFFu, cmax = 0u, any_hi = false;
    pm0 = pm1 = pm2 = 0, nf0 = nf1 = nf2 = 0;
  }
  return true;
}

#ifndef FEM_JOIN_WAVES_LO
#define FEM_JOIN_WAVES_LO 7
#endif
#ifndef FEM_JOIN_WAVES_HI
#define FEM_JOIN_WAVES_HI 6
#endif

constexpr int join_waves(int R) { return R <= 6 ? FEM_JOIN_WAVES_LO : FEM_JOIN_WAVES_HI; }

template <int R, bool BANKED = false, bool PADDED = false>
__device__ __forceinline__ void seed_join_body(const SeedParams &p, uint8_t *smem) {
  constexpr uint32_t kSeeds = (uint32_t)(kStep * R);
  static_assert(2 * kStep * R <= kWave, "both strands' seeds must fit the lanes of one wave");
  const uint32_t ln = lane_id();
  const uint32_t wave_in_block = (uint32_t)__builtin_amdgcn_readfirstlane((int)(threadIdx.x >> 6));
  uint8_t *wbase = smem + (size_t)wave_in_block * p.lay.wave_bytes;
  uint32_t *scatter = (uint32_t *)(wbase + p.lay.X);
  uint32_t *flg = (uint32_t *)(wbase + p.lay.A);
  uint32_t *bitmap = (uint32_t *)(wbase + p.lay.F);
  uint2 *blk_entries = (uint2 *)(wbase + p.lay.B);
  uint32_t *cand_lds = (uint32_t *)(wbase + p.lay.sf);
  uint2 *seqtab = (uint2 *)(smem + p.lay.picked);
  const bool small_ref = p.n_seq <= (uint32_t)kWave;
  if (wave_in_block == 0) seqtab[ln] = ln < p.n_seq ? make_uint2(p.goff[ln], p.seq_len[ln]) : make_uint2(0xFFFFFFFFu, 0u);
  __syncthreads();
  for (uint32_t i = ln; i < join_bitmap_words(R, PADDED); i += kWave) bitmap[i] = i < join_slots(R, PADDED) / 32u ? 0u : 0xFFFFFFFFu;
  wave_sync_lds();
  unsigned long long pre_sum = 0, cand_sum = 0;
  SlotChunk chunk, qchunk;

  auto queue_slow = [&](uint32_t read) {
    if (qchunk.left == 0) {
      uint32_t base = 0;
      if (ln == 0) base = atomicAdd(&p.ctr[2], kQueueChunk);
      qchunk.next = bcast0(base);
      qchunk.left = kQueueChunk;
    }
    if (qchunk.next < p.slow_cap) {
      if (ln == 0) p.slow_queue[qchunk.next] = read;
    } else if (ln == 0) {
      atomicOr(&p.ctr[1], kFlagQueueOverflow);
    }
    ++qchunk.next, --qchunk.left;
  };

  for (;;) {
    uint32_t pull = 0;
    if (ln == 0) pull = atomicAdd(p.work_cursor, kReadBlock);
    pull = bcast0(pull);
    if ((uint64_t)p.read_begin + pull >= p.n_reads) break;
    const uint32_t r0 = p.read_begin + pull;
    const uint32_t n_blk = p.n_reads - r0 < kReadBlock ? p.n_reads - r0 : kReadBlock;
    if (ln < 2u * kReadBlock) blk_entries[ln] = make_uint2(kBlkSkip, 0u);
    uint2 hdr = make_uint2(kSelSlow, 0u);
    if (ln < n_blk) hdr = p.sel_hdr[r0 + ln];
    uint2 sel_next = make_uint2(0u, 0u);
    if (!BANKED && ln < 2u * kSeeds) sel_next = p.sel[(size_t)r0 * (2u * kSeeds) + ln];
    for (uint32_t rb = 0; rb < n_blk; ++rb) {
      const uint32_t read = r0 + rb;
      const uint32_t h0 = (uint32_t)__builtin_amdgcn_readlane((int)hdr.x, (int)rb);
      const uint32_t status = h0 & 3u, L = h0 >> 8;
      const uint2 sel = sel_next;
      if (!BANKED && rb + 1u < n_blk && ln < 2u * kSeeds) sel_next = p.sel[(size_t)(read + 1u) * (2u * kSeeds) + ln];
      if (status == kSelSlow) continue;
      if (status == kSelNone) {
        if (ln / 2u == rb) blk_entries[ln] = make_uint2(0u, 0u);
        continue;
      }
      if constexpr (BANKED) {
        constexpr uint32_t kStash = (uint32_t)kWave;
        uint64_t *stash = (uint64_t *)(wbase + p.lay.gq);
        uint32_t acc[2] = {0u, 0u};
        bool failed = false;
        for (uint32_t b = 0; b < p.n_banks && !failed; ++b) {
          uint2 sel_b = make_uint2(0u, 0u);
          if (ln < 2u * kSeeds) sel_b = p.sel[((size_t)read * p.n_banks + b) * (2u * kSeeds) + ln];
          uint32_t kept0 = 0, kept1 = 0;
          if (!join_read<R, true>(p, sel_b.y & 0xFFFFu, sel_b.x, sel_b.y >> 16, bitmap, flg, scatter, cand_lds, kept0, kept1, p.bank_first[b])) {
            failed = true;
            break;
          }
          const uint32_t sq_lo = p.bank_first[b], sq_hi = p.bank_first[b + 1u];
#pragma unroll 1
          for (uint32_t strand = 0; strand < 2u; ++strand) {
            const uint32_t kept = strand ? kept1 : kept0;
            if (kept == 0) continue;
            const uint32_t v = cand_lds[strand * (uint32_t)kWave + ln];
            uint32_t sq = 0, pos = 0, slen = 0;
            if (small_ref) {
              const uint2 tab = seqtab[ln];
              const bool mine = ln >= sq_lo && ln < sq_hi;
              for (uint32_t i = 0; i < kept; ++i) {
                const uint32_t vi = (uint32_t)__builtin_amdgcn_readlane((int)v, (int)i);
                const uint32_t s_i = sq_lo + (uint32_t)__popcll(__builtin_amdgcn_ballot_w64(mine && tab.x <= vi)) - 1u;
                const uint32_t g_i = (uint32_t)__builtin_amdgcn_readlane((int)tab.x, (int)s_i);
                const uint32_t l_i = (uint32_t)__builtin_amdgcn_readlane((int)tab.y, (int)s_i);
                if (ln == i) sq = s_i, pos = vi - g_i, slen = l_i;
              }
            } else if (ln < kept) {
              sq = p.blkseq[(size_t)b * p.blk_stride + (v >> kDenseBlkShift)];
              while (sq + 1u < sq_hi && p.goff[sq + 1u] <= v) ++sq;
              pos = v - p.goff[sq];
              slen = p.seq_len[sq];
            }
            const bool ok = ln < kept && pos >= (uint32_t)p.e && pos + L + (uint32_t)p.e < slen;
            const uint64_t mo = __ballot(ok);
            const uint32_t n_ok = (uint32_t)__popcll(mo);
            if (acc[strand] + n_ok > kStash) {
              failed = true;
              break;
            }
            if (ok) stash[strand * kStash + acc[strand] + (uint32_t)__popcll(mo & ((1ull << ln) - 1ull))] = (((uint64_t)sq << 32) | pos) - (uint64_t)p.e;
            acc[strand] += n_ok;
          }
        }
        if (failed) {
          queue_slow(read);
          continue;
        }
        pre_sum += (uint32_t)__builtin_amdgcn_readlane((int)hdr.y, (int)rb);
        wave_sync_lds();
#pragma unroll 1
        for (uint32_t strand = 0; strand < 2u; ++strand) {
          const uint32_t n_out = acc[strand];
          uint32_t base = 0;
          if (n_out > 0) {
            if (n_out <= chunk.left) {
              base = chunk.next;
              chunk.next += n_out, chunk.left -= n_out;
            } else {
              pad_chunk(p, chunk);
              if (ln == 0) base = atomicAdd(&p.ctr[0], kSlotChunk);
              base = bcast0(base);
              chunk.next = base + n_out, chunk.left = kSlotChunk - n_out;
            }
            if ((unsigned long long)base + n_out > p.cand_cap) {
              if (ln == 0) atomicOr(&p.ctr[1], kFlagCandOverflow);
            } else {
              for (uint32_t i = ln; i < n_out; i += (uint32_t)kWave) {
                p.cand[base + i] = stash[strand * kStash + i];
                p.cand_meta[base + i] = (read * 2u + strand) | (i < (n_out & ~7u) ? kMeta16 : 0u);
              }
            }
          }
          if (ln == 0) blk_entries[2u * rb + strand] = make_uint2(base, n_out);
          cand_sum += n_out;
        }
        wave_sync_lds();
        continue;
      }
      const uint32_t s_lo = sel.x, s_start = sel.y & 0xFFFFu, s_freq = sel.y >> 16;
      uint32_t kept0 = 0, kept1 = 0;
      if (!join_read<R, false, PADDED>(p, s_start, s_lo, s_freq, bitmap, flg, scatter, cand_lds, kept0, kept1)) {
        queue_slow(read);
        continue;
      }
      if (FEM_JOIN_ABL & 16) kept0 = kept1 = 0;
      pre_sum += (uint32_t)__builtin_amdgcn_readlane((int)hdr.y, (int)rb);
#pragma unroll 1
      for (uint32_t strand = 0; strand < 2u; ++strand) {
        const uint32_t kept = strand ? kept1 : kept0;
        uint64_t out = 0;
        bool ok = false;
        if (kept == 0) {
          if (ln == 0) blk_entries[2u * rb + strand] = make_uint2(0u, 0u);
          continue;
        }
        const uint32_t v = cand_lds[strand * (uint32_t)kWave + ln];
        uint32_t sq = 0, pos = 0, slen = 0;
        if (small_ref) {
          const uint2 tab = seqtab[ln];
          for (uint32_t i = 0; i < kept; ++i) {
            const uint32_t vi = (uint32_t)__builtin_amdgcn_readlane((int)v, (int)i);
            const uint32_t s_i = (uint32_t)__popcll(__builtin_amdgcn_ballot_w64(tab.x <= vi)) - 1u;
            const uint32_t g_i = (uint32_t)__builtin_amdgcn_readlane((int)tab.x, (int)s_i);
            const uint32_t l_i = (uint32_t)__builtin_amdgcn_readlane((int)tab.y, (int)s_i);
            if (ln == i) sq = s_i, pos = vi - g_i, slen = l_i;
          }
        } else if (ln < kept) {
          sq = p.blkseq[v >> kDenseBlkShift];
          while (sq + 1u < p.n_seq && p.goff[sq + 1u] <= v) ++sq;
          pos = v - p.goff[sq];
          slen = p.seq_len[sq];
        }
        if (ln < kept) {
          ok = pos >= (uint32_t)p.e && pos + L + (uint32_t)p.e < slen;
          out = (((uint64_t)sq << 32) | pos) - (uint64_t)p.e;
        }
        const uint64_t mo = __ballot(ok);
        const uint32_t n_out = (uint32_t)__popcll(mo);
        uint32_t base = 0;
        if (n_out > 0) {
          if (n_out <= chunk.left) {
            base = chunk.next;
            chunk.next += n_out, chunk.left -= n_out;
          } else {
            pad_chunk(p, chunk);
            if (ln == 0) base = atomicAdd(&p.ctr[0], kSlotChunk);
            base = bcast0(base);
            chunk.next = base + n_out, chunk.left = kSlotChunk - n_out;
          }
          if ((unsigned long long)base + n_out > p.cand_cap) {
            if (ln == 0) atomicOr(&p.ctr[1], kFlagCandOverflow);
          } else if (ok) {
            const uint32_t rank = (uint32_t)__popcll(mo & ((1ull << ln) - 1ull)), at = base + rank;
            p.cand[at] = out;
            p.cand_meta[at] = (read * 2u + strand) | (rank < (n_out & ~7u) ? kMeta16 : 0u);
          }
        }
        if (ln == 0) blk_entries[2u * rb + strand] = make_uint2(base, n_out);
        cand_sum += n_out;
      }
    }
    wave_sync_lds();
    const uint2 entry = blk_entries[ln];
    wave_sync_lds();
    if (ln < 2u * kReadBlock && r0 + ln / 2u < p.n_reads && entry.x != kBlkSkip) {
      __builtin_nontemporal_store(entry.x, &p.cand_begin[r0 * 2u + ln]);
      __builtin_nontemporal_store(entry.y, &p.cand_count[r0 * 2u + ln]);
    }
  }
  pad_chunk(p, chunk);
  for (uint32_t i = ln; i < qchunk.left; i += kWave)
    if (qchunk.next + i < p.slow_cap) p.slow_queue[qchunk.next + i] = kInvalidRead;
  if (ln == 0) {
    if (pre_sum) atomicAdd(&p.stats[0], pre_sum);
    if (cand_sum) atomicAdd(&p.stats[1], cand_sum);
  }
}


#define FEM_JOIN_KERNEL(R, WAVES)                                                                                               \
  __global__ void __launch_bounds__(256) __attribute__((amdgpu_waves_per_eu(WAVES, 8))) seed_join_kernel_r##R(SeedParams p) {                         \
    extern __shared__ __attribute__((aligned(16))) uint8_t smem[];                                                               \
    seed_join_body<R>(p, smem);                                                                                                  \
  }                                                                                                                              \
  __global__ void __launch_bounds__(256) __attribute__((amdgpu_waves_per_eu(FEM_JOIN_WAVES_HI, 8))) seed_join_banked_kernel_r##R(SeedParams p) {  \
    extern __shared__ __attribute__((aligned(16))) uint8_t smem[];                                                               \
    seed_join_body<R, true>(p, smem);                                                                                            \
  }                                                                                                                              \
  __global__ void __launch_bounds__(256) __attribute__((amdgpu_waves_per_eu(WAVES, 8))) seed_join_kernel_padded_r##R(SeedParams p) {  \
    extern __shared__ __attribute__((aligned(16))) uint8_t smem[];                                                               \
    seed_join_body<R, false, true>(p, smem);                                                                                     \
  }
FEM_JOIN_KERNEL(1, FEM_JOIN_WAVES_LO)
FEM_JOIN_KERNEL(2, FEM_JOIN_WAVES_LO)
FEM_JOIN_KERNEL(3, FEM_JOIN_WAVES_LO)
FEM_JOIN_KERNEL(4, FEM_JOIN_WAVES_LO)
FEM_JOIN_KERNEL(5, FEM_JOIN_WAVES_LO)
FEM_JOIN_KERNEL(6, FEM_JOIN_WAVES_LO)
FEM_JOIN_KERNEL(7, FEM_JOIN_WAVES_HI)
FEM_JOIN_KERNEL(8, FEM_JOIN_WAVES_HI)
FEM_JOIN_KERNEL(9, FEM_JOIN_WAVES_HI)
FEM_JOIN_KERNEL(10, FEM_JOIN_WAVES_HI)
#undef FEM_JOIN_KERNEL

}
```

Baseline: 336.9.

## Defer verify kernel and run it as a ride-along tail of the next batch's join kernel

Instead of launching verify_kernel right after a batch's seeding, the batch's verify parameters are parked and executed by waves of the next batch's seed_join kernel once they finish their join work, pulling tickets of candidates from an atomic cursor and reusing the join's LDS bitmap as staging. This is meant to fill the idle tail of the join kernel and remove a separate kernel launch and its serialization. Pending verifies are settled explicitly whenever a slot is reused, synced, destroyed or takes a non-overlap path. It adds cross-batch coupling, extra register/code pressure in join kernels (mitigated with noinline cold tails), and delays result delivery for the previous batch.

```diff
diff --git a/fem_amd/csrc/fem_hip.hip b/fem_amd/csrc/fem_hip.hip
--- a/fem_amd/csrc/fem_hip.hip
+++ b/fem_amd/csrc/fem_hip.hip
@@ -131,6 +131,10 @@
   uint32_t n_packed = 0, n_big = 0;
   fem_params params{};
   bool mapped = false, synced = false;
+  bool verify_pending = false;
+  femk::VerifyParams ride_vp{};
+  uint32_t ride_vgrid = 0;
+  hipEvent_t ev_ride = nullptr;
   uint64_t stats[5] = {0, 0, 0, 0, 0};
   uint32_t n_cand = 0;
   std::vector<TimedLaunch> pending;
@@ -154,7 +158,8 @@
 constexpr size_t kCtlBytes = kCtlPackCursor + 2 * sizeof(uint32_t);
 constexpr uint32_t kBigCap = 4096;
 constexpr size_t kCtlWorkCursor = 128, kCtlWorkCursor2 = 192, kCtlPartStride = 128, kCtlAlloc = 1024;
-static_assert(kCtlWorkCursor2 + (kMaxParts - 1) * kCtlPartStride + 64 <= kCtlAlloc, "control block layout");
+constexpr size_t kCtlRideCursor = 768;
+static_assert(kCtlWorkCursor2 + (kMaxParts - 1) * kCtlPartStride + 64 <= kCtlRideCursor && kCtlRideCursor + 64 <= kCtlAlloc, "control block layout");
 static_assert(kCtlBytes <= kCtlWorkCursor, "control block layout");
 
 }
@@ -268,6 +273,8 @@
   hipEvent_t ev_select_done = nullptr;
   bool have_select_done = false;
   bool no_overlap = false;
+  int pending_slot = -1;
+  bool no_ride = false;
   hipEvent_t ev_h2d_done = nullptr;
   bool have_h2d_done = false;
   hipStream_t side_stream = nullptr;
@@ -470,7 +477,7 @@
                               : hipOccupancyMaxActiveBlocksPerMultiprocessor(&nb, femk::seed_select_kernel<R>, block, lds);
   return e == hipSuccess ? nb : 0;
 }
-typedef void (*JoinKernel)(femk::SeedParams);
+typedef void (*JoinKernel)(femk::SeedParams, femk::RideParams);
 JoinKernel join_kernel(int R, int which) {
   static const JoinKernel k[3][femk::kMaxR] = {
       {femk::seed_join_kernel_r1, femk::seed_join_kernel_r2, femk::seed_join_kernel_r3, femk::seed_join_kernel_r4, femk::seed_join_kernel_r5,
@@ -532,8 +539,8 @@
   int nb = 0;
   return hipOccupancyMaxActiveBlocksPerMultiprocessor(&nb, join_kernel(R, which), block, lds) == hipSuccess ? nb : 0;
 }
-void launch_join(int R, int which, dim3 grid, dim3 block, uint32_t lds, hipStream_t st, const femk::SeedParams &sp) {
-  hipLaunchKernelGGL(join_kernel(R, which), grid, block, lds, st, sp);
+void launch_join(int R, int which, dim3 grid, dim3 block, uint32_t lds, hipStream_t st, const femk::SeedParams &sp, const femk::RideParams &rp) {
+  hipLaunchKernelGGL(join_kernel(R, which), grid, block, lds, st, sp, rp);
 }
 
 template <int R>
@@ -777,7 +784,66 @@
   return FEM_OK;
 }
 
+template <typename F>
+int timed_launch(fem_dev *h, Slot &s, int id, hipStream_t st, F &&launch, bool counts = true) {
+  TimedLaunch t{id, nullptr, nullptr, counts};
+  if (h->timing) {
+    t.start = get_event(h), t.stop = get_event(h);
+    HIP_TRY(h, hipEventRecord(t.start, st));
+  }
+  launch();
+  HIP_TRY(h, hipGetLastError());
+  if (h->timing) {
+    HIP_TRY(h, hipEventRecord(t.stop, st));
+    s.pending.push_back(t);
+  }
+  return FEM_OK;
+}
+
+int enqueue_results_home(fem_dev *h, Slot &s) {
+  HIP_TRY(h, hipMemcpyAsync(s.h_ctl, s.d_ctl, kCtlBytes, hipMemcpyDeviceToHost, s.stream));
+  s.prefetched_reads2 = 0, s.prefetched_cand = 0;
+  static const bool no_prefetch = testing_switch("FEM_NO_PREFETCH");
+  if (s.prefetch_results && !s.want_packed && s.staged_by_copy && !no_prefetch) {
+    hipStream_t st = d2h_begin(h, s);
+    {
+      Span span(h, s, 21, st);
+      const size_t n2 = (size_t)s.n_reads * 2;
+      if (n2 && s.h_begin && n2 <= s.h_per_read_cap) {
+        HIP_TRY(h, hipMemcpyAsync(s.h_begin, s.d_begin, n2 * sizeof(uint32_t), hipMemcpyDeviceToHost, st));
+        HIP_TRY(h, hipMemcpyAsync(s.h_count, s.d_count, n2 * sizeof(uint32_t), hipMemcpyDeviceToHost, st));
+        s.prefetched_reads2 = n2;
+      }
+      const size_t guess = std::min<size_t>({(size_t)(s.last_n_cand + s.last_n_cand / 32 + 1024), s.h_cand_cap, (size_t)s.cand_cap});
+      if (s.last_n_cand && s.h_cand && guess) {
+        HIP_TRY(h, hipMemcpyAsync(s.h_cand, s.d_cand, guess * sizeof(uint64_t), hipMemcpyDeviceToHost, st));
+        HIP_TRY(h, hipMemcpyAsync(s.h_ed, s.d_ed, guess * sizeof(uint8_t), hipMemcpyDeviceToHost, st));
+        HIP_TRY(h, hipMemcpyAsync(s.h_end, s.d_end, guess * sizeof(int16_t), hipMemcpyDeviceToHost, st));
+        s.prefetched_cand = guess;
+      }
+    }
+    int rc2 = d2h_end(h, s, st);
+    if (rc2) return rc2;
+  }
+  return FEM_OK;
+}
+
+int settle_pending(fem_dev *h) {
+  if (h->pending_slot < 0) return FEM_OK;
+  Slot &ps = h->slot[h->pending_slot];
+  h->pending_slot = -1, ps.verify_pending = false;
+  const femk::VerifyParams vp = ps.ride_vp;
+  const uint32_t vgrid = ps.ride_vgrid;
+  hipStream_t st = ps.stream;
+  int rc = timed_launch(h, ps, 1, st, [&] { hipLaunchKernelGGL(femk::verify_kernel, dim3(vgrid), dim3(256), 0, st, vp); });
+  if (rc) return rc;
+  HIP_TRY(h, hipEventRecord(h->ev_kernels_done, st));
+  return enqueue_results_home(h, ps);
+}
+int settle_pending(fem_dev *h, const Slot &s) { return s.verify_pending ? settle_pending(h) : FEM_OK; }
+
 int launch_batch(fem_dev *h, Slot &s) {
+  if (int rc0 = settle_pending(h, s)) return rc0;
   const fem_params &p = s.params;
   uint32_t *d_ctr = (uint32_t *)s.d_ctl;
   unsigned long long *d_arena_ctr = (unsigned long long *)(s.d_ctl + 4 * sizeof(uint32_t));
@@ -840,25 +906,14 @@
   };
   if (sp.lay.wave_bytes > 64u * 1024u) return fail(h, FEM_ERR_UNSUPPORTED, "read too long for the device path");
 
-  auto timed = [&](int id, hipStream_t st, auto &&launch, bool counts = true) -> int {
-    TimedLaunch t{id, nullptr, nullptr, counts};
-    if (h->timing) {
-      t.start = get_event(h), t.stop = get_event(h);
-      HIP_TRY(h, hipEventRecord(t.start, st));
-    }
-    launch();
-    HIP_TRY(h, hipGetLastError());
-    if (h->timing) {
-      HIP_TRY(h, hipEventRecord(t.stop, st));
-      s.pending.push_back(t);
-    }
-    return FEM_OK;
-  };
-
+  auto timed = [&](int id, hipStream_t st, auto &&launch, bool counts = true) -> int { return timed_launch(h, s, id, st, launch, counts); };
+
+  bool defer = false;
   if (s.n_reads) {
     int rc;
     const bool split_dense = use_fast && h->d_occ32 && h->d_freq11;
     const bool overlap = split_dense && !h->no_overlap;
+    if (!split_dense && (rc = settle_pending(h))) return rc;
     if (!overlap && h->have_kernels_done) HIP_TRY(h, hipStreamWaitEvent(s.stream, h->ev_kernels_done, 0));
     femk::VerifyParams vp{};
     vp.bases = s.bases(), vp.read_off = s.d_off;
@@ -950,8 +1005,17 @@
           fp.lay = lay_join;
           const uint32_t grid = (uint32_t)std::max<uint64_t>(1, std::min<uint64_t>((blocks_of_reads + wpb_j - 1) / wpb_j, (uint64_t)h->n_cu * per_cu_j));
           fp.work_cursor = (uint32_t *)(s.d_ctl + kCtlWorkCursor2 + (size_t)q * kCtlPartStride);
-          rc = timed(0, s.stream, [&] { launch_join(R, which, dim3(grid), dim3(64u * wpb_j), lds_j, s.stream, fp); }, q == 0);
+          femk::RideParams rp{};
+          Slot *rider = h->pending_slot >= 0 ? &h->slot[h->pending_slot] : nullptr;
+          if (rider) rp.v = rider->ride_vp, rp.cursor = (uint32_t *)(rider->d_ctl + kCtlRideCursor);
+          rc = timed(0, s.stream, [&] { launch_join(R, which, dim3(grid), dim3(64u * wpb_j), lds_j, s.stream, fp, rp); }, q == 0);
           if (rc) return rc;
+          if (rider) {
+            h->pending_slot = -1, rider->verify_pending = false;
+            HIP_TRY(h, hipEventRecord(rider->ev_ride, s.stream));
+            HIP_TRY(h, hipStreamWaitEvent(rider->stream, rider->ev_ride, 0));
+            if ((rc = enqueue_results_home(h, *rider))) return rc;
+          }
         }
       }
       sp.work_queue = s.d_slow;
@@ -996,8 +1060,14 @@
       rc = timed(2, s.stream, [&] { hipLaunchKernelGGL(femk::seed_filter_kernel, dim3(grid), dim3(64u * wpb), lds_bytes, s.stream, sp); });
       if (rc) return rc;
     }
-    rc = timed(1, s.stream, [&] { hipLaunchKernelGGL(femk::verify_kernel, dim3(vgrid), dim3(256), 0, s.stream, vp); });
-    if (rc) return rc;
+    defer = overlap && !s.want_packed && !h->no_ride;
+    if (defer) {
+      s.ride_vp = vp, s.ride_vgrid = vgrid;
+      s.verify_pending = true, h->pending_slot = (int)(&s - h->slot);
+    } else {
+      rc = timed(1, s.stream, [&] { hipLaunchKernelGGL(femk::verify_kernel, dim3(vgrid), dim3(256), 0, s.stream, vp); });
+      if (rc) return rc;
+    }
     s.packed_enqueued = false, s.packed_home = 0, s.packed_per_read_home = false;
     if (s.want_packed && split_dense && (rc = enqueue_pack(h, s, true, false))) return rc;
     HIP_TRY(h, hipEventRecord(h->ev_kernels_done, s.stream));
@@ -1006,28 +1076,9 @@
   } else {
     s.packed_enqueued = false, s.packed_home = 0, s.packed_per_read_home = false;
   }
-  HIP_TRY(h, hipMemcpyAsync(s.h_ctl, s.d_ctl, kCtlBytes, hipMemcpyDeviceToHost, s.stream));
   s.prefetched_reads2 = 0, s.prefetched_cand = 0;
-  static const bool no_prefetch = testing_switch("FEM_NO_PREFETCH");
-  if (s.prefetch_results && !s.want_packed && s.staged_by_copy && !no_prefetch) {
-    hipStream_t st = d2h_begin(h, s);
-    {
-      Span span(h, s, 21, st);
-      const size_t n2 = (size_t)s.n_reads * 2;
-      if (n2 && s.h_begin && n2 <= s.h_per_read_cap) {
-        HIP_TRY(h, hipMemcpyAsync(s.h_begin, s.d_begin, n2 * sizeof(uint32_t), hipMemcpyDeviceToHost, st));
-        HIP_TRY(h, hipMemcpyAsync(s.h_count, s.d_count, n2 * sizeof(uint32_t), hipMemcpyDeviceToHost, st));
-        s.prefetched_reads2 = n2;
-      }
-      const size_t guess = std::min<size_t>({(size_t)(s.last_n_cand + s.last_n_cand / 32 + 1024), s.h_cand_cap, (size_t)s.cand_cap});
-      if (s.last_n_cand && s.h_cand && guess) {
-        HIP_TRY(h, hipMemcpyAsync(s.h_cand, s.d_cand, guess * sizeof(uint64_t), hipMemcpyDeviceToHost, st));
-        HIP_TRY(h, hipMemcpyAsync(s.h_ed, s.d_ed, guess * sizeof(uint8_t), hipMemcpyDeviceToHost, st));
-        HIP_TRY(h, hipMemcpyAsync(s.h_end, s.d_end, guess * sizeof(int16_t), hipMemcpyDeviceToHost, st));
-        s.prefetched_cand = guess;
-      }
-    }
-    int rc2 = d2h_end(h, s, st);
+  if (!defer) {
+    int rc2 = enqueue_results_home(h, s);
     if (rc2) return rc2;
   }
   s.mapped = true;
@@ -1189,6 +1240,7 @@
   const uint64_t code_bytes = fempack::code_bytes(n, len), n_bases = n * (uint64_t)len;
   const uint64_t total = code_bytes + n_exc * 5u;
   int rc;
+  if ((rc = settle_pending(h, s))) return rc;
   if ((rc = dev_realloc(h, &s.d_packed, &s.packed_cap, (size_t)total + 64))) return rc;
   if ((rc = dev_realloc(h, &s.d_bases_alloc, &s.bases_cap, kFrontPad + (size_t)n_bases + 64))) return rc;
   if ((rc = dev_realloc(h, &s.d_off, &s.off_cap, (size_t)n + 1))) return rc;
@@ -1291,7 +1343,8 @@
     Slot &sl = h->slot[i];
     ok_ev = hipEventCreateWithFlags(&sl.ev_zeroed, hipEventDisableTiming) == hipSuccess &&
             hipEventCreateWithFlags(&sl.ev_results, hipEventDisableTiming) == hipSuccess &&
-            hipEventCreateWithFlags(&sl.ev_home, hipEventDisableTiming) == hipSuccess;
+            hipEventCreateWithFlags(&sl.ev_home, hipEventDisableTiming) == hipSuccess &&
+            hipEventCreateWithFlags(&sl.ev_ride, hipEventDisableTiming) == hipSuccess;
     for (int q = 0; ok_ev && q < kMaxParts; ++q)
       ok_ev = hipEventCreateWithFlags(&sl.ev_part[q], hipEventDisableTiming) == hipSuccess &&
               hipEventCreateWithFlags(&sl.ev_sel[q], hipEventDisableTiming) == hipSuccess;
@@ -1303,6 +1356,7 @@
   if (testing_switch("FEM_TESTING")) {
     h->no_overlap = testing_switch("FEM_NO_OVERLAP");
     h->no_parts = testing_switch("FEM_NO_PARTS");
+    h->no_ride = testing_switch("FEM_NO_RIDE");
     if (const char *mp = getenv("FEM_PARTS")) h->max_parts = std::min(kMaxParts, std::max(1, atoi(mp)));
     h->timeline = testing_switch("FEM_TIMELINE");
     if (h->timeline && hipEventCreate(&h->ev_epoch) == hipSuccess && hipEventRecord(h->ev_epoch, h->side_stream) == hipSuccess)
@@ -1327,6 +1381,10 @@
     if (g_comm && std::find(g_comm->devs.begin(), g_comm->devs.end(), h->device) != g_comm->devs.end()) destroy_comm_set();
   }
   (void)hipSetDevice(h->device);
+  {
+    FEM_LOCK(h);
+    (void)settle_pending(h);
+  }
   (void)hipDeviceSynchronize();
   delete h->stage_pool;
   h->stage_pool = nullptr;
@@ -1366,6 +1424,7 @@
     if (sl.ev_zeroed) (void)hipEventDestroy(sl.ev_zeroed);
     if (sl.ev_results) (void)hipEventDestroy(sl.ev_results);
     if (sl.ev_home) (void)hipEventDestroy(sl.ev_home);
+    if (sl.ev_ride) (void)hipEventDestroy(sl.ev_ride);
     for (int q = 0; q < kMaxParts; ++q) {
       if (sl.ev_part[q]) (void)hipEventDestroy(sl.ev_part[q]);
       if (sl.ev_sel[q]) (void)hipEventDestroy(sl.ev_sel[q]);
@@ -1530,6 +1589,7 @@
   if (n_reads_cap > 0x3FFFFFF0ull) return fail(h, FEM_ERR_UNSUPPORTED, "more than 2^30 reads in one batch");
   Slot &s = h->slot[slot];
   HIP_TRY(h, hipSetDevice(h->device));
+  if ((rc = settle_pending(h, s))) return rc;
   HIP_TRY(h, hipStreamSynchronize(s.stream));
   if (s.out_stream) HIP_TRY(h, hipStreamSynchronize(s.out_stream));
   drain_timing(h, s);
@@ -1553,6 +1613,7 @@
   const uint64_t n_bases = n_reads ? s.h_off[n_reads] : 0;
   if (n_reads && (s.h_off[0] != 0 || n_bases > s.acq_bases)) return fail(h, FEM_ERR_INVALID, "staged offsets must start at 0 and end inside the buffer");
   HIP_TRY(h, hipSetDevice(h->device));
+  if ((rc = settle_pending(h, s))) return rc;
   if ((rc = dev_realloc(h, &s.d_bases_alloc, &s.bases_cap, kFrontPad + (size_t)n_bases + 64))) return rc;
   if ((rc = dev_realloc(h, &s.d_off, &s.off_cap, (size_t)n_reads + 1))) return rc;
   if ((rc = h2d_begin(h, s))) return rc;
@@ -1577,6 +1638,7 @@
   const uint64_t n_bases = n_reads * (uint64_t)read_len;
   if (n_reads > s.acq_reads || n_bases > s.acq_bases) return fail(h, FEM_ERR_INVALID, "more reads than the staging buffers were acquired for");
   HIP_TRY(h, hipSetDevice(h->device));
+  if ((rc = settle_pending(h, s))) return rc;
   if ((rc = dev_realloc(h, &s.d_bases_alloc, &s.bases_cap, kFrontPad + (size_t)n_bases + 64))) return rc;
   if ((rc = dev_realloc(h, &s.d_off, &s.off_cap, (size_t)n_reads + 1))) return rc;
   if ((rc = h2d_begin(h, s))) return rc;
@@ -1733,6 +1795,7 @@
   Slot &s = h->slot[slot];
   if (!s.staged) return fail(h, FEM_ERR_STATE, "no reads staged in this slot");
   HIP_TRY(h, hipSetDevice(h->device));
+  if ((rc = settle_pending(h, s))) return rc;
   s.params = *p;
   if ((rc = ensure_outputs(h, s))) return rc;
   return launch_batch(h, s);
@@ -1746,6 +1809,10 @@
   HIP_TRY(h, hipSetDevice(h->device));
   if (s.synced) return FEM_OK;
   for (int attempt = 0; attempt < 8; ++attempt) {
+    {
+      FEM_LOCK(h);
+      if ((rc = settle_pending(h, s))) return rc;
+    }
     HIP_TRY(h, hipStreamSynchronize(s.stream));
     FEM_LOCK(h);
     drain_timing(h, s);
diff --git a/fem_amd/csrc/fem_kernels.hip.h b/fem_amd/csrc/fem_kernels.hip.h
--- a/fem_amd/csrc/fem_kernels.hip.h
+++ b/fem_amd/csrc/fem_kernels.hip.h
@@ -1211,17 +1211,15 @@
 
 constexpr int kStepsPerPlaneLoad = 6;
 
-__global__ void __launch_bounds__(256) verify_kernel(VerifyParams p) {
-  if (p.ctr[1] != 0) return;
-  const uint32_t total = min(p.ctr[0], p.cand_cap);
-  const uint32_t stride = gridDim.x * blockDim.x;
+constexpr int kStageChunks = 4;
+typedef uint32_t StageWord4 __attribute__((ext_vector_type(4)));
+
+template <uint32_t kRow, typename StagePtr>
+__device__ __forceinline__ void verify_slots(const VerifyParams &p, uint32_t first, uint32_t limit, uint32_t stride, StagePtr stage,
+                                             uint32_t &mappings, uint32_t &mapped) {
   const int e = p.e;
   const uint32_t width = 2u * (uint32_t)e + 1u;
-  constexpr int kStageChunks = 4;
-  __shared__ uint4 stage[kStageChunks][256];
-  uint32_t(*part)[4] = (uint32_t(*)[4]) & stage[0][0];
-  uint32_t mappings = 0, mapped = 0;
-  for (uint32_t i = blockIdx.x * blockDim.x + threadIdx.x; i < total; i += stride) {
+  for (uint32_t i = first; i < limit; i += stride) {
     const uint32_t meta = p.cand_meta[i];
     if (meta == kInvalidMeta) {
       p.ed[i] = 0xFF, p.end[i] = 0;
@@ -1252,9 +1250,9 @@
 #pragma unroll
         for (int c = 0; c < kStageChunks; ++c) t4[c] = step + c < n_steps ? text_chunk(col + 16 * c) : make_uint4(0, 0, 0, 0);
 #pragma unroll
-        for (int c = 0; c < kStageChunks; ++c) stage[c][threadIdx.x] = t4[c];
-      }
-      const uint4 r = stage[step % kStageChunks][threadIdx.x];
+        for (int c = 0; c < kStageChunks; ++c) stage[(uint32_t)c * kRow] = StageWord4{t4[c].x, t4[c].y, t4[c].z, t4[c].w};
+      }
+      const StageWord4 r = stage[(uint32_t)(step % kStageChunks) * kRow];
       if (sub == 0) {
         P0 = P0n, P1 = P1n, P2 = P2n;
         if (step + kStepsPerPlaneLoad < n_steps) {
@@ -1321,6 +1319,16 @@
       if (accepted) ++mappings;
     }
   }
+}
+
+__global__ void __launch_bounds__(256) verify_kernel(VerifyParams p) {
+  if (p.ctr[1] != 0) return;
+  const uint32_t total = min(p.ctr[0], p.cand_cap);
+  const uint32_t stride = gridDim.x * blockDim.x;
+  __shared__ StageWord4 stage[kStageChunks][256];
+  uint32_t(*part)[4] = (uint32_t(*)[4]) & stage[0][0];
+  uint32_t mappings = 0, mapped = 0;
+  verify_slots<256u>(p, blockIdx.x * blockDim.x + threadIdx.x, total, stride, &stage[0][threadIdx.x], mappings, mapped);
   for (int d = 32; d >= 1; d >>= 1) mappings += __shfl_xor(mappings, d), mapped += __shfl_xor(mapped, d);
   __syncthreads();
   if (lane_id() == 0) part[0][threadIdx.x >> 6] = mappings, part[1][threadIdx.x >> 6] = mapped;
diff --git a/fem_amd/csrc/fem_seed_join.hip.h b/fem_amd/csrc/fem_seed_join.hip.h
--- a/fem_amd/csrc/fem_seed_join.hip.h
+++ b/fem_amd/csrc/fem_seed_join.hip.h
@@ -508,8 +508,82 @@
 
 constexpr int join_waves(int R) { return R <= 6 ? FEM_JOIN_WAVES_LO : FEM_JOIN_WAVES_HI; }
 
-template <int R, bool BANKED = false, bool PADDED = false>
-__device__ __forceinline__ void seed_join_body(const SeedParams &p, uint8_t *smem) {
+struct RideParams {
+  VerifyParams v;
+  uint32_t *cursor;
+};
+#ifndef FEM_RIDE_TICKET
+#define FEM_RIDE_TICKET 256u
+#endif
+#ifndef FEM_RIDE_TICKET_END
+#define FEM_RIDE_TICKET_END FEM_RIDE_TICKET
+#endif
+static_assert(FEM_RIDE_TICKET % 64u == 0u && FEM_RIDE_TICKET >= 64u, "a ticket is whole rounds of a wave");
+static_assert(FEM_RIDE_TICKET_END % 64u == 0u && FEM_RIDE_TICKET_END >= 64u && FEM_RIDE_TICKET_END <= FEM_RIDE_TICKET, "a ticket is whole rounds of a wave");
+
+template <typename T>
+__device__ __forceinline__ T *wave_uniform(T *p) {
+  const uint64_t a = (uint64_t)(uintptr_t)p;
+  return (T *)(uintptr_t)((uint64_t)(uint32_t)__builtin_amdgcn_readfirstlane((int)(uint32_t)a) |
+                          ((uint64_t)(uint32_t)__builtin_amdgcn_readfirstlane((int)(uint32_t)(a >> 32)) << 32));
+}
+__device__ __forceinline__ void join_ride_tail_body(const RideParams &rp_in, uint32_t *bitmap_in, uint32_t *sums_in, uint32_t wave_bytes) {
+  typedef __attribute__((address_space(3))) StageWord4 *LdsStage;
+  typedef __attribute__((address_space(3))) uint32_t *LdsWords;
+  VerifyParams v;
+  v.bases = wave_uniform(rp_in.v.bases), v.read_off = wave_uniform(rp_in.v.read_off), v.planes = wave_uniform(rp_in.v.planes);
+  v.seq_off = wave_uniform(rp_in.v.seq_off), v.cand = wave_uniform(rp_in.v.cand), v.cand_meta = wave_uniform(rp_in.v.cand_meta);
+  v.ctr = wave_uniform(rp_in.v.ctr), v.ed = wave_uniform(rp_in.v.ed), v.end = wave_uniform(rp_in.v.end);
+  v.n_map = wave_uniform(rp_in.v.n_map), v.stats = wave_uniform(rp_in.v.stats);
+  v.cand_cap = (uint32_t)__builtin_amdgcn_readfirstlane((int)rp_in.v.cand_cap), v.e = __builtin_amdgcn_readfirstlane(rp_in.v.e);
+  uint32_t *cursor = wave_uniform(rp_in.cursor);
+  wave_bytes = (uint32_t)__builtin_amdgcn_readfirstlane((int)wave_bytes);
+  const LdsStage stage = (LdsStage)bitmap_in;
+  const LdsWords sums = (LdsWords)sums_in;
+  if (v.ctr[1] != 0) return;
+  const uint32_t total = min(v.ctr[0], v.cand_cap);
+  const uint32_t ln = lane_id();
+  uint32_t mappings = 0, mapped = 0;
+  const uint32_t n_big = (total - total / 4u) / FEM_RIDE_TICKET;
+  for (;;) {
+    uint32_t k = 0;
+    if (ln == 0) k = atomicAdd(cursor, 1u);
+    k = bcast0(k);
+    const uint32_t size = k < n_big ? FEM_RIDE_TICKET : FEM_RIDE_TICKET_END;
+    const uint64_t base64 = k < n_big ? (uint64_t)k * FEM_RIDE_TICKET : (uint64_t)n_big * FEM_RIDE_TICKET + (uint64_t)(k - n_big) * FEM_RIDE_TICKET_END;
+    if (base64 >= total) break;
+    const uint32_t base = (uint32_t)base64;
+    const uint32_t limit = total - base < size ? total : base + size;
+    verify_slots<(uint32_t)kWave>(v, base + ln, limit, (uint32_t)kWave, stage + ln, mappings, mapped);
+  }
+  for (int d = 32; d >= 1; d >>= 1) mappings += __shfl_xor(mappings, d), mapped += __shfl_xor(mapped, d);
+  wave_sync_lds();
+  if (ln == 0) sums[0] = mappings, sums[1] = mapped;
+  __syncthreads();
+  if (threadIdx.x == 0) {
+    uint32_t a = 0, b = 0;
+    for (uint32_t w = 0; w < blockDim.x / (uint32_t)kWave; ++w) a += sums[w * (wave_bytes / 4u)], b += sums[w * (wave_bytes / 4u) + 1u];
+    if (a) atomicAdd(&v.stats[2], (unsigned long long)a);
+    if (b) atomicAdd(&v.stats[3], (unsigned long long)b);
+  }
+}
+#define FEM_RIDE_TAIL(WAVES)                                                                                                      \
+  __device__ __attribute__((noinline, cold)) void join_ride_tail_w##WAVES(                                                        \
+      RideParams rp, uint32_t *bitmap, uint32_t *sums, uint32_t wave_bytes) {                                                     \
+    join_ride_tail_body(rp, bitmap, sums, wave_bytes);                                                                            \
+  }
+FEM_RIDE_TAIL(6)
+FEM_RIDE_TAIL(7)
+#undef FEM_RIDE_TAIL
+template <int WAVES>
+__device__ __forceinline__ void join_ride_tail(const RideParams &rp, uint32_t *bitmap, uint32_t *sums, uint32_t wave_bytes) {
+  static_assert(WAVES == 6 || WAVES == 7, "one copy of the tail per register budget of the join kernels");
+  if (rp.cursor == nullptr) return;
+  if (WAVES == 7) join_ride_tail_w7(rp, bitmap, sums, wave_bytes); else join_ride_tail_w6(rp, bitmap, sums, wave_bytes);
+}
+
+template <int R, bool BANKED = false, bool PADDED = false, int WAVES = 7>
+__device__ __forceinline__ void seed_join_body(const SeedParams &p, const RideParams &rp, uint8_t *smem) {
   constexpr uint32_t kSeeds = (uint32_t)(kStep * R);
   static_assert(2 * kStep * R <= kWave, "both strands' seeds must fit the lanes of one wave");
   const uint32_t ln = lane_id();
@@ -727,21 +801,23 @@
     if (pre_sum) atomicAdd(&p.stats[0], pre_sum);
     if (cand_sum) atomicAdd(&p.stats[1], cand_sum);
   }
+  static_assert(join_bitmap_words(R, PADDED) * 4u >= (uint32_t)kStageChunks * (uint32_t)kWave * 16u, "the bitmap holds a wave's staged chunks");
+  join_ride_tail<WAVES>(rp, bitmap, cand_lds, p.lay.wave_bytes);
 }
 
 
 #define FEM_JOIN_KERNEL(R, WAVES)                                                                                               \
-  __global__ void __launch_bounds__(256) __attribute__((amdgpu_waves_per_eu(WAVES, 8))) seed_join_kernel_r##R(SeedParams p) {                         \
+  __global__ void __launch_bounds__(256) __attribute__((amdgpu_waves_per_eu(WAVES, 8))) seed_join_kernel_r##R(SeedParams p, RideParams rp) {                         \
     extern __shared__ __attribute__((aligned(16))) uint8_t smem[];                                                               \
-    seed_join_body<R>(p, smem);                                                                                                  \
+    seed_join_body<R, false, false, WAVES>(p, rp, smem);                                                                                                  \
   }                                                                                                                              \
-  __global__ void __launch_bounds__(256) __attribute__((amdgpu_waves_per_eu(FEM_JOIN_WAVES_HI, 8))) seed_join_banked_kernel_r##R(SeedParams p) {  \
+  __global__ void __launch_bounds__(256) __attribute__((amdgpu_waves_per_eu(FEM_JOIN_WAVES_HI, 8))) seed_join_banked_kernel_r##R(SeedParams p, RideParams rp) {  \
     extern __shared__ __attribute__((aligned(16))) uint8_t smem[];                                                               \
-    seed_join_body<R, true>(p, smem);                                                                                            \
+    seed_join_body<R, true, false, FEM_JOIN_WAVES_HI>(p, rp, smem);                                                                                            \
   }                                                                                                                              \
-  __global__ void __launch_bounds__(256) __attribute__((amdgpu_waves_per_eu(WAVES, 8))) seed_join_kernel_padded_r##R(SeedParams p) {  \
+  __global__ void __launch_bounds__(256) __attribute__((amdgpu_waves_per_eu(WAVES, 8))) seed_join_kernel_padded_r##R(SeedParams p, RideParams rp) {  \
     extern __shared__ __attribute__((aligned(16))) uint8_t smem[];                                                               \
-    seed_join_body<R, false, true>(p, smem);                                                                                     \
+    seed_join_body<R, false, true, WAVES>(p, rp, smem);                                                                                     \
   }
 FEM_JOIN_KERNEL(1, FEM_JOIN_WAVES_LO)
 FEM_JOIN_KERNEL(2, FEM_JOIN_WAVES_LO)
```

Result: slower. 327.1 (-2.9%).
